# iris-ua/iris_lama

Measured on AMD Instinct MI355X. Metric: particle-scans/sec, higher is better.
Workload: dtype f64; 1 GPU; PFSlam2D 30 particles, 1080-beam synthetic corridor log (SURVEY.md 8(d)), res 0.05 m, patch 32, l2_max 0.5, GN+Cauchy(0.15), seed 42; particles=30, beams=1080, parallelism=particle-shard x1

## Files before the change

### include/lama_hip.h

```cpp
#ifndef LAMA_HIP_H
#define LAMA_HIP_H

#include <stdint.h>

#ifdef __cplusplus
extern "C" {
#endif

#define LAMA_HIP_OK 0
#define LAMA_HIP_E_INVALID (-1)
#define LAMA_HIP_E_HIP (-2)
#define LAMA_HIP_E_WINDOW (-3)
#define LAMA_HIP_E_CAPACITY (-4)
#define LAMA_HIP_E_STATE (-5)
#define LAMA_HIP_E_NUMERIC (-6)

typedef struct lama_hip_ctx lama_hip_ctx;

typedef struct lama_hip_cfg {
    uint32_t particles;
    double resolution;
    uint32_t patch_size;
    double l2_max;
    double meas_sigma;
// ... 21 lines not shown

int32_t lama_hip_ctx_create(const lama_hip_cfg* cfg, lama_hip_ctx** out);
void lama_hip_ctx_destroy(lama_hip_ctx* ctx);
const char* lama_hip_last_error(const lama_hip_ctx* ctx);

int32_t lama_hip_pf_init(lama_hip_ctx* ctx, const double* pts_xyz, uint32_t n,
                         const double* sensor_origin3, const double* sensor_quat_wxyz,
                         const double* pose0);

int32_t lama_hip_pf_set_poses(lama_hip_ctx* ctx, const double* poses);
int32_t lama_hip_pf_get_poses(lama_hip_ctx* ctx, double* poses);

int32_t lama_hip_pf_scan_match(lama_hip_ctx* ctx, const double* pts_xyz, uint32_t n,
                               const double* sensor_origin3, const double* sensor_quat_wxyz,
                               double* poses_out, double* loglik_out, int32_t* iters_out);

int32_t lama_hip_pf_resample(lama_hip_ctx* ctx, const int32_t* sample_idx);

int32_t lama_hip_pf_update_maps(lama_hip_ctx* ctx, const double* pts_xyz, uint32_t n,
                                const double* sensor_origin3, const double* sensor_quat_wxyz);

#define LAMA_HIP_MAP_DISTANCE 0
#define LAMA_HIP_MAP_OCCUPANCY 1
int32_t lama_hip_pf_map_patches(lama_hip_ctx* ctx, uint32_t particle, int32_t kind, uint32_t* num_patches);
int32_t lama_hip_pf_download_map(lama_hip_ctx* ctx, uint32_t particle, int32_t kind, uint32_t cap,
                                 uint64_t* patch_ids, uint8_t* cells, uint64_t* masks, uint32_t* num_patches);

int32_t lama_hip_pf_upload_map(lama_hip_ctx* ctx, uint32_t particle, int32_t kind, uint32_t num_patches,
                               const uint64_t* patch_ids, const uint8_t* cells, const uint64_t* masks);

int32_t lama_hip_pf_update_maps_begin(lama_hip_ctx* ctx, const double* pts_xyz, uint32_t n,
                                      const double* sensor_origin3, const double* sensor_quat_wxyz);
int32_t lama_hip_sync(lama_hip_ctx* ctx);
int32_t lama_hip_ctx_device(const lama_hip_ctx* ctx);

int32_t lama_hip_pf_patch_ids(lama_hip_ctx* ctx, uint32_t particle, int32_t kind, uint32_t cap, uint64_t* patch_ids, uint32_t* num_patches);
int32_t lama_hip_pf_map_checksums(lama_hip_ctx* ctx, int32_t kind, uint64_t* out);
int32_t lama_hip_pf_delete_patches(lama_hip_ctx* ctx, uint32_t particle, const uint64_t* patch_ids, uint32_t n, uint32_t* deleted);

int32_t lama_hip_match_batch(lama_hip_ctx* ctx, uint32_t particle, const double* pts_xyz, uint32_t n,
                             const double* sensor_origin3, const double* sensor_quat_wxyz,
                             const double* poses, uint32_t num_poses, double* loglik_out);

int32_t lama_hip_eval_batch(lama_hip_ctx* ctx, uint32_t particle, const double* pts_xyz, uint32_t n,
                            const double* sensor_origin3, const double* sensor_quat_wxyz,
                            const double* poses, uint32_t num_poses, double* sqnorm_out, double* loglik_out);

#define LAMA_HIP_SAMPLE_MAX_TERMS 256
int32_t lama_hip_map_sample_likelihood(lama_hip_ctx* ctx, uint32_t particle, const double* pts_xyz, uint32_t n,
                                       const double* sensor_origin3, const double* sensor_quat_wxyz, double yaw,
                                       const double* xy, uint32_t num_samples, uint32_t point_step, double* l_out);

int32_t lama_hip_map_add_obstacles(lama_hip_ctx* ctx, uint32_t particle, const uint32_t* cells_xy, uint32_t n);
int32_t lama_hip_match_solve(lama_hip_ctx* ctx, uint32_t particle, const double* pts_xyz, uint32_t n,
                             const double* sensor_origin3, const double* sensor_quat_wxyz, double* pose_inout,
                             double* out7, int32_t* iters_out, int32_t do_solve);
int32_t lama_hip_match_solve_with(lama_hip_ctx* ctx, uint32_t particle, const double* pts_xyz, uint32_t n,
                                  const double* sensor_origin3, const double* sensor_quat_wxyz, double* pose_inout,
                                  double* out7, int32_t* iters_out, int32_t strategy, uint32_t max_iterations );
int32_t lama_hip_match_eval(lama_hip_ctx* ctx, uint32_t particle, const double* pts_xyz, uint32_t n,
                            const double* sensor_origin3, const double* sensor_quat_wxyz, const double* pose,
                            double* residuals, double* jacobian);
int32_t lama_hip_match_cell_distances(lama_hip_ctx* ctx, uint32_t particle, const double* pts_xyz, uint32_t n,
                                      const double* sensor_origin3, const double* sensor_quat_wxyz, const double* pose,
                                      double* distances);

#define LAMA_HIP_ROBUST_UNIT 0
#define LAMA_HIP_ROBUST_TUKEY 1
#define LAMA_HIP_ROBUST_TDIST 2
#define LAMA_HIP_ROBUST_CAUCHY 3
#define LAMA_HIP_ROBUST_HUBER 4
#define LAMA_HIP_ROBUST_STORED 0x100
int32_t lama_hip_match_solve_batch(lama_hip_ctx* ctx, uint32_t num_problems, const uint32_t* particles, const double* pts_xyz,
                                   const uint32_t* scan_offsets, const double* sensor_origin3_per_problem,
                                   const double* sensor_quat_wxyz_per_problem, double* poses_inout, const uint32_t* max_iterations,
                                   int32_t strategy, int32_t robust_kind, double robust_param, double* out8, int32_t* iters_out,
                                   uint32_t* status_out);

#define LAMA_HIP_MAP_BUILD_FULL 1u
#define LAMA_HIP_MAP_BUILD_PRUNE 2u
int32_t lama_hip_map_integrate_scans(lama_hip_ctx* ctx, uint32_t particle, uint32_t num_scans, const double* poses4,
                                     const double* pts_xyz, const uint32_t* scan_offsets, const double* sensor_origin3_per_scan,
                                     const double* sensor_quat_wxyz_per_scan, uint32_t flags);
int32_t lama_hip_map_occupied_cells(lama_hip_ctx* ctx, uint32_t particle, uint32_t cap, uint32_t* cells_xy, uint32_t* n);

int32_t lama_hip_pf_export_particle(lama_hip_ctx* ctx, uint32_t particle, void* device_buf, uint64_t cap, uint64_t* bytes);
int32_t lama_hip_pf_import_particle(lama_hip_ctx* ctx, uint32_t particle, const void* device_buf, uint64_t bytes);
int32_t lama_hip_pf_export_particles(lama_hip_ctx* ctx, uint32_t n, const uint32_t* particles, void* const* device_bufs, const uint64_t* caps,
                                     uint64_t* bytes_out);
int32_t lama_hip_pf_import_particles(lama_hip_ctx* ctx, uint32_t n, const uint32_t* particles, const void* const* device_bufs, const uint64_t* bytes);

int32_t lama_hip_blob_alloc(lama_hip_ctx* ctx, uint64_t bytes, void** device_buf);
int32_t lama_hip_blob_free(lama_hip_ctx* ctx, void* device_buf);
int32_t lama_hip_blob_copy(lama_hip_ctx* dst_ctx, void* dst_device_buf, lama_hip_ctx* src_ctx, const void* src_device_buf, uint64_t bytes);

typedef struct lama_hip_pgo lama_hip_pgo;
int32_t lama_hip_pgo_create(int32_t device, uint32_t num_poses, const int32_t* fi, const int32_t* fj, const double* meas4,
                            const double* sqrt_info3, uint32_t num_factors, lama_hip_pgo** out);
void lama_hip_pgo_destroy(lama_hip_pgo* g);
const char* lama_hip_pgo_last_error(const lama_hip_pgo* g);
int32_t lama_hip_pgo_linearize(lama_hip_pgo* g, const double* poses4, double* err, double* Hdiag, double* Hoff, double* b,
                               double* chi2, double* kernel_ms);

int32_t lama_hip_pgo_pattern(const lama_hip_pgo* g, int32_t* row_ptr, int32_t* cols, uint32_t* nnzb);
int32_t lama_hip_pgo_set_poses(lama_hip_pgo* g, const double* poses4);
int32_t lama_hip_pgo_get_poses(lama_hip_pgo* g, double* poses4);
int32_t lama_hip_pgo_linearize_system(lama_hip_pgo* g, double* blocks, double* b, double* diag, double* half_chi2, double* kernel_ms);
int32_t lama_hip_pgo_try_step(lama_hip_pgo* g, const double* dx, double* half_chi2, double* kernel_ms);
int32_t lama_hip_pgo_accept(lama_hip_pgo* g);

typedef struct lama_hip_counters {
    double ms_scan_match;  uint64_t launches_scan_match;
    double ms_update_maps; uint64_t launches_update_maps;
    double ms_raycast;     uint64_t launches_raycast;
    double ms_brushfire;   uint64_t launches_brushfire;
    double ms_resample;    uint64_t launches_resample;
    uint64_t gn_iterations;
    uint64_t gn_evals;
    uint64_t ray_cells;
    uint64_t bf_cells;
    uint64_t dm_patches;
    uint64_t occ_patches;
    double ms_eval_batch;  uint64_t launches_eval_batch;
    uint64_t arena_growths;
    uint64_t window_shifts;
    uint64_t wrap_guard_scans;
    uint32_t brushfire_mode;
    uint32_t brushfire_waves;
    uint64_t sequential_raycast_scans;
    uint64_t parallel_raycast_scans;
    uint32_t brushfire_handovers;
    uint32_t replay_handovers;
    uint32_t window_patches;
    uint32_t window_growths;
    uint64_t bf_longest_chain_sum;
    uint64_t bf_longest_chain_last;
    uint64_t brushfire_early;
    uint64_t brushfire_routed;
    uint64_t pool_growths;
    uint64_t resample_clones;
    uint64_t resample_bytes;
    uint64_t hbm_bytes_allocated;
    uint64_t hbm_bytes_used;
    uint64_t hbm_bytes_total;
    uint32_t peer_access;
    uint32_t struct_bytes;
    double peer_copy_ms;
    uint64_t peer_copy_bytes;
} lama_hip_counters;
int32_t lama_hip_get_counters(lama_hip_ctx* ctx, lama_hip_counters* out);
int32_t lama_hip_get_counters_sized(lama_hip_ctx* ctx, void* out, uint32_t bytes);
uint32_t lama_hip_counters_bytes(void);
int32_t lama_hip_reset_counters(lama_hip_ctx* ctx);

#ifdef __cplusplus
}
#endif
#endif
```

### iris_lama_amd/csrc/lama_hip.hip

```cpp
#include "../../include/lama_hip.h"

#include <hip/hip_runtime.h>

#include <algorithm>
#include <cmath>
#include <cstdio>
#include <cstdlib>
#include <cstring>
#include <map>
#include <memory>
#include <mutex>
#include <string>
#include <vector>

#include "lama_kernels.h"
#include "lama_pgo.h"
#include "lama_map_build.h"
#include "lama_match_batch.h"
#include "../host/pgo_pattern.hpp"

using namespace lama_dev;

namespace {

// ... 19 lines not shown
    }
    size_t bytes() const { return n * sizeof(T); }
    void swap(DevBuf& o) { std::swap(p, o.p); std::swap(n, o.n); }
    operator T*() const { return p; }
};

template <class H, hipError_t (*Destroy)(H)>
struct HipHandle {
    H h = nullptr;
    HipHandle() {}
    HipHandle(HipHandle&& o) noexcept : h(o.h) { o.h = nullptr; }
    HipHandle& operator=(HipHandle&&) = delete;
    ~HipHandle() { if (h) (void)Destroy(h); }
    operator H() const { return h; }
};
using Stream = HipHandle<hipStream_t, hipStreamDestroy>;
using Event = HipHandle<hipEvent_t, hipEventDestroy>;
struct Delete { template <class T> void operator()(T* q) const { delete q; } };

struct RegionAlloc;
struct PoolChunk {
    DevBuf<uint8_t> plane[4];
    uint32_t patches = 0;
};
struct MapStore {
    DevBuf<int16_t> dm_dir, occ_dir;
    int32_t* counts = nullptr;
    std::vector<PoolChunk> dm_chunks, occ_chunks;
};
constexpr size_t DM_PLANE_B[3] = {SV_PATCH_BYTES, 4096, 128};
constexpr size_t OCC_PLANE_B[4] = {4096, 128, 128, 4};
struct HostPart { uint32_t home, dm_chunk, dm_off, dm_cap, occ_chunk, occ_off, occ_cap; };

struct RegionAlloc {
    std::map<uint32_t, uint32_t> free_;
    uint32_t cap = 0, used = 0;
    void reset(uint32_t c) { free_.clear(); cap = c; used = 0; if (c) free_[0] = c; }
    bool alloc(uint32_t n, uint32_t& off)
    {
        if (n == 0) { off = 0; return true; }
        for (auto it = free_.begin(); it != free_.end(); ++it) {
            if (it->second < n) continue;
            off = it->first;
            const uint32_t rest = it->second - n;
            free_.erase(it);
            if (rest) free_[off + n] = rest;
            used += n;
            return true;
        }
        return false;
    }
    void release(uint32_t off, uint32_t n)
    {
        if (n == 0) return;
        used -= n;
        auto nx = free_.lower_bound(off);
        if (nx != free_.begin()) {
            auto pv = std::prev(nx);
            if (pv->first + pv->second == off) { off = pv->first; n += pv->second; free_.erase(pv); }
        }
        if (nx != free_.end() && off + n == nx->first) { n += nx->second; free_.erase(nx); }
        free_[off] = n;
    }
    void extend(uint32_t newcap) { if (newcap > cap) { const uint32_t o = cap, n = newcap - cap; cap = newcap; used += n; release(o, n); } }
    uint32_t largest_free() const { uint32_t m = 0; for (auto& kv : free_) m = std::max(m, kv.second); return m; }
};

}

template <class T>
struct PinVec {
    T* p = nullptr; size_t n = 0, cap = 0; bool pinned = false;
    PinVec() {}
    PinVec(const PinVec&) = delete;
    PinVec& operator=(const PinVec&) = delete;
    ~PinVec() { release(); }
    void release() { if (p) { if (pinned) (void)hipHostFree(p); else std::free(p); } p = nullptr; }
    void reserve(size_t m)
    {
        if (m <= cap) return;
        m = std::max(m, 2 * cap);
        T* q = nullptr;
        bool pin = hipHostMalloc((void**)&q, m * sizeof(T), hipHostMallocDefault) == hipSuccess && q;
        if (!pin) { (void)hipGetLastError(); q = (T*)std::malloc(m * sizeof(T)); }
        if (!q) std::abort();
        if (p) std::memcpy(q, p, n * sizeof(T));
        release();
        p = q; cap = m; pinned = pin;
    }
    void resize(size_t m) { reserve(m); if (m > n) std::memset(p + n, 0, (m - n) * sizeof(T)); n = m; }
    void assign(size_t m, T v) { reserve(m); n = m; for (size_t i = 0; i < m; ++i) p[i] = v; }
    T* data() { return p; }
    const T* data() const { return p; }
    size_t size() const { return n; }
    T& operator[](size_t i) { return p[i]; }
    const T& operator[](size_t i) const { return p[i]; }
};

struct lama_hip_ctx {
    lama_hip_cfg cfg;
    std::string error;
    Stream stream;
    Event ev0, ev1;
    struct PendingTimer { hipEvent_t a, b; double* acc; uint64_t* launches; };
    std::vector<Event> ev_pool;
    std::vector<PendingTimer> pending;
    size_t ev_used = 0;
    bool initialised = false;
    bool poisoned = false;

    uint32_t P = 0, W = 0, WC = 0, wx0 = 0, wy0 = 0;
    uint32_t max_sqdist = 0;
    double scale = 0, off = 0;

    MapStore ms;
    std::vector<RegionAlloc> ra_dm, ra_occ;
    std::vector<HostPart> h_part;
    DevBuf<PartRec> d_part;
    PinVec<PartRec> h_part_stage;
    PinVec<CloneJob> h_jobs; DevBuf<CloneJob> d_jobs;
    PinVec<ZeroJob> h_zjobs; DevBuf<ZeroJob> d_zjobs;
    uint32_t floor_dm = 128, floor_occ = 128;
    PinVec<uint32_t> h_guard;
    uint64_t clone_bytes = 0;
    double* d_poses = nullptr;
    DevBuf<uint64_t> d_qlower, d_qraise;
    uint64_t* d_stats = nullptr;
    DevBuf<uint32_t> d_qsizes;
    DevBuf<uint64_t> d_dbg;
    DevBuf<uint32_t> d_slow;
    DevBuf<uint32_t> d_slow_list; uint32_t* d_slow_n = nullptr;
    DevBuf<uint8_t> d_heavy;
    DevBuf<uint8_t> d_early; DevBuf<uint32_t> d_elist;
    Stream stream3; Event ev_alloc, ev_go, ev_early;
    bool early_ok = false;
    uint32_t early_candidates = 0;
    std::vector<double> h_ll; bool ll_valid = false;
    PinVec<uint32_t> h_hlist; DevBuf<uint32_t> d_hlist;
    uint32_t early_on = 1;
    uint32_t early_min_count = 1024;
    Stream stream2; Event ev_route, ev_heavy;
    uint32_t route_min_count = 64, route_min_events = 48, route_percent = 150, route_cap = 64;
    bool route_forced = false; uint32_t num_cus = 256;
    bool debug_tail = false, debug_window = false;
    uint32_t big_stage_pad = 0;
    DevBuf<uint64_t> d_act; DevBuf<uint32_t> d_act_count;
    DevBuf<lama_dev::RayRec> d_rrec; DevBuf<uint64_t> d_rbbox; DevBuf<lama_dev::RayChunk> d_rchunk;
    int32_t* d_err = nullptr;
    DevBuf<double> d_pts; uint32_t last_n = 0;
    PinVec<uint64_t> h_stats;
    PinVec<double> h_tfs, h_pts;
    PinVec<int32_t> h_err;
    PinVec<uint32_t> h_slow_n;
    DevBuf<double> d_tfs;
    double* d_loglik = nullptr; int32_t* d_iters = nullptr;
    DevBuf<uint8_t> d_results;
    size_t results_bytes = 0, status_off = 0, status_bytes = 0;
    PinVec<uint8_t> h_status;
    PinVec<uint8_t> h_results;
    DevBuf<int32_t> d_oldcounts;
    DevBuf<double> d_mb_pts, d_mb_tfs; DevBuf<uint32_t> d_mb_offs; DevBuf<lama_dev::MbRay> d_mb_rays;
    DevBuf<uint32_t> d_mb_table, d_mb_off, d_mb_list, d_mb_bins; DevBuf<int32_t> d_mb_slot; DevBuf<uint64_t> d_mb_meta;
    PinVec<double> h_mb_tfs; PinVec<uint32_t> h_mb_offs; PinVec<uint64_t> h_mb_meta;
    DevBuf<double> d_bposes, d_bout;
    DevBuf<double> d_msb_f64; DevBuf<uint32_t> d_msb_u32;
    PinVec<double> h_msb_f64; PinVec<uint32_t> h_msb_u32;

    double scan_reach = 0.0;
    uint32_t visit_bound = 0;
    DevBuf<uint32_t> d_scalar;
    DevBuf<lama_dev::ShipDesc> d_ship_desc; DevBuf<uint8_t> d_ship_heads;
    PinVec<lama_dev::ShipDesc> h_ship_desc; PinVec<uint8_t> h_ship_heads;
    uint32_t* d_guard = nullptr;
    Affine last_mtf; uint32_t last_first = 0, last_count = 0;
    bool last_guarded = false;
    int recover_depth = 0;
    int64_t mbx0 = 0, mbx1 = 0, mby0 = 0, mby1 = 0; bool mb_valid = false;
    bool unguarded_retry = false;
    uint32_t saved_visit_bound = 0; lama_hip_counters saved_ctr;
    bool pending_maps = false;
    PinVec<double> h_poses;
    PinVec<int32_t> h_counts;
    lama_hip_counters ctr;

    ~lama_hip_ctx()
    {
        (void)hipSetDevice(cfg.device);
        if (stream) (void)hipStreamSynchronize(stream);
    }
};

namespace {

int32_t hip_fail(lama_hip_ctx* ctx, hipError_t e, const char* what)
{
    ctx->error = std::string(what) + ": " + hipGetErrorString(e);
    (void)hipStreamSynchronize(ctx->stream);
    return LAMA_HIP_E_HIP;
}
#define HIPCHK(ctx, call)                                                                              \
    do {                                                                                               \
        const hipError_t e_ = (call);                                                                  \
        if (e_ != hipSuccess) return hip_fail((ctx), e_, #call);                                       \
    } while (0)

int32_t fail(lama_hip_ctx* ctx, int32_t code, const std::string& msg)
{
    ctx->error = msg;
    return code;
}

Affine moving_tf(const double* origin3, const double* q)
{
    Affine a;
    const double w = q ? q[0] : 1.0, x = q ? q[1] : 0.0, y = q ? q[2] : 0.0, z = q ? q[3] : 0.0;
    const double tx = 2.0 * x, ty = 2.0 * y, tz = 2.0 * z;
    const double twx = tx * w, twy = ty * w, twz = tz * w;
    const double txx = tx * x, txy = ty * x, txz = tz * x;
    const double tyy = ty * y, tyz = tz * y, tzz = tz * z;
    a.R[0][0] = 1.0 - (tyy + tzz); a.R[0][1] = txy - twz;         a.R[0][2] = txz + twy;
    a.R[1][0] = txy + twz;         a.R[1][1] = 1.0 - (txx + tzz); a.R[1][2] = tyz - twx;
    a.R[2][0] = txz - twy;         a.R[2][1] = tyz + twx;         a.R[2][2] = 1.0 - (txx + tyy);
    for (int i = 0; i < 3; ++i) a.t[i] = origin3 ? origin3[i] : 0.0;
    return a;
}

void host_scan_tf(const double* pose4, const Affine& m, double* out12)
{
    const double theta = std::atan2(pose4[1], pose4[0]);
    const double sn = std::sin(theta), cs = std::cos(theta);
    const double F[3][3] = {{cs, 0.0 - sn, 0.0}, {sn, cs, 0.0}, {0.0, 0.0, (1.0 - cs) + cs}};
    const double ft[3] = {pose4[2], pose4[3], 0.0};
    for (int i = 0; i < 3; ++i) {
        for (int j = 0; j < 3; ++j) out12[3 * i + j] = (F[i][0] * m.R[0][j] + F[i][1] * m.R[1][j]) + F[i][2] * m.R[2][j];
        out12[9 + i] = ((F[i][0] * m.t[0] + F[i][1] * m.t[1]) + F[i][2] * m.t[2]) + ft[i];
    }
}

DevParams make_params(const lama_hip_ctx* c)
{
    DevParams p;
    p.P = c->P; p.W = c->W; p.WC = c->WC; p.wx0 = c->wx0; p.wy0 = c->wy0;
    p.qcap = c->cfg.queue_capacity; p.part = c->d_part;
    p.max_sqdist = c->max_sqdist; p.max_iter = c->cfg.max_iter;
    p.scale = c->scale; p.off = c->off; p.resolution = c->cfg.resolution;
    p.maxdist = std::sqrt((double)c->max_sqdist) * c->cfg.resolution;
    p.meas_sigma = c->cfg.meas_sigma;
    p.trunc_ray = c->cfg.truncated_ray; p.trunc_range = c->cfg.truncated_range;
    const MapStore& s = c->ms;
    p.dm_dir = s.dm_dir; p.occ_dir = s.occ_dir; p.counts = s.counts;
    p.guard = c->d_guard;
    p.guard_r = ((uint32_t)std::ceil(std::sqrt((double)c->max_sqdist)) + 1u + 31u) / 32u;
    p.poses = c->d_poses; p.q_lower = c->d_qlower; p.q_raise = c->d_qraise; p.stats = c->d_stats; p.qsizes = c->d_qsizes; p.err = c->d_err; p.dbg = c->d_dbg; p.slow = c->d_slow; p.slow_list = c->d_slow_list; p.slow_n = c->d_slow_n; p.heavy = nullptr; p.elist = nullptr; p.elist_n = nullptr; p.early = nullptr; p.lane = 0;
    p.act = c->d_act; p.act_count = c->d_act_count; p.act_cap = c->cfg.active_capacity;
    p.occ_policy = c->cfg.occupancy_policy; p.ray_rule = c->cfg.ray_rule; p.strategy = c->cfg.solver_strategy;
    auto logods = [](float prob) { return (double)(float)std::log(prob / (1.0 - prob)); };
    p.lo_miss = logods(0.4f); p.lo_hit = logods(0.7f); p.lo_min = logods(0.12f); p.lo_max = logods(0.97f);
    return p;
}

int32_t upload_scan(lama_hip_ctx* c, const double* pts, uint32_t n)
{
    if (!pts) {
        if (c->last_n == 0 || n != c->last_n) return fail(c, LAMA_HIP_E_INVALID, "pts == NULL but no matching scan is resident");
        return LAMA_HIP_OK;
    }
    c->last_n = n;
    HIPCHK(c, c->d_pts.grow((size_t)3 * n, (size_t)3 * 2048));
    c->h_pts.resize((size_t)3 * n);
    std::memcpy(c->h_pts.data(), pts, sizeof(double) * 3 * n);
    double r2 = 0.0;
    for (uint32_t i = 0; i < n; ++i) r2 = std::max(r2, pts[3 * i] * pts[3 * i] + pts[3 * i + 1] * pts[3 * i + 1] + pts[3 * i + 2] * pts[3 * i + 2]);
    if (!std::isfinite(r2)) { c->last_n = 0; return fail(c, LAMA_HIP_E_INVALID, "the scan holds a non-finite point (filter NaN / inf ranges before the update, as iris_lama_ros does)"); }
    c->scan_reach = std::sqrt(r2);
    HIPCHK(c, hipMemcpyAsync(c->d_pts, c->h_pts.data(), sizeof(double) * 3 * n, hipMemcpyHostToDevice, c->stream));
    return LAMA_HIP_OK;
}

int32_t ensure_batch(lama_hip_ctx* c, size_t entries, size_t floor = 0)
{
    if (entries <= c->d_bout.n) return LAMA_HIP_OK;
    c->d_bposes.reset(); c->d_bout.reset();
    const size_t cap = std::max(entries, floor);
    HIPCHK(c, c->d_bposes.alloc(4 * cap));
    HIPCHK(c, c->d_bout.alloc(cap));
    return LAMA_HIP_OK;
}

void resolve_timers(lama_hip_ctx* c);

int32_t grow_arenas(lama_hip_ctx* c, uint32_t need_dm, uint32_t need_occ);
int32_t recover_update(lama_hip_ctx* c, int32_t e);
int32_t run_update_maps(lama_hip_ctx* c, uint32_t n, const Affine& mtf, uint32_t first, uint32_t count);
int32_t permute_particles(lama_hip_ctx* c, const int32_t* idx);

int32_t check_device_errors(lama_hip_ctx* c, bool maps = false, bool match = false, bool err_in_results = false)
{
    c->h_err.resize(1);
    int32_t& e = c->h_err[0];
    e = 0;
    const bool stats = maps || match;
    const bool packed = maps && !err_in_results;
    if (stats) c->h_stats.resize((size_t)c->P * 4);
    if (packed) {
        c->h_status.resize(c->status_bytes); c->h_guard.resize(c->P); c->h_slow_n.resize(5);
        HIPCHK(c, hipMemcpyAsync(c->h_status.data(), c->d_results + c->status_off, c->status_bytes, hipMemcpyDeviceToHost, c->stream));
    } else {
        if (stats) {
            HIPCHK(c, hipMemcpyAsync(c->h_counts.data(), c->ms.counts, sizeof(int32_t) * 2 * c->P, hipMemcpyDeviceToHost, c->stream));
            if (maps) { c->h_guard.resize(c->P); HIPCHK(c, hipMemcpyAsync(c->h_guard.data(), c->d_guard, sizeof(uint32_t) * c->P, hipMemcpyDeviceToHost, c->stream)); }
            HIPCHK(c, hipMemcpyAsync(c->h_stats.data(), c->d_stats, sizeof(uint64_t) * c->h_stats.size(), hipMemcpyDeviceToHost, c->stream));
        }
        if (!err_in_results) HIPCHK(c, hipMemcpyAsync(&e, c->d_err, sizeof(e), hipMemcpyDeviceToHost, c->stream));
        if (maps) { c->h_slow_n.resize(5); HIPCHK(c, hipMemcpyAsync(c->h_slow_n.data(), c->d_slow_n, 5 * sizeof(uint32_t), hipMemcpyDeviceToHost, c->stream)); }
    }
    HIPCHK(c, hipStreamSynchronize(c->stream));
    if (packed) {
        const uint8_t* b = c->h_status.data();
        const size_t o_slow = (const uint8_t*)c->d_slow_n - (c->d_results + c->status_off);
        std::memcpy(&e, b, sizeof(e));
        std::memcpy(c->h_slow_n.data(), b + o_slow, 5 * sizeof(uint32_t));
        std::memcpy(c->h_stats.data(), b + o_slow + 32, sizeof(uint64_t) * 4 * c->P);
        std::memcpy(c->h_guard.data(), b + o_slow + 32 + sizeof(uint64_t) * 4 * c->P, sizeof(uint32_t) * c->P);
        std::memcpy(c->h_counts.data(), b + o_slow + 32 + sizeof(uint64_t) * 4 * c->P + sizeof(uint32_t) * 2 * c->P, sizeof(int32_t) * 2 * c->P);
    }
    if (maps) { c->ctr.brushfire_handovers += c->h_slow_n[0]; c->ctr.replay_handovers += c->h_slow_n[1] + c->h_slow_n[3]; c->ctr.brushfire_routed += c->h_slow_n[2] + c->h_slow_n[4]; c->ctr.brushfire_early += c->h_slow_n[4]; c->early_candidates = c->h_slow_n[2] + c->h_slow_n[4]; }
    if (err_in_results) std::memcpy(&e, c->h_results.data() + ((const uint8_t*)c->d_err - c->d_results), sizeof(e));
    resolve_timers(c);
    if (e != 0) {
        HIPCHK(c, hipMemsetAsync(c->d_err, 0, sizeof(int32_t), c->stream));
        if (maps && (e & ERR_CLEAN_ABORT) && (e & (ERR_DM_CAP | ERR_OCC_CAP)) && !(e & ERR_WINDOW) && c->last_guarded && c->recover_depth < 10) {
            const int32_t rr = recover_update(c, e);
            if (rr != LAMA_HIP_E_CAPACITY) return rr;
        }
        if (e & (ERR_DM_CAP | ERR_OCC_CAP)) {
            if (!stats) HIPCHK(c, hipMemcpyAsync(c->h_counts.data(), c->ms.counts, sizeof(int32_t) * 2 * c->P, hipMemcpyDeviceToHost, c->stream));
            HIPCHK(c, hipStreamSynchronize(c->stream));
            bool clamped = false;
            for (uint32_t p = 0; p < c->P; ++p) {
                const HostPart& hp = c->h_part[p];
                if ((uint32_t)c->h_counts[2 * p] > hp.dm_cap) { c->h_counts[2 * p] = (int32_t)hp.dm_cap; clamped = true; }
                if ((uint32_t)c->h_counts[2 * p + 1] > hp.occ_cap) { c->h_counts[2 * p + 1] = (int32_t)hp.occ_cap; clamped = true; }
            }
            if (clamped) {
                HIPCHK(c, hipMemcpyAsync(c->ms.counts, c->h_counts.data(), sizeof(int32_t) * 2 * c->P, hipMemcpyHostToDevice, c->stream));
                HIPCHK(c, hipStreamSynchronize(c->stream));
            }
        }
        if (e & ERR_WINDOW) return fail(c, LAMA_HIP_E_WINDOW, "a map cell fell outside the device window (the mapped area is wider than 1016 patches)");
        if (e & ERR_DM_CAP) return fail(c, LAMA_HIP_E_CAPACITY, "a particle's distance map exceeds 32767 patches (or the device is out of memory)");
        if (e & ERR_OCC_CAP) return fail(c, LAMA_HIP_E_CAPACITY, "a particle's occupancy map exceeds 32767 patches (or the device is out of memory)");
        if (e & ERR_QUEUE) return fail(c, LAMA_HIP_E_CAPACITY, "brushfire queue full (raise cfg.queue_capacity)");
        return fail(c, LAMA_HIP_E_NUMERIC, "unit complex number is (near) zero (SophusException in the reference)");
    }
    if (stats) {
        const PinVec<uint64_t>& st = c->h_stats;
        uint64_t dm = 0, oc = 0;
        for (uint32_t p = 0; p < c->P; ++p) {
            if (match) { c->ctr.gn_iterations += st[4 * p]; c->ctr.gn_evals += st[4 * p + 1]; }
            if (maps) { c->ctr.ray_cells += st[4 * p + 2]; c->ctr.bf_cells += st[4 * p + 3]; }
            dm += c->h_counts[2 * p]; oc += c->h_counts[2 * p + 1];
        }
        c->ctr.dm_patches = dm; c->ctr.occ_patches = oc;
        if (maps) {
            uint64_t mx = 0, sum = 0; uint32_t arg = 0;
            for (uint32_t p = 0; p < c->P; ++p) { sum += st[4 * p + 3]; if (st[4 * p + 3] > mx) { mx = st[4 * p + 3]; arg = p; } }
            c->ctr.bf_longest_chain_sum += mx; c->ctr.bf_longest_chain_last = mx;
            if (c->debug_tail) {
                uint32_t rank = 0; double ll = 0, mean_ll = 0;
                if (c->h_results.size() >= c->results_bytes && c->P > 1) {
                    const double* L = reinterpret_cast<const double*>(c->h_results.data() + sizeof(double) * 4 * c->P);
                    ll = L[arg];
                    for (uint32_t p = 0; p < c->P; ++p) { rank += L[p] < ll ? 1u : 0u; mean_ll += L[p]; }
                    mean_ll /= c->P;
                }
                std::fprintf(stderr, "brushfire pops: mean %.0f max %llu (particle %u) handovers %u brushfire %.3f ms; log-lik of that particle %.1f (pool mean %.1f), rank %u of %u\n", (double)sum / c->P, (unsigned long long)mx, arg, c->h_slow_n[0], c->ctr.ms_brushfire, ll, mean_ll, rank, c->P);
            }
        }
        if (maps) return grow_arenas(c, 0, 0);
    }
    return LAMA_HIP_OK;
}

constexpr uint32_t MAX_PATCHES = 32767u;

static uint32_t round_up32(uint32_t v) { return (v + 31u) / 32u * 32u; }

static uint32_t want_capacity(uint32_t floor_cap, uint32_t count, uint32_t extra)
{
    const uint32_t head = std::max<uint32_t>(std::max<uint32_t>(32u, count / 4u), extra);
    return std::min<uint32_t>(MAX_PATCHES, std::max<uint32_t>(floor_cap, round_up32(count + head)));
}

static PartRec dev_part(const lama_hip_ctx* c, const HostPart& h)
{
    PartRec r{};
    r.home = h.home; r.dm_cap = h.dm_cap; r.occ_cap = h.occ_cap;
    const PoolChunk& d = c->ms.dm_chunks[h.dm_chunk];
    const PoolChunk& o = c->ms.occ_chunks[h.occ_chunk];
    r.dm_sv = (sv_t*)(d.plane[0] + (size_t)h.dm_off * DM_PLANE_B[0]);
    r.dm_obs = (uint32_t*)(d.plane[1] + (size_t)h.dm_off * DM_PLANE_B[1]);
    r.dm_mask = (uint64_t*)(d.plane[2] + (size_t)h.dm_off * DM_PLANE_B[2]);
    r.occ = (uint32_t*)(o.plane[0] + (size_t)h.occ_off * OCC_PLANE_B[0]);
    r.occ_mask = (uint64_t*)(o.plane[1] + (size_t)h.occ_off * OCC_PLANE_B[1]);
    r.occ_hit = (uint64_t*)(o.plane[2] + (size_t)h.occ_off * OCC_PLANE_B[2]);
    r.rev = (int32_t*)(o.plane[3] + (size_t)h.occ_off * OCC_PLANE_B[3]);
    return r;
}

int32_t upload_part(lama_hip_ctx* c)
{
    c->h_part_stage.resize(c->P);
    for (uint32_t p = 0; p < c->P; ++p) c->h_part_stage[p] = dev_part(c, c->h_part[p]);
    HIPCHK(c, hipMemcpyAsync(c->d_part, c->h_part_stage.data(), sizeof(PartRec) * c->P, hipMemcpyHostToDevice, c->stream));
    return LAMA_HIP_OK;
}

int32_t add_chunk(lama_hip_ctx* c, bool dm, uint32_t min_patches)
{
    std::vector<PoolChunk>& chunks = dm ? c->ms.dm_chunks : c->ms.occ_chunks;
    uint64_t total = 0;
    for (const PoolChunk& k : chunks) total += k.patches;
    uint64_t want = std::max<uint64_t>(std::max<uint64_t>(min_patches, total / 4u), 1024u);
    want = (want + 1023u) / 1024u * 1024u;
    const uint64_t per_patch = dm ? (SV_PATCH_BYTES + 4096 + 128) : (4096 + 128 + 128 + 4);
    size_t free_b = 0, total_b = 0;
    if (hipMemGetInfo(&free_b, &total_b) == hipSuccess) {
        const uint64_t room = free_b > (1ull << 30) ? free_b - (1ull << 30) : 0;
        if (want * per_patch > room) want = room / per_patch / 32u * 32u;
        if (want < min_patches)
            return fail(c, LAMA_HIP_E_CAPACITY, std::string(dm ? "distance-map" : "occupancy") + " pool: the device has no room for " + std::to_string(min_patches) + " more patches");
    }
    if (want > 0xFFFFFFF0ull) want = 0xFFFFFFF0ull;
    PoolChunk k;
    k.patches = (uint32_t)want;
    const int nplanes = dm ? 3 : 4;
    for (int i = 0; i < nplanes; ++i) {
        const size_t bytes = (size_t)k.patches * (dm ? DM_PLANE_B[i] : OCC_PLANE_B[i]);
        hipError_t e = k.plane[i].alloc(bytes);
        if (e == hipSuccess && !(!dm && i == 3)) e = hipMemsetAsync(k.plane[i], 0, bytes, c->stream);
        if (e != hipSuccess) {
            (void)hipGetLastError();
            return fail(c, LAMA_HIP_E_CAPACITY, std::string(dm ? "distance-map" : "occupancy") + " pool: " + hipGetErrorString(e));
        }
    }
    chunks.push_back(std::move(k));
    (dm ? c->ra_dm : c->ra_occ).emplace_back();
    (dm ? c->ra_dm : c->ra_occ).back().reset(chunks.back().patches);
    c->ctr.pool_growths += 1;
    return LAMA_HIP_OK;
}

int32_t region_alloc(lama_hip_ctx* c, bool dm, uint32_t n, uint32_t& chunk, uint32_t& off)
{
    std::vector<RegionAlloc>& ras = dm ? c->ra_dm : c->ra_occ;
    for (uint32_t k = 0; k < ras.size(); ++k)
        if (ras[k].alloc(n, off)) { chunk = k; return LAMA_HIP_OK; }
    const int32_t rc = add_chunk(c, dm, n);
    if (rc) return rc;
    chunk = (uint32_t)ras.size() - 1;
    if (!ras[chunk].alloc(n, off)) return fail(c, LAMA_HIP_E_CAPACITY, "patch pool exhausted");
    return LAMA_HIP_OK;
}
static void region_release(lama_hip_ctx* c, bool dm, uint32_t chunk, uint32_t off, uint32_t n) { (dm ? c->ra_dm : c->ra_occ)[chunk].release(off, n); }

static void region_ptrs(const lama_hip_ctx* c, const HostPart& h, void* out[5])
{
    const PartRec r = dev_part(c, h);
    out[0] = r.dm_sv; out[1] = r.dm_obs; out[2] = r.dm_mask; out[3] = r.occ; out[4] = r.occ_mask;
}

static int32_t run_jobs(lama_hip_ctx* c, bool zero_first, size_t j0 = 0, size_t z0 = 0)
{
    const uint32_t nj = (uint32_t)(c->h_jobs.size() - j0), nz = (uint32_t)(c->h_zjobs.size() - z0);
    if (nj == 0 && nz == 0) return LAMA_HIP_OK;
    HIPCHK(c, c->d_jobs.grow(nj, 256));
    HIPCHK(c, c->d_zjobs.grow(nz, 256));
    const DevParams prm = make_params(c);
    if (nj) HIPCHK(c, hipMemcpyAsync(c->d_jobs, c->h_jobs.data() + j0, sizeof(CloneJob) * nj, hipMemcpyHostToDevice, c->stream));
    if (nz) HIPCHK(c, hipMemcpyAsync(c->d_zjobs, c->h_zjobs.data() + z0, sizeof(ZeroJob) * nz, hipMemcpyHostToDevice, c->stream));
    if (nz && zero_first) hipLaunchKernelGGL(k_zero_regions, dim3(nz, 5, CLONE_SPLIT), dim3(256), 0, c->stream, (const ZeroJob*)c->d_zjobs);
    if (nj) hipLaunchKernelGGL(k_clone_particles, dim3(nj, 7, CLONE_SPLIT), dim3(256), 0, c->stream, prm, (const CloneJob*)c->d_jobs);
    if (nz && !zero_first) hipLaunchKernelGGL(k_zero_regions, dim3(nz, 5, CLONE_SPLIT), dim3(256), 0, c->stream, (const ZeroJob*)c->d_zjobs);
    HIPCHK(c, hipGetLastError());
    return LAMA_HIP_OK;
}

struct CapRequest { uint32_t p, dm_cap, occ_cap; };
int32_t set_capacities(lama_hip_ctx* c, const std::vector<CapRequest>& reqs)
{
    constexpr size_t GROUP = 64;
    struct Old { bool dm; uint32_t chunk, off, cap; };
    bool any = false;
    int32_t err = LAMA_HIP_OK;
    c->h_jobs.resize(0); c->h_zjobs.resize(0);
    c->h_jobs.reserve(reqs.size()); c->h_zjobs.reserve(reqs.size());
    for (size_t g0 = 0; g0 < reqs.size() && err == LAMA_HIP_OK; g0 += GROUP) {
        std::vector<Old> released;
        const size_t j0 = c->h_jobs.size(), z0 = c->h_zjobs.size();
        for (size_t q = g0; q < std::min(reqs.size(), g0 + GROUP); ++q) {
            const CapRequest& r = reqs[q];
            HostPart& hp = c->h_part[r.p];
            const bool gd = r.dm_cap > hp.dm_cap, go = r.occ_cap > hp.occ_cap;
            if (!gd && !go) continue;
            if (r.dm_cap > MAX_PATCHES || r.occ_cap > MAX_PATCHES) { err = fail(c, LAMA_HIP_E_CAPACITY, "a particle's map exceeds 32767 patches"); break; }
            const HostPart before = hp;
            uint32_t dch = 0, doff = 0, och = 0, ooff = 0;
            if (gd) { err = region_alloc(c, true, r.dm_cap, dch, doff); if (err) break; }
            if (go) { err = region_alloc(c, false, r.occ_cap, och, ooff); if (err) { if (gd) region_release(c, true, dch, doff, r.dm_cap); break; } }
            if (gd) {
                released.push_back(Old{true, hp.dm_chunk, hp.dm_off, hp.dm_cap});
                hp.dm_chunk = dch; hp.dm_off = doff; hp.dm_cap = r.dm_cap;
            }
            if (go) {
                released.push_back(Old{false, hp.occ_chunk, hp.occ_off, hp.occ_cap});
                hp.occ_chunk = och; hp.occ_off = ooff; hp.occ_cap = r.occ_cap;
            }
            CloneJob j{};
            j.src_home = j.dst_home = hp.home;
            j.sdm = c->h_counts[2 * r.p]; j.socc = c->h_counts[2 * r.p + 1];
            void* sp[5]; void* dp[5];
            region_ptrs(c, before, sp); region_ptrs(c, hp, dp);
            ZeroJob z{};
            for (int k = 0; k < 5; ++k) { j.s[k] = sp[k]; j.d[k] = dp[k]; z.d[k] = (sp[k] != dp[k]) ? sp[k] : nullptr; }
            z.ndm = j.sdm; z.nocc = j.socc;
            c->h_jobs.resize(c->h_jobs.size() + 1); c->h_jobs[c->h_jobs.size() - 1] = j;
            c->h_zjobs.resize(c->h_zjobs.size() + 1); c->h_zjobs[c->h_zjobs.size() - 1] = z;
        }
        if (released.empty()) continue;
        any = true;
        const int32_t rc = run_jobs(c, false, j0, z0);
        if (rc) return rc;
        for (const Old& o : released) region_release(c, o.dm, o.chunk, o.off, o.cap);
    }
    if (!any) return err;
    const std::string msg = c->error;
    const int32_t rc = upload_part(c);
    if (rc) return rc;
    HIPCHK(c, hipStreamSynchronize(c->stream));
    c->ctr.arena_growths += 1;
    if (err) c->error = msg;
    return err;
}

int32_t grow_arenas(lama_hip_ctx* c, uint32_t , uint32_t )
{
    std::vector<CapRequest> reqs;
    for (uint32_t p = 0; p < c->P; ++p) {
        const HostPart& pr = c->h_part[p];
        const uint32_t dmc = (uint32_t)c->h_counts[2 * p], occ = (uint32_t)c->h_counts[2 * p + 1];
        const uint32_t gh = p < c->h_guard.size() ? c->h_guard[p] : 0u;
        uint32_t nd = pr.dm_cap, no = pr.occ_cap;
        if (dmc + std::max<uint32_t>(std::max<uint32_t>(16u, dmc / 16u), gh) > pr.dm_cap) nd = want_capacity(c->floor_dm, dmc, gh + gh / 4u);
        if (occ + std::max<uint32_t>(16u, occ / 16u) > pr.occ_cap) no = want_capacity(c->floor_occ, occ, 0u);
        if (nd > pr.dm_cap || no > pr.occ_cap) reqs.push_back(CapRequest{p, std::max(nd, pr.dm_cap), std::max(no, pr.occ_cap)});
    }
    if (reqs.empty()) return LAMA_HIP_OK;
    return set_capacities(c, reqs);
}

int32_t recover_update(lama_hip_ctx* c, int32_t e)
{
    ++c->recover_depth;
    c->visit_bound = c->saved_visit_bound;
    {
        const lama_hip_counters now = c->ctr;
        c->ctr = c->saved_ctr;
        c->ctr.arena_growths = now.arena_growths; c->ctr.pool_growths = now.pool_growths; c->ctr.dm_patches = now.dm_patches; c->ctr.occ_patches = now.occ_patches;
    }
    DevParams prm = make_params(c);
    const size_t WW = (size_t)c->W * c->W;
    hipLaunchKernelGGL(k_update_cleanup, dim3(c->P, (unsigned)((WW + 255) / 256)), dim3(256), 0, c->stream, prm);
    for (const PoolChunk& k : c->ms.occ_chunks) HIPCHK(c, hipMemsetAsync(k.plane[2], 0, (size_t)k.patches * 128, c->stream));
    HIPCHK(c, hipMemsetAsync(c->d_act_count, 0, (size_t)c->P * 4, c->stream));
    HIPCHK(c, hipMemsetAsync(c->d_err, 0, sizeof(int32_t), c->stream));
    c->h_guard.resize(c->P);
    HIPCHK(c, hipMemcpyAsync(c->h_counts.data(), c->ms.counts, sizeof(int32_t) * 2 * c->P, hipMemcpyDeviceToHost, c->stream));
    HIPCHK(c, hipMemcpyAsync(c->h_guard.data(), c->d_guard, sizeof(uint32_t) * c->P, hipMemcpyDeviceToHost, c->stream));
    HIPCHK(c, hipStreamSynchronize(c->stream));
    std::vector<CapRequest> reqs;
    bool at_limit = false, fixed_counts = false;
    for (uint32_t p = 0; p < c->P; ++p) {
        HostPart& pr = c->h_part[p];
        uint32_t wdm = (uint32_t)c->h_counts[2 * p], wocc = (uint32_t)c->h_counts[2 * p + 1];
        uint32_t nd = pr.dm_cap, no = pr.occ_cap;
        if (wocc > pr.occ_cap) { no = want_capacity(c->floor_occ, wocc, 0u); c->h_counts[2 * p + 1] = (int32_t)pr.occ_cap; fixed_counts = true; }
        if (wdm > pr.dm_cap) { c->h_counts[2 * p] = (int32_t)pr.dm_cap; wdm = pr.dm_cap; fixed_counts = true; nd = want_capacity(c->floor_dm, wdm, 64u); }
        const uint32_t gh = c->h_guard[p];
        if ((e & ERR_DM_CAP) && !c->unguarded_retry && (uint64_t)wdm + gh > pr.dm_cap) {
            if ((uint64_t)wdm + gh > MAX_PATCHES) at_limit = true;
            nd = std::max(nd, std::min<uint32_t>(MAX_PATCHES, round_up32(wdm + gh + gh / 8u + 16u)));
        }
        if (nd > pr.dm_cap || no > pr.occ_cap) {
            if (no > MAX_PATCHES || (wocc > MAX_PATCHES)) { --c->recover_depth; return LAMA_HIP_E_CAPACITY; }
            reqs.push_back(CapRequest{p, std::max(nd, pr.dm_cap), std::max(no, pr.occ_cap)});
        }
    }
    if (fixed_counts) HIPCHK(c, hipMemcpyAsync(c->ms.counts, c->h_counts.data(), sizeof(int32_t) * 2 * c->P, hipMemcpyHostToDevice, c->stream));
    if (reqs.empty() && !at_limit) { --c->recover_depth; return LAMA_HIP_E_CAPACITY; }
    if (at_limit && c->unguarded_retry) { --c->recover_depth; return LAMA_HIP_E_CAPACITY; }
    int32_t rc = set_capacities(c, reqs);
    const bool saved_unguarded = c->unguarded_retry;
    c->unguarded_retry = at_limit;
    if (rc == LAMA_HIP_OK) rc = run_update_maps(c, c->last_n, c->last_mtf, c->last_first, c->last_count);
    if (rc == LAMA_HIP_OK) rc = check_device_errors(c, true, false);
    --c->recover_depth;
    c->unguarded_retry = saved_unguarded;
    return rc;
}

int32_t finish_pending(lama_hip_ctx* c)
{
    if (!c->pending_maps) return LAMA_HIP_OK;
    c->pending_maps = false;
    (void)hipSetDevice(c->cfg.device);
    const int32_t rc = check_device_errors(c, true, false);
    if (rc) c->error = "deferred from lama_hip_pf_update_maps_begin: " + c->error;
    return rc;
}
#define ENTER(c) do { if ((c)->poisoned) return fail((c), LAMA_HIP_E_STATE, "the context ran out of device memory in the middle of a resample and cannot continue"); const int32_t rc_enter_ = finish_pending(c); if (rc_enter_) return rc_enter_; } while (0)

struct Timer {
    lama_hip_ctx* c; double* acc; uint64_t* launches; hipEvent_t a = nullptr, b = nullptr;
    Timer(lama_hip_ctx* c_, double* acc_, uint64_t* l_) : c(c_), acc(acc_), launches(l_)
    {
        if (!c->cfg.profile) return;
        if (c->ev_used + 2 > c->ev_pool.size())
            for (int i = 0; i < 2; ++i) { c->ev_pool.emplace_back(); (void)hipEventCreate(&c->ev_pool.back().h); }
        a = c->ev_pool[c->ev_used++]; b = c->ev_pool[c->ev_used++];
        (void)hipEventRecord(a, c->stream);
    }
    void stop()
    {
        if (!c->cfg.profile) return;
        (void)hipEventRecord(b, c->stream);
        c->pending.push_back({a, b, acc, launches});
    }
};

void resolve_timers(lama_hip_ctx* c)
{
    for (auto& t : c->pending) {
        float ms = 0;
        if (hipEventElapsedTime(&ms, t.a, t.b) == hipSuccess) { *t.acc += ms; *t.launches += 1; }
    }
    c->pending.clear();
    c->ev_used = 0;
    c->ctr.ms_update_maps = c->ctr.ms_raycast + c->ctr.ms_brushfire;
    c->ctr.launches_update_maps = c->ctr.launches_raycast;
}

constexpr int64_t LAMA_HIP_MAX_WINDOW = 1016;

int32_t regrid_window(lama_hip_ctx* c, uint32_t newW, int64_t nox, int64_t noy)
{
    const int64_t ox = c->wx0 >> 5, oy = c->wy0 >> 5;
    const int dx = (int)(nox - ox), dy = (int)(noy - oy);
    const size_t WW = (size_t)c->W * c->W, nWW = (size_t)newW * newW, P = c->P;
    if (!c->initialised && newW == c->W) { c->wx0 = (uint32_t)(nox * 32); c->wy0 = (uint32_t)(noy * 32); return LAMA_HIP_OK; }
    {
        size_t free_b = 0, total_b = 0;
        if (hipMemGetInfo(&free_b, &total_b) == hipSuccess && 2 * P * nWW * 2 + (1ull << 28) > free_b)
            return fail(c, LAMA_HIP_E_WINDOW, "not enough device memory to re-tile the window directories (" + std::to_string(2 * P * nWW * 2 >> 20) + " MB for a " + std::to_string(newW) + "-patch window)");
    }
    DevBuf<int16_t> nd[2];
    for (int k = 0; k < 2; ++k) {
        hipError_t e = nd[k].alloc(P * nWW);
        if (e == hipSuccess && newW != c->W) e = hipMemsetAsync(nd[k], 0xFF, P * nWW * 2, c->stream);
        if (e != hipSuccess) return hip_fail(c, e, "window directories");
    }
    const dim3 grid((unsigned)P, (unsigned)((std::max(WW, nWW) + 255) / 256));
    int16_t* const to_dm = nd[0]; int16_t* const to_occ = nd[1];
    hipLaunchKernelGGL(k_shift_window, grid, dim3(256), 0, c->stream, c->ms.dm_dir, to_dm, c->W, newW, dx, dy, WW, nWW, c->d_err);
    hipLaunchKernelGGL(k_shift_window, grid, dim3(256), 0, c->stream, c->ms.occ_dir, to_occ, c->W, newW, dx, dy, WW, nWW, c->d_err);
    {
        hipError_t e = hipGetLastError();
        if (e == hipSuccess) e = hipStreamSynchronize(c->stream);
        if (e != hipSuccess) return hip_fail(c, e, "k_shift_window");
    }
    c->ms.dm_dir.swap(nd[0]); c->ms.occ_dir.swap(nd[1]);
    if (newW != c->W) {
        c->W = newW; c->WC = newW * 32; c->cfg.window_patches = newW;
        c->ctr.window_growths += 1;
    }
    c->wx0 = (uint32_t)(nox * 32); c->wy0 = (uint32_t)(noy * 32);
    c->ctr.window_shifts += 1;
    c->ctr.window_patches = c->W;
    return LAMA_HIP_OK;
}

int32_t ensure_window(lama_hip_ctx* c, int64_t x0, int64_t x1, int64_t y0, int64_t y1)
{
    if (!c->mb_valid) { c->mbx0 = x0; c->mbx1 = x1; c->mby0 = y0; c->mby1 = y1; c->mb_valid = true; }
    else { c->mbx0 = std::min(c->mbx0, x0); c->mbx1 = std::max(c->mbx1, x1); c->mby0 = std::min(c->mby0, y0); c->mby1 = std::max(c->mby1, y1); }
    const int64_t ox = c->wx0 >> 5, oy = c->wy0 >> 5, W = c->W;
    if (c->debug_window) std::fprintf(stderr, "ensure_window: box x [%ld, %ld] y [%ld, %ld] mapped x [%ld, %ld] y [%ld, %ld] window x [%ld, %ld) y [%ld, %ld)\n", (long)x0, (long)x1, (long)y0, (long)y1, (long)c->mbx0, (long)c->mbx1, (long)c->mby0, (long)c->mby1, (long)ox, (long)(ox + W), (long)oy, (long)(oy + W));
    if (c->mbx0 >= ox && c->mbx1 < ox + W && c->mby0 >= oy && c->mby1 < oy + W) return LAMA_HIP_OK;
    const int64_t span = std::max(c->mbx1 - c->mbx0 + 1, c->mby1 - c->mby0 + 1);
    int64_t newW = W;
    if (span > W) newW = std::min<int64_t>(LAMA_HIP_MAX_WINDOW, std::max<int64_t>((span + 8 + 7) / 8 * 8, (W + W / 2 + 7) / 8 * 8));
    int64_t hx0 = c->mbx0, hx1 = c->mbx1, hy0 = c->mby0, hy1 = c->mby1;
    if (span > newW) { hx0 = x0; hx1 = x1; hy0 = y0; hy1 = y1; if (x1 - x0 + 1 > newW || y1 - y0 + 1 > newW) return LAMA_HIP_OK; }
    auto place = [&](int64_t o, int64_t lo, int64_t hi) {
        const int64_t a = hi - newW + 1, b = lo;
        int64_t no = std::min(std::max(o, a), b);
        if (no > o) no = std::min(no + 4, b); else if (no < o) no = std::max(no - 4, a);
        return no;
    };
    const int64_t nox = c->initialised ? place(ox, hx0, hx1) : (hx0 + hx1 + 1) / 2 - newW / 2;
    const int64_t noy = c->initialised ? place(oy, hy0, hy1) : (hy0 + hy1 + 1) / 2 - newW / 2;
    return regrid_window(c, (uint32_t)newW, nox, noy);
}

int32_t start_without_first_scan(lama_hip_ctx* c)
{
    if (c->initialised) return LAMA_HIP_OK;
    for (uint32_t p = 0; p < c->P; ++p) { c->h_poses[4 * p] = 1.0; c->h_poses[4 * p + 1] = 0.0; c->h_poses[4 * p + 2] = 0.0; c->h_poses[4 * p + 3] = 0.0; }
    HIPCHK(c, hipMemcpyAsync(c->d_poses, c->h_poses.data(), sizeof(double) * 4 * c->P, hipMemcpyHostToDevice, c->stream));
    c->initialised = true;
    return LAMA_HIP_OK;
}

int32_t fit_window(lama_hip_ctx* c, const Affine& mtf, uint32_t first, uint32_t count)
{
    double far = c->scan_reach;
    if (c->cfg.ray_rule == 0 && c->cfg.truncated_range > 0.0) far = std::min(far, c->cfg.truncated_range);
    const uint32_t guard_r = ((uint32_t)std::ceil(std::sqrt((double)c->max_sqdist)) + 1u + 31u) / 32u;
    const double reach = far + std::sqrt(mtf.t[0] * mtf.t[0] + mtf.t[1] * mtf.t[1]) + (double)(guard_r + 1u) * 32.0 * c->cfg.resolution;
    double xlo = 1e300, xhi = -1e300, ylo = 1e300, yhi = -1e300;
    for (uint32_t p = first; p < first + count; ++p) {
        const double x = c->h_poses[4 * p + 2], y = c->h_poses[4 * p + 3];
        xlo = std::min(xlo, x - reach); xhi = std::max(xhi, x + reach);
        ylo = std::min(ylo, y - reach); yhi = std::max(yhi, y + reach);
    }
    auto patch = [&](double w) { return (int64_t)std::floor((c->scale * w + c->off) / 32.0); };
    return ensure_window(c, patch(xlo), patch(xhi), patch(ylo), patch(yhi));
}

static unsigned xcd_grid(const lama_hip_ctx* c, uint32_t first, uint32_t count)
{
    return (first == 0 && count == c->P) ? (count + 7u) / 8u * 8u : count;
}

int32_t launch_allocation_phase(lama_hip_ctx* c, const DevParams& prm, uint32_t n, uint32_t first, uint32_t count, int alloc_only)
{
    const size_t need = (size_t)c->P * n;
    if (need > c->d_rrec.n) {
        c->d_rrec.reset(); c->d_rbbox.reset(); c->d_rchunk.reset();
        hipError_t e = c->d_rrec.alloc(need);
        if (e == hipSuccess) e = c->d_rbbox.alloc(need);
        if (e == hipSuccess) e = c->d_rchunk.alloc((size_t)c->P * ((n + 63) / 64));
        if (e != hipSuccess) { c->d_rrec.reset(); return hip_fail(c, e, "ray buffers"); }
    }
    hipLaunchKernelGGL(k_ray_hits, dim3(xcd_grid(c, first, count), (n + 255) / 256), dim3(256), 0, c->stream, prm, c->d_pts, (int)n, c->d_tfs, (int)first,
                       c->d_rrec, c->d_rbbox, alloc_only, c->d_rchunk);
    const int rw_seg = count <= 64 ? 4 : 1;
    hipLaunchKernelGGL(k_ray_alloc_walk, dim3(xcd_grid(c, first, count), (n * rw_seg + 255) / 256), dim3(256), 0, c->stream, prm, (const lama_dev::RayRec*)c->d_rrec, (int)n, (int)first, rw_seg);
    double far = c->scan_reach;
    if (c->cfg.truncated_range > 0.0) far = std::min(far, c->cfg.truncated_range);
    const int reach_cells = (int)std::ceil(far * c->scale) + 2;
    hipLaunchKernelGGL(k_occ_reverse_dir, dim3(count), dim3(256), 0, c->stream, prm, (int)first, (const double*)c->d_tfs, reach_cells,
                       c->unguarded_retry ? 1 : 0);
    return LAMA_HIP_OK;
}

static uint32_t route_places(const lama_hip_ctx* c, uint32_t count)
{
    const uint32_t slots = c->num_cus * 12u;
    if (c->route_forced || count >= slots) return c->route_cap;
    return std::min<uint32_t>(c->route_cap, std::max<uint32_t>(8u, (slots - count) / 7u));
}

int32_t run_update_maps(lama_hip_ctx* c, uint32_t n, const Affine& mtf, uint32_t first, uint32_t count)
{
    {
        const int32_t rcw = fit_window(c, mtf, first, count);
        if (rcw) return rcw;
    }
    c->last_mtf = mtf; c->last_first = first; c->last_count = count;
    if (c->recover_depth == 0) { c->saved_visit_bound = c->visit_bound; c->saved_ctr = c->ctr; }
    PinVec<double>& tfs = c->h_tfs;
    tfs.resize((size_t)c->P * 12);
    for (uint32_t p = 0; p < c->P; ++p) host_scan_tf(&c->h_poses[4 * p], mtf, &tfs[12 * (size_t)p]);
    HIPCHK(c, hipMemcpyAsync(c->d_tfs, tfs.data(), sizeof(double) * tfs.size(), hipMemcpyHostToDevice, c->stream));
    DevParams prm = make_params(c);
    bool early_lane = false;
    {
        Timer t(c, &c->ctr.ms_raycast, &c->ctr.launches_raycast);
        (void)hipMemsetAsync(c->d_slow_n, 0, 32 + sizeof(uint64_t) * 4 * c->P, c->stream);
        bool sequential = c->cfg.sequential_raycast == 1 || c->cfg.occupancy_policy == 1 ||
                          c->cfg.ray_rule == 1;
        if (!sequential && (n > 4096u || (uint64_t)n + 4096u > c->cfg.active_capacity)) sequential = true;
        if (!sequential && (uint64_t)c->visit_bound + n >= 65536u) {
            uint32_t m = 0;
            if (c->initialised) {
                (void)hipMemsetAsync(c->d_scalar, 0, sizeof(uint32_t), c->stream);
                hipLaunchKernelGGL(k_occ_max_visited, dim3(c->P), dim3(256), 0, c->stream, prm, c->d_scalar);
                HIPCHK(c, hipMemcpyAsync(&m, c->d_scalar, sizeof(uint32_t), hipMemcpyDeviceToHost, c->stream));
                HIPCHK(c, hipStreamSynchronize(c->stream));
            }
            c->visit_bound = m;
            if ((uint64_t)m + n >= 65536u) { sequential = true; c->ctr.wrap_guard_scans += 1; }
        }
        c->visit_bound = (uint32_t)std::min<uint64_t>((uint64_t)c->visit_bound + n, 65535u);
        if (sequential) c->ctr.sequential_raycast_scans += 1; else c->ctr.parallel_raycast_scans += 1;
        c->last_guarded = c->cfg.ray_rule == 0;
        if (!c->last_guarded) {
            const double side = 32.0 * c->cfg.resolution;
            const double rp = c->scan_reach / side + 2.5;
            const uint32_t bound = (uint32_t)std::min(32767.0, std::ceil(3.1416 * rp * rp));
            std::vector<CapRequest> reqs;
            for (uint32_t p = first; p < first + count; ++p) {
                const HostPart& pr = c->h_part[p];
                const uint32_t nd = std::min<uint32_t>(MAX_PATCHES, round_up32((uint32_t)c->h_counts[2 * p] + bound)), no = std::min<uint32_t>(MAX_PATCHES, round_up32((uint32_t)c->h_counts[2 * p + 1] + bound));
                if (nd > pr.dm_cap || no > pr.occ_cap) reqs.push_back(CapRequest{p, std::max(nd, pr.dm_cap), std::max(no, pr.occ_cap)});
            }
            if (!reqs.empty()) {
                const int32_t rg = set_capacities(c, reqs);
                if (rg) return rg;
                prm = make_params(c);
            }
        }
        if (sequential) {
            if (c->last_guarded) { const int32_t ra = launch_allocation_phase(c, prm, n, first, count, 1); if (ra) return ra; }
            hipLaunchKernelGGL(k_raycast, dim3(count), dim3(UM_BLOCK), 0, c->stream, prm, c->d_pts, (int)n, c->d_tfs, (int)first);
        } else {
            const bool two_waves_e = c->cfg.brushfire_waves == 2 || (c->cfg.brushfire_waves == 0 && count <= BF_TW_MAX_PARTICLES);
            early_lane = c->early_on && two_waves_e && c->cfg.brushfire_mode == 0 && first == 0 && count == c->P &&
                         count >= std::max<uint32_t>(c->route_min_count, c->early_min_count) && c->route_cap > 0;
            uint32_t host_n = 0;
            if (early_lane && c->ll_valid) {
                const uint32_t places = route_places(c, count);
                double mean = 0; for (uint32_t p = 0; p < c->P; ++p) mean += c->h_ll[p]; mean /= c->P;
                const double lim = 2.5 * std::min(mean, 0.0) - 5.0;
                std::vector<std::pair<double, uint32_t>> cand;
                for (uint32_t p = 0; p < c->P; ++p) if (c->h_ll[p] < lim) cand.emplace_back(c->h_ll[p], p);
                if (cand.size() > places) { std::partial_sort(cand.begin(), cand.begin() + places, cand.end()); cand.resize(places); }
                c->h_hlist.resize(256);
                for (auto& e : cand) c->h_hlist[host_n++] = e.second;
                if (host_n) HIPCHK(c, hipMemcpyAsync(c->d_hlist, c->h_hlist.data(), sizeof(uint32_t) * host_n, hipMemcpyHostToDevice, c->stream));
            }
            const bool prev_ok = c->early_ok && c->early_candidates > 0;
            early_lane = early_lane && (host_n > 0 || prev_ok);
            if (early_lane)
                hipLaunchKernelGGL(k_early_list, dim3(1), dim3(256), 0, c->stream, prev_ok ? (const uint8_t*)c->d_heavy : (const uint8_t*)nullptr,
                                   (const uint32_t*)c->d_hlist, host_n, c->d_early, c->d_elist, c->d_slow_n + 4, (int)c->P, route_places(c, count));
            { const int32_t ra = launch_allocation_phase(c, prm, n, first, count, 0); if (ra) return ra; }
#ifdef LAMA_WAVE_SIM
            const unsigned gy = 4u;
#else
            const unsigned gy = count <= 64 ? 128u : (count >= 1024 ? 8u : 32u);
#endif
            if (early_lane) {
                DevParams pe = prm;
                pe.elist = c->d_elist; pe.elist_n = c->d_slow_n + 4; pe.lane = 1;
                const unsigned eg = route_places(c, count);
                hipLaunchKernelGGL(k_ray_patches, dim3(eg, 128u), dim3(256), 0, c->stream, pe, (const lama_dev::RayRec*)c->d_rrec,
                                   (const uint64_t*)c->d_rbbox, (const lama_dev::RayChunk*)c->d_rchunk, (int)n, 0);
                hipLaunchKernelGGL((k_ray_replay<RP_SORT_SMALL, RP_SORT_SMALL, false, RP_BLOCK_LARGE>), dim3(eg), dim3(RP_BLOCK_LARGE), 0, c->stream, pe, 0);
                hipLaunchKernelGGL((k_ray_replay<8192, 8192, true, RP_BLOCK_LARGE>), dim3(eg), dim3(RP_BLOCK_LARGE), 0, c->stream, pe, 0);
                HIPCHK(c, hipEventRecord(c->ev_alloc, c->stream));
                HIPCHK(c, hipStreamWaitEvent(c->stream3, c->ev_alloc, 0));
                hipLaunchKernelGGL(k_mark_early, dim3(1), dim3(64), 0, c->stream3, pe);
                HIPCHK(c, hipEventRecord(c->ev_go, c->stream3));
                hipLaunchKernelGGL((k_brushfire<LQ_BIG, RQ_BIG, true, true>), dim3(eg), dim3(2 * UM_BLOCK), c->big_stage_pad, c->stream3, pe, 0, 2);
                HIPCHK(c, hipEventRecord(c->ev_early, c->stream3));
                HIPCHK(c, hipStreamWaitEvent(c->stream, c->ev_go, 0));
                prm.early = c->d_early;
            }
            hipLaunchKernelGGL(k_ray_patches, dim3(xcd_grid(c, first, count), gy), dim3(256), 0, c->stream, prm, (const lama_dev::RayRec*)c->d_rrec,
                               (const uint64_t*)c->d_rbbox, (const lama_dev::RayChunk*)c->d_rchunk, (int)n, (int)first);
            const unsigned resume_grid = std::min<unsigned>(count, 256u);
            if (count <= 512) {
                hipLaunchKernelGGL((k_ray_replay<RP_SORT_SMALL, RP_SORT_SMALL, false, RP_BLOCK_LARGE>), dim3(count), dim3(RP_BLOCK_LARGE), 0, c->stream, prm, (int)first);
                hipLaunchKernelGGL((k_ray_replay<8192, 8192, true, RP_BLOCK_LARGE>), dim3(resume_grid), dim3(RP_BLOCK_LARGE), 0, c->stream, prm, (int)first);
            } else {
                hipLaunchKernelGGL((k_ray_replay<RP_SORT_SMALL, RP_SORT_SMALL, false, RP_BLOCK_SMALL>), dim3(count), dim3(RP_BLOCK_SMALL), 0, c->stream, prm, (int)first);
                hipLaunchKernelGGL((k_ray_replay<8192, 8192, true, RP_BLOCK_SMALL>), dim3(resume_grid), dim3(RP_BLOCK_SMALL), 0, c->stream, prm, (int)first);
            }
        }
        t.stop();
    }
    HIPCHK(c, hipGetLastError());
    {
        Timer t(c, &c->ctr.ms_brushfire, &c->ctr.launches_brushfire);
        if (c->cfg.brushfire_mode == 1)
            hipLaunchKernelGGL(k_brushfire_canon, dim3(count), dim3(CN_BLOCK), 0, c->stream, prm, (int)first);
        const bool two_waves = c->cfg.brushfire_waves == 2 || (c->cfg.brushfire_waves == 0 && count <= BF_TW_MAX_PARTICLES);
        c->ctr.brushfire_mode = c->cfg.brushfire_mode;
        c->ctr.brushfire_waves = two_waves ? 2u : 1u;
        const unsigned resume_grid = std::min<unsigned>(count, 256u);
        const bool route = two_waves && count >= c->route_min_count && c->route_cap > 0;
        if (two_waves) {
            if (route) {
                prm.heavy = c->d_heavy;
                hipLaunchKernelGGL(k_bf_route, dim3(1), dim3(256), 0, c->stream, prm, (int)first, (int)count, c->route_min_events, c->route_percent, route_places(c, count));
                HIPCHK(c, hipEventRecord(c->ev_route, c->stream));
                hipLaunchKernelGGL((k_brushfire<LQ_BIG, RQ_BIG, true, true>), dim3(route_places(c, count)), dim3(2 * UM_BLOCK), 0, c->stream, prm, (int)first, 1);
                HIPCHK(c, hipStreamWaitEvent(c->stream2, c->ev_route, 0));
                hipLaunchKernelGGL((k_brushfire<LQ_SMALL, RQ_SMALL, false, true>), dim3(count), dim3(2 * UM_BLOCK), 0, c->stream2, prm, (int)first, 0);
                HIPCHK(c, hipEventRecord(c->ev_heavy, c->stream2));
                HIPCHK(c, hipStreamWaitEvent(c->stream, c->ev_heavy, 0));
            } else {
                hipLaunchKernelGGL((k_brushfire<LQ_SMALL, RQ_SMALL, false, true>), dim3(count), dim3(2 * UM_BLOCK), 0, c->stream, prm, (int)first, 0);
            }
            hipLaunchKernelGGL((k_brushfire<LQ_BIG, RQ_BIG, true, true>), dim3(resume_grid), dim3(2 * UM_BLOCK), 0, c->stream, prm, (int)first, 0);
        } else {
            hipLaunchKernelGGL((k_brushfire<LQ_SMALL, RQ_SMALL, false, false>), dim3(count), dim3(UM_BLOCK), 0, c->stream, prm, (int)first, 0);
            hipLaunchKernelGGL((k_brushfire<LQ_BIG, RQ_BIG, true, false>), dim3(resume_grid), dim3(UM_BLOCK), 0, c->stream, prm, (int)first, 0);
        }
        if (early_lane) HIPCHK(c, hipStreamWaitEvent(c->stream, c->ev_early, 0));
        hipLaunchKernelGGL(k_brushfire_slow, dim3(count), dim3(UM_BLOCK), 0, c->stream, prm, (int)first);
        c->early_ok = route && first == 0 && count == c->P;
        t.stop();
    }
    HIPCHK(c, hipGetLastError());
    return LAMA_HIP_OK;
}


int32_t permute_particles(lama_hip_ctx* c, const int32_t* idx)
{
    const uint32_t P = c->P;
    std::vector<uint8_t> taken(P, 0);
    std::vector<HostPart> np(P);
    std::vector<int32_t> nc(2 * (size_t)P);
    std::vector<double> npose(4 * (size_t)P);
    std::vector<uint32_t> clones;
    for (uint32_t i = 0; i < P; ++i) {
        const uint32_t j = (uint32_t)idx[i];
        std::memcpy(&npose[4 * i], &c->h_poses[4 * j], sizeof(double) * 4);
        nc[2 * i] = c->h_counts[2 * j]; nc[2 * i + 1] = c->h_counts[2 * j + 1];
        if (!taken[j]) { taken[j] = 1; np[i] = c->h_part[j]; } else clones.push_back(i);
    }
    std::vector<uint32_t> dead;
    for (uint32_t j = 0; j < P; ++j) if (!taken[j]) dead.push_back(j);
    c->h_jobs.resize(0); c->h_zjobs.resize(0);
    c->clone_bytes = 0;
    const size_t WW = (size_t)c->W * c->W;
    uint32_t dir_off16 = 0, dir_n16 = (uint32_t)(WW * 2 / 16);
    {
        const int64_t oy = c->wy0 >> 5, W = c->W;
// ... 4 lines not shown
    }
    struct Slot { bool keep_dm, keep_occ; HostPart rec; int32_t odm, oocc; };
    std::vector<Slot> slots(dead.size());
    for (size_t k = 0; k < dead.size(); ++k) {
        const uint32_t d = dead[k], i = clones[k], j = (uint32_t)idx[i];
        const HostPart& dr = c->h_part[d];
        const HostPart& sr = c->h_part[j];
        Slot sl{dr.dm_cap == sr.dm_cap, dr.occ_cap == sr.occ_cap, dr, c->h_counts[2 * d], c->h_counts[2 * d + 1]};
        void* dp[5];
        region_ptrs(c, dr, dp);
        ZeroJob z{};
        if (!sl.keep_dm) { z.ndm = sl.odm; z.d[0] = dp[0]; z.d[1] = dp[1]; z.d[2] = dp[2]; region_release(c, true, dr.dm_chunk, dr.dm_off, dr.dm_cap); }
        if (!sl.keep_occ) { z.nocc = sl.oocc; z.d[3] = dp[3]; z.d[4] = dp[4]; region_release(c, false, dr.occ_chunk, dr.occ_off, dr.occ_cap); }
        if (z.ndm || z.nocc) { c->h_zjobs.resize(c->h_zjobs.size() + 1); c->h_zjobs[c->h_zjobs.size() - 1] = z; }
        slots[k] = sl;
    }
    for (size_t k = 0; k < dead.size(); ++k) {
        const uint32_t i = clones[k], j = (uint32_t)idx[i];
        const HostPart sr = c->h_part[j];
        Slot& sl = slots[k];
        HostPart r = sl.rec;
        r.dm_cap = sr.dm_cap; r.occ_cap = sr.occ_cap;
        CloneJob job{};
        job.src_home = sr.home; job.dst_home = r.home;
        job.sdm = c->h_counts[2 * j]; job.socc = c->h_counts[2 * j + 1];
        if (sl.keep_dm) job.odm = sl.odm;
        else { const int32_t rc = region_alloc(c, true, sr.dm_cap, r.dm_chunk, r.dm_off); if (rc) { c->poisoned = true; return rc; } job.odm = 0; }
        if (sl.keep_occ) job.oocc = sl.oocc;
        else { const int32_t rc = region_alloc(c, false, sr.occ_cap, r.occ_chunk, r.occ_off); if (rc) { c->poisoned = true; return rc; } job.oocc = 0; }
        void* sp[5]; void* dp[5];
        region_ptrs(c, sr, sp); region_ptrs(c, r, dp);
        for (int q = 0; q < 5; ++q) { job.s[q] = sp[q]; job.d[q] = dp[q]; }
        job.dir_off16 = dir_off16; job.dir_n16 = dir_n16;
        np[i] = r;
        c->h_jobs.resize(c->h_jobs.size() + 1); c->h_jobs[c->h_jobs.size() - 1] = job;
        c->clone_bytes += 2 * (uint64_t)dir_n16 * 16 + (uint64_t)job.sdm * (SV_PATCH_BYTES + 4096 + 128) + (uint64_t)job.socc * (4096 + 128);
    }
    c->h_part = np;
    std::memcpy(c->h_poses.data(), npose.data(), npose.size() * sizeof(double));
    std::memcpy(c->h_counts.data(), nc.data(), nc.size() * sizeof(int32_t));
    int32_t rc = upload_part(c);
    if (rc) return rc;
    {
        Timer t(c, &c->ctr.ms_resample, &c->ctr.launches_resample);
        rc = run_jobs(c, true);
        t.stop();
    }
    if (rc) return rc;
    HIPCHK(c, hipMemcpyAsync(c->ms.counts, c->h_counts.data(), sizeof(int32_t) * 2 * P, hipMemcpyHostToDevice, c->stream));
    HIPCHK(c, hipMemcpyAsync(c->d_poses, c->h_poses.data(), sizeof(double) * 4 * P, hipMemcpyHostToDevice, c->stream));
    HIPCHK(c, hipStreamSynchronize(c->stream));
    resolve_timers(c);
    c->ctr.resample_clones += clones.size();
    c->ctr.resample_bytes += c->clone_bytes;
    return LAMA_HIP_OK;
}

}

extern "C" {

void lama_hip_default_cfg(lama_hip_cfg* cfg)
{
    std::memset(cfg, 0, sizeof(*cfg));
    cfg->particles = 30;
    cfg->resolution = 0.05;
    cfg->patch_size = 32;
    cfg->l2_max = 0.5;
    cfg->meas_sigma = 0.05;
    cfg->max_iter = 100;
    cfg->device = 0;
    cfg->window_patches = 128;
    cfg->dm_patch_capacity = 128;
    cfg->occ_patch_capacity = 128;
    cfg->queue_capacity = 32768;
    cfg->active_capacity = 8192;
}

int32_t lama_hip_device_count(int32_t* count)
{
    int n = 0;
    hipError_t e = hipGetDeviceCount(&n);
    if (count) *count = (e == hipSuccess) ? n : 0;
    return e == hipSuccess ? LAMA_HIP_OK : LAMA_HIP_E_HIP;
}

const char* lama_hip_last_error(const lama_hip_ctx* ctx) { return ctx ? ctx->error.c_str() : "null context"; }

int32_t lama_hip_ctx_create(const lama_hip_cfg* cfg_in, lama_hip_ctx** out)
{
    if (!cfg_in || !out) return LAMA_HIP_E_INVALID;
    *out = nullptr;
    lama_hip_cfg cfg = *cfg_in;
    if (cfg.window_patches == 0) cfg.window_patches = 128;
    if (cfg.dm_patch_capacity == 0) cfg.dm_patch_capacity = 128;
    if (cfg.occ_patch_capacity == 0) cfg.occ_patch_capacity = 128;
    if (cfg.queue_capacity == 0) cfg.queue_capacity = 32768;
    if (cfg.active_capacity == 0) cfg.active_capacity = 8192;
    if (cfg.active_capacity > 8192) cfg.active_capacity = 8192;
    if (cfg.brushfire_mode > 1 || cfg.brushfire_waves > 2) return LAMA_HIP_E_INVALID;
    if (cfg.particles == 0 || cfg.patch_size != 32 || !(cfg.resolution > 0) || cfg.window_patches > (uint32_t)LAMA_HIP_MAX_WINDOW ||
        (cfg.window_patches & 7) || cfg.dm_patch_capacity > 32767 || cfg.occ_patch_capacity > 32767 ||
        cfg.queue_capacity < (uint32_t)LQ_BIG)
        return LAMA_HIP_E_INVALID;
    int ndev = 0;
    if (hipGetDeviceCount(&ndev) != hipSuccess || ndev <= 0 || cfg.device < 0 || cfg.device >= ndev) return LAMA_HIP_E_HIP;

    std::unique_ptr<lama_hip_ctx, Delete> owner(new lama_hip_ctx());
    lama_hip_ctx* c = owner.get();
    c->cfg = cfg;
    std::memset(&c->ctr, 0, sizeof(c->ctr));
    c->P = cfg.particles; c->W = cfg.window_patches; c->WC = c->W * 32;
    c->ctr.window_patches = c->W;
    c->debug_tail = std::getenv("LAMA_HIP_DEBUG_TAIL") != nullptr;
    c->debug_window = std::getenv("LAMA_HIP_DEBUG_WINDOW") != nullptr;
    {
        constexpr uint32_t CU_LDS = 160u * 1024u, GRAN = 1280u;
        const uint32_t used = (uint32_t)((sizeof(lama_dev::BfLds<LQ_BIG, RQ_BIG>) + GRAN - 1) / GRAN * GRAN);
        c->big_stage_pad = CU_LDS > used + 2u * GRAN ? CU_LDS - used - 2u * GRAN : 0u;
    }
    if (const char* rr = std::getenv("LAMA_HIP_BF_ROUTE")) {
        unsigned a = 0, b = 0, pc = 0, d = 0, e = 1;
        if (std::sscanf(rr, "%u,%u,%u,%u,%u", &a, &b, &pc, &d, &e) >= 4) { c->route_min_count = a; c->route_min_events = b; c->route_percent = pc; c->route_cap = std::min(d, 256u); c->early_on = e; c->early_min_count = 0; c->route_forced = true; }
    }
    c->scale = 1.0 / cfg.resolution;
    c->off = double(2642244ull >> 1) * 32.0;
    uint32_t md = (uint32_t)std::ceil(cfg.l2_max * c->scale);
    c->max_sqdist = md * md;
    if (c->max_sqdist == 0 || md > MAX_OFFSET_CELLS) return LAMA_HIP_E_INVALID;

    if (hipSetDevice(cfg.device)) return LAMA_HIP_E_HIP;
    { hipDeviceProp_t prop; if (hipGetDeviceProperties(&prop, cfg.device) == hipSuccess && prop.multiProcessorCount > 0) c->num_cus = (uint32_t)prop.multiProcessorCount; }
    if (hipStreamCreate(&c->stream.h) || hipEventCreate(&c->ev0.h) || hipEventCreate(&c->ev1.h)) return LAMA_HIP_E_HIP;
    const size_t P = c->P, WW = (size_t)c->W * c->W, dc = cfg.dm_patch_capacity, oc = cfg.occ_patch_capacity;
    {
        MapStore& m = c->ms;
        c->floor_dm = (uint32_t)dc; c->floor_occ = (uint32_t)oc;
        if (P * dc > 0xFFFFFFF0ull || P * oc > 0xFFFFFFF0ull) return LAMA_HIP_E_INVALID;
        if (m.dm_dir.alloc(P * WW) || hipMemset(m.dm_dir, 0xFF, P * WW * 2)) return LAMA_HIP_E_HIP;
        if (m.occ_dir.alloc(P * WW) || hipMemset(m.occ_dir, 0xFF, P * WW * 2)) return LAMA_HIP_E_HIP;
        if (add_chunk(c, true, (uint32_t)(P * dc)) != LAMA_HIP_OK || add_chunk(c, false, (uint32_t)(P * oc)) != LAMA_HIP_OK) return LAMA_HIP_E_HIP;
        c->ctr.pool_growths = 0;
        c->h_part.resize(P);
        for (size_t p = 0; p < P; ++p) {
            HostPart r{};
            r.home = (uint32_t)p; r.dm_cap = (uint32_t)dc; r.occ_cap = (uint32_t)oc;
            if (region_alloc(c, true, (uint32_t)dc, r.dm_chunk, r.dm_off) != LAMA_HIP_OK || region_alloc(c, false, (uint32_t)oc, r.occ_chunk, r.occ_off) != LAMA_HIP_OK) return LAMA_HIP_E_HIP;
            c->h_part[p] = r;
        }
        if (c->d_part.alloc(P)) return LAMA_HIP_E_HIP;
        if (upload_part(c) != LAMA_HIP_OK) return LAMA_HIP_E_HIP;
        if (hipStreamSynchronize(c->stream)) return LAMA_HIP_E_HIP;
    }
    c->results_bytes = P * 4 * 8 + P * 8 + P * 4 + 8;
    c->status_off = P * 4 * 8 + P * 8 + P * 4;
    const size_t slow_off = (c->results_bytes + 7) / 8 * 8;
    c->status_bytes = (slow_off - c->status_off) + 32 + P * 4 * 8 + P * 2 * 4 + P * 2 * 4;
    if (c->d_results.alloc(c->status_off + c->status_bytes) || hipMemset(c->d_results, 0, c->status_off + c->status_bytes)) return LAMA_HIP_E_HIP;
    c->d_poses = reinterpret_cast<double*>(c->d_results.p);
    c->d_loglik = c->d_poses + P * 4;
    c->d_iters = reinterpret_cast<int32_t*>(c->d_loglik + P);
    c->d_err = c->d_iters + P;
    c->d_slow_n = reinterpret_cast<uint32_t*>(c->d_results + slow_off);
    c->d_stats = reinterpret_cast<uint64_t*>(c->d_results + slow_off + 32);
    c->d_guard = reinterpret_cast<uint32_t*>(c->d_stats + P * 4);
    c->ms.counts = reinterpret_cast<int32_t*>(c->d_guard + P * 2);
    if (c->d_qlower.alloc(P * (size_t)cfg.queue_capacity) || c->d_qraise.alloc(P * (size_t)cfg.queue_capacity)) return LAMA_HIP_E_HIP;
    if (c->d_qsizes.alloc(P * 2) || hipMemset(c->d_qsizes, 0, P * 2 * 4)) return LAMA_HIP_E_HIP;
    if (c->d_dbg.alloc(P * 16 + (1u << 20) / 8) || hipMemset(c->d_dbg, 0, P * 16 * 8 + (1u << 20))) return LAMA_HIP_E_HIP;
    if (c->d_slow.alloc(P) || hipMemset(c->d_slow, 0, P * 4)) return LAMA_HIP_E_HIP;
    if (c->d_slow_list.alloc(4 * P) || hipMemset(c->d_slow_list, 0, 4 * P * 4)) return LAMA_HIP_E_HIP;
    if (c->d_heavy.alloc(P) || hipMemset(c->d_heavy, 0, P)) return LAMA_HIP_E_HIP;
    if (c->d_early.alloc(P) || hipMemset(c->d_early, 0, P)) return LAMA_HIP_E_HIP;
    if (c->d_elist.alloc(256) || hipMemset(c->d_elist, 0, 256 * 4)) return LAMA_HIP_E_HIP;
    if (c->d_hlist.alloc(256) || hipMemset(c->d_hlist, 0, 256 * 4)) return LAMA_HIP_E_HIP;
    if (hipStreamCreate(&c->stream2.h) || hipStreamCreate(&c->stream3.h)) return LAMA_HIP_E_HIP;
    if (hipEventCreateWithFlags(&c->ev_alloc.h, hipEventDisableTiming) || hipEventCreateWithFlags(&c->ev_early.h, hipEventDisableTiming) ||
        hipEventCreateWithFlags(&c->ev_go.h, hipEventDisableTiming) ||
        hipEventCreateWithFlags(&c->ev_route.h, hipEventDisableTiming) || hipEventCreateWithFlags(&c->ev_heavy.h, hipEventDisableTiming))
        return LAMA_HIP_E_HIP;
    if (c->d_scalar.alloc(4) || hipMemset(c->d_scalar, 0, 16)) return LAMA_HIP_E_HIP;
    if (c->d_act.alloc(P * (size_t)cfg.active_capacity)) return LAMA_HIP_E_HIP;
    if (c->d_act_count.alloc(P) || hipMemset(c->d_act_count, 0, P * 4)) return LAMA_HIP_E_HIP;
    if (c->d_tfs.alloc(P * 12) || c->d_oldcounts.alloc(P * 2)) return LAMA_HIP_E_HIP;
    if (hipDeviceSynchronize()) return LAMA_HIP_E_HIP;
    c->h_poses.assign(P * 4, 0.0);
    c->h_counts.assign(P * 2, 0);
    *out = owner.release();
    return LAMA_HIP_OK;
}

void lama_hip_ctx_destroy(lama_hip_ctx* c) { delete c; }

int32_t lama_hip_pf_set_poses(lama_hip_ctx* c, const double* poses)
{
    if (!c || !poses) return LAMA_HIP_E_INVALID;
    ENTER(c);
    HIPCHK(c, hipSetDevice(c->cfg.device));
    std::memcpy(c->h_poses.data(), poses, sizeof(double) * 4 * c->P);
    HIPCHK(c, hipMemcpyAsync(c->d_poses, c->h_poses.data(), sizeof(double) * 4 * c->P, hipMemcpyHostToDevice, c->stream));
    return LAMA_HIP_OK;
}

int32_t lama_hip_pf_get_poses(lama_hip_ctx* c, double* poses)
{
    if (!c || !poses) return LAMA_HIP_E_INVALID;
    ENTER(c);
    std::memcpy(poses, c->h_poses.data(), sizeof(double) * 4 * c->P);
    return LAMA_HIP_OK;
}

int32_t lama_hip_pf_init(lama_hip_ctx* c, const double* pts, uint32_t n, const double* origin3, const double* quat,
                         const double* pose0)
{
    if (!c || !pts || !pose0 || n == 0) return LAMA_HIP_E_INVALID;
    ENTER(c);
    if (c->initialised) return fail(c, LAMA_HIP_E_STATE, "lama_hip_pf_init called twice");
    HIPCHK(c, hipSetDevice(c->cfg.device));
    const double mx = c->scale * pose0[2] + c->off, my = c->scale * pose0[3] + c->off;
    const uint32_t px = ((uint32_t)mx) >> 5, py = ((uint32_t)my) >> 5;
    c->wx0 = (px - c->W / 2) * 32;
    c->wy0 = (py - c->W / 2) * 32;
    for (uint32_t p = 0; p < c->P; ++p) std::memcpy(&c->h_poses[4 * p], pose0, sizeof(double) * 4);
    HIPCHK(c, hipMemcpyAsync(c->d_poses, c->h_poses.data(), sizeof(double) * 4 * c->P, hipMemcpyHostToDevice, c->stream));
    int32_t rc = upload_scan(c, pts, n);
    if (rc) return rc;
    const Affine mtf = moving_tf(origin3, quat);
    rc = run_update_maps(c, n, mtf, 0, 1);
    if (rc) return rc;
    rc = check_device_errors(c, true, false);
    if (rc) return rc;
    if (c->P > 1) {
        std::vector<int32_t> idx(c->P, 0);
        rc = permute_particles(c, idx.data());
        if (rc) return rc;
    }
    rc = check_device_errors(c, true, false);
    if (rc) return rc;
    c->initialised = true;
    return LAMA_HIP_OK;
}

int32_t lama_hip_pf_scan_match(lama_hip_ctx* c, const double* pts, uint32_t n, const double* origin3, const double* quat,
                               double* poses_out, double* loglik_out, int32_t* iters_out)
{
    if (!c || !pts || n == 0) return LAMA_HIP_E_INVALID;
    ENTER(c);
    if (!c->initialised) return fail(c, LAMA_HIP_E_STATE, "lama_hip_pf_scan_match before lama_hip_pf_init");
    HIPCHK(c, hipSetDevice(c->cfg.device));
    int32_t rc = upload_scan(c, pts, n);
    if (rc) return rc;
    const Affine mtf = moving_tf(origin3, quat);
    DevParams prm = make_params(c);
    {
        Timer t(c, &c->ctr.ms_scan_match, &c->ctr.launches_scan_match);
        if (c->max_sqdist > (uint32_t)SM_LUT) hipLaunchKernelGGL(k_scan_match<true>, dim3(c->P), dim3(SM_BLOCK), 0, c->stream, prm, c->d_pts, (int)n, mtf, c->d_loglik, c->d_iters);
        else hipLaunchKernelGGL(k_scan_match<false>, dim3(c->P), dim3(SM_BLOCK), 0, c->stream, prm, c->d_pts, (int)n, mtf, c->d_loglik, c->d_iters);
        t.stop();
    }
    HIPCHK(c, hipGetLastError());
    c->h_results.resize(c->results_bytes);
    HIPCHK(c, hipMemcpyAsync(c->h_results.data(), c->d_results, c->results_bytes, hipMemcpyDeviceToHost, c->stream));
    rc = check_device_errors(c, false, c->cfg.profile != 0, true);
    if (rc) return rc;
    const uint8_t* r = c->h_results.data();
    std::memcpy(c->h_poses.data(), r, sizeof(double) * 4 * c->P);
    if (poses_out) std::memcpy(poses_out, r, sizeof(double) * 4 * c->P);
    if (loglik_out) std::memcpy(loglik_out, r + sizeof(double) * 4 * c->P, sizeof(double) * c->P);
    if (iters_out) std::memcpy(iters_out, r + sizeof(double) * 5 * c->P, sizeof(int32_t) * c->P);
    c->h_ll.resize(c->P); std::memcpy(c->h_ll.data(), r + sizeof(double) * 4 * c->P, sizeof(double) * c->P); c->ll_valid = true;
    return LAMA_HIP_OK;
}

int32_t lama_hip_pf_resample(lama_hip_ctx* c, const int32_t* sample_idx)
{
    if (!c || !sample_idx) return LAMA_HIP_E_INVALID;
    ENTER(c);
    if (!c->initialised) return fail(c, LAMA_HIP_E_STATE, "lama_hip_pf_resample before lama_hip_pf_init");
    for (uint32_t i = 0; i < c->P; ++i)
        if (sample_idx[i] < 0 || (uint32_t)sample_idx[i] >= c->P) return fail(c, LAMA_HIP_E_INVALID, "sample_idx out of range");
    HIPCHK(c, hipSetDevice(c->cfg.device));
    c->early_ok = false;
    if (c->ll_valid) { std::vector<double> nl(c->P); for (uint32_t i = 0; i < c->P; ++i) nl[i] = c->h_ll[sample_idx[i]]; c->h_ll.swap(nl); }
    return permute_particles(c, sample_idx);
}

int32_t lama_hip_pf_update_maps_begin(lama_hip_ctx* c, const double* pts, uint32_t n, const double* origin3, const double* quat)
{
    if (!c || n == 0) return LAMA_HIP_E_INVALID;
    ENTER(c);
    if (!c->initialised) return fail(c, LAMA_HIP_E_STATE, "lama_hip_pf_update_maps before lama_hip_pf_init");
    HIPCHK(c, hipSetDevice(c->cfg.device));
    int32_t rc = upload_scan(c, pts, n);
    if (rc) return rc;
    const Affine mtf = moving_tf(origin3, quat);
    rc = run_update_maps(c, n, mtf, 0, c->P);
    if (rc) return rc;
    c->pending_maps = true;
    return LAMA_HIP_OK;
}

int32_t lama_hip_ctx_device(const lama_hip_ctx* c) { return c ? c->cfg.device : -1; }

int32_t lama_hip_sync(lama_hip_ctx* c)
{
    if (!c) return LAMA_HIP_E_INVALID;
    HIPCHK(c, hipSetDevice(c->cfg.device));
    return finish_pending(c);
}

int32_t lama_hip_pf_update_maps(lama_hip_ctx* c, const double* pts, uint32_t n, const double* origin3, const double* quat)
{
    const int32_t rc = lama_hip_pf_update_maps_begin(c, pts, n, origin3, quat);
    if (rc) return rc;
    return lama_hip_sync(c);
}

int32_t lama_hip_pf_map_patches(lama_hip_ctx* c, uint32_t particle, int32_t kind, uint32_t* num)
{
    if (!c || !num || particle >= c->P || (kind != LAMA_HIP_MAP_DISTANCE && kind != LAMA_HIP_MAP_OCCUPANCY)) return LAMA_HIP_E_INVALID;
    ENTER(c);
    *num = (uint32_t)c->h_counts[2 * particle + (kind == LAMA_HIP_MAP_OCCUPANCY ? 1 : 0)];
    return LAMA_HIP_OK;
}

int32_t lama_hip_pf_patch_ids(lama_hip_ctx* c, uint32_t particle, int32_t kind, uint32_t cap, uint64_t* patch_ids, uint32_t* num_patches)
{
    if (!c || particle >= c->P || (kind != LAMA_HIP_MAP_DISTANCE && kind != LAMA_HIP_MAP_OCCUPANCY)) return LAMA_HIP_E_INVALID;
    ENTER(c);
    HIPCHK(c, hipSetDevice(c->cfg.device));
    const MapStore& s = c->ms;
    const size_t WW = (size_t)c->W * c->W;
    const bool dm = kind == LAMA_HIP_MAP_DISTANCE;
    std::vector<int16_t> dir(WW);
    HIPCHK(c, hipMemcpy(dir.data(), (dm ? s.dm_dir : s.occ_dir) + c->h_part[particle].home * WW, WW * 2, hipMemcpyDeviceToHost));
    std::vector<uint64_t> ids;
    for (uint32_t wy = 0; wy < c->W; ++wy)
        for (uint32_t wx = 0; wx < c->W; ++wx)
            if (dir[wy * c->W + wx] >= 0) ids.push_back(((uint64_t)(c->wx0 >> 5) + wx) * 2642244ull + ((uint64_t)(c->wy0 >> 5) + wy));
    std::sort(ids.begin(), ids.end());
    if (num_patches) *num_patches = (uint32_t)ids.size();
    if (patch_ids) for (size_t k = 0; k < ids.size() && k < cap; ++k) patch_ids[k] = ids[k];
    return LAMA_HIP_OK;
}

int32_t lama_hip_pf_map_checksums(lama_hip_ctx* c, int32_t kind, uint64_t* out)
{
    if (!c || !out || (kind != LAMA_HIP_MAP_DISTANCE && kind != LAMA_HIP_MAP_OCCUPANCY)) return LAMA_HIP_E_INVALID;
    ENTER(c);
    if (c->cfg.occupancy_policy != 0 && kind == LAMA_HIP_MAP_OCCUPANCY) return fail(c, LAMA_HIP_E_INVALID, "map checksums cover the frequency occupancy policy");
    HIPCHK(c, hipSetDevice(c->cfg.device));
    DevBuf<uint64_t> sums;
    HIPCHK(c, sums.alloc(c->P));
    uint64_t* const d_out = sums;
    DevParams prm = make_params(c);
    hipLaunchKernelGGL(k_map_checksum, dim3(c->P), dim3(256), 0, c->stream, prm, kind == LAMA_HIP_MAP_DISTANCE ? 0 : 1, d_out);
    HIPCHK(c, hipGetLastError());
    HIPCHK(c, hipMemcpyAsync(out, d_out, sizeof(uint64_t) * c->P, hipMemcpyDeviceToHost, c->stream));
    HIPCHK(c, hipStreamSynchronize(c->stream));
    return LAMA_HIP_OK;
}

int32_t lama_hip_pf_delete_patches(lama_hip_ctx* c, uint32_t particle, const uint64_t* patch_ids, uint32_t n, uint32_t* deleted)
{
    if (!c || particle >= c->P || (!patch_ids && n)) return LAMA_HIP_E_INVALID;
    ENTER(c);
    if (deleted) *deleted = 0;
    if (n == 0) return LAMA_HIP_OK;
    HIPCHK(c, hipSetDevice(c->cfg.device));
    HIPCHK(c, hipStreamSynchronize(c->stream));
    MapStore& s = c->ms;
    const size_t WW = (size_t)c->W * c->W;
    const HostPart hp = c->h_part[particle];
    const PartRec pr = dev_part(c, hp);
    for (int kind = 0; kind < 2; ++kind) {
        const bool dm = kind == 0;
        int16_t* d_dir = (dm ? s.dm_dir : s.occ_dir) + hp.home * WW;
        std::vector<int16_t> dir(WW);
        HIPCHK(c, hipMemcpy(dir.data(), d_dir, WW * 2, hipMemcpyDeviceToHost));
        int count = c->h_counts[2 * particle + (dm ? 0 : 1)];
        bool touched = false;
        for (uint32_t k = 0; k < n; ++k) {
            const uint64_t px = patch_ids[k] / 2642244ull, py = patch_ids[k] % 2642244ull;
            const int64_t wx = (int64_t)px - (int64_t)(c->wx0 >> 5), wy = (int64_t)py - (int64_t)(c->wy0 >> 5);
            if (wx < 0 || wy < 0 || wx >= (int64_t)c->W || wy >= (int64_t)c->W) continue;
            const size_t pidx = (size_t)wy * c->W + (size_t)wx;
            const int slot = dir[pidx];
            if (slot < 0) continue;
            const int last = count - 1;
            auto plane_move = [&](void* plane, size_t bytes_per_slot) -> hipError_t {
                char* b = (char*)plane;
                if (slot != last) {
                    hipError_t e = hipMemcpyAsync(b + (size_t)slot * bytes_per_slot, b + (size_t)last * bytes_per_slot, bytes_per_slot, hipMemcpyDeviceToDevice, c->stream);
                    if (e != hipSuccess) return e;
                }
                return hipMemsetAsync(b + (size_t)last * bytes_per_slot, 0, bytes_per_slot, c->stream);
            };
            if (dm) {
                HIPCHK(c, plane_move(pr.dm_sv, SV_PATCH_BYTES)); HIPCHK(c, plane_move(pr.dm_obs, 4096)); HIPCHK(c, plane_move(pr.dm_mask, 128));
            } else {
                HIPCHK(c, plane_move(pr.occ, 4096)); HIPCHK(c, plane_move(pr.occ_mask, 128));
                HIPCHK(c, plane_move(pr.occ_hit, 128));
            }
            if (slot != last)
                for (size_t q = 0; q < WW; ++q) if (dir[q] == last) { dir[q] = (int16_t)slot; break; }
            dir[pidx] = -1;
            --count;
            touched = true;
            if (dm && deleted) ++*deleted;
        }
        if (touched) {
            HIPCHK(c, hipMemcpyAsync(d_dir, dir.data(), WW * 2, hipMemcpyHostToDevice, c->stream));
            c->h_counts[2 * particle + (dm ? 0 : 1)] = count;
            HIPCHK(c, hipMemcpyAsync(s.counts + 2 * particle + (dm ? 0 : 1), &c->h_counts[2 * particle + (dm ? 0 : 1)], sizeof(int32_t), hipMemcpyHostToDevice, c->stream));
            HIPCHK(c, hipStreamSynchronize(c->stream));
        }
    }
    return LAMA_HIP_OK;
}

int32_t lama_hip_pf_download_map(lama_hip_ctx* c, uint32_t particle, int32_t kind, uint32_t cap,
                                 uint64_t* patch_ids, uint8_t* cells, uint64_t* masks, uint32_t* num_patches)
{
    if (!c || particle >= c->P || (kind != LAMA_HIP_MAP_DISTANCE && kind != LAMA_HIP_MAP_OCCUPANCY)) return LAMA_HIP_E_INVALID;
    ENTER(c);
    HIPCHK(c, hipSetDevice(c->cfg.device));
    const MapStore& s = c->ms;
    const size_t WW = (size_t)c->W * c->W;
    const bool dm = kind == LAMA_HIP_MAP_DISTANCE;
    const HostPart hp = c->h_part[particle];
    const PartRec pr = dev_part(c, hp);
    const uint32_t count = (uint32_t)c->h_counts[2 * particle + (dm ? 0 : 1)];
    if (num_patches) *num_patches = count;
    if (count == 0 || cap == 0) return LAMA_HIP_OK;
    std::vector<int16_t> dir(WW);
    HIPCHK(c, hipMemcpy(dir.data(), (dm ? s.dm_dir : s.occ_dir) + hp.home * WW, WW * 2, hipMemcpyDeviceToHost));
    std::vector<std::pair<uint64_t, int>> order;
    for (uint32_t wy = 0; wy < c->W; ++wy)
        for (uint32_t wx = 0; wx < c->W; ++wx) {
            int slot = dir[wy * c->W + wx];
            if (slot < 0) continue;
            const uint64_t px = (c->wx0 >> 5) + wx, py = (c->wy0 >> 5) + wy;
            order.emplace_back(px * 2642244ull + py, slot);
        }
    std::sort(order.begin(), order.end());
    if (order.size() != count) return fail(c, LAMA_HIP_E_STATE, "directory / count mismatch");
    std::vector<uint64_t> hmask((size_t)count * 16);
    HIPCHK(c, hipMemcpy(hmask.data(), dm ? pr.dm_mask : pr.occ_mask,
                        hmask.size() * 8, hipMemcpyDeviceToHost));
    std::vector<sv_t> hsv; std::vector<uint32_t> hobs, hocc;
    if (dm) {
// ... 281 lines not shown
    PGOCHK(g, hipMemcpyAsync(g->d_poses, poses4, sizeof(double) * 4 * g->N, hipMemcpyHostToDevice, g->stream));
    PgoPtrs p{g->d_poses, g->d_fi, g->d_fj, g->d_meas, g->d_sqrt, g->d_err, g->d_hoff, g->d_fdi, g->d_fdj, g->d_fg, g->d_incptr, g->d_inc,
              g->d_hdiag, g->d_b, g->d_chi};
    PGOCHK(g, hipEventRecord(g->ev0, g->stream));
    hipLaunchKernelGGL(k_pgo_factors, dim3(g->blocksF), dim3(PGO_BLOCK), 0, g->stream, p, g->F);
    hipLaunchKernelGGL(k_pgo_reduce, dim3((g->N + PGO_BLOCK - 1) / PGO_BLOCK), dim3(PGO_BLOCK), 0, g->stream, p, g->N);
    PGOCHK(g, hipEventRecord(g->ev1, g->stream));
    PGOCHK(g, hipGetLastError());
    if (err) PGOCHK(g, hipMemcpyAsync(err, g->d_err, sizeof(double) * 3 * g->F, hipMemcpyDeviceToHost, g->stream));
    if (Hoff) PGOCHK(g, hipMemcpyAsync(Hoff, g->d_hoff, sizeof(double) * 9 * g->F, hipMemcpyDeviceToHost, g->stream));
    if (Hdiag) PGOCHK(g, hipMemcpyAsync(Hdiag, g->d_hdiag, sizeof(double) * 9 * g->N, hipMemcpyDeviceToHost, g->stream));
    if (b) PGOCHK(g, hipMemcpyAsync(b, g->d_b, sizeof(double) * 3 * g->N, hipMemcpyDeviceToHost, g->stream));
    PGOCHK(g, hipMemcpyAsync(g->h_chi.data(), g->d_chi, sizeof(double) * g->blocksF, hipMemcpyDeviceToHost, g->stream));
    PGOCHK(g, hipStreamSynchronize(g->stream));
    if (chi2) { double t = 0; for (double x : g->h_chi) t += x; *chi2 = t; }
    if (kernel_ms) { float ms = 0; PGOCHK(g, hipEventElapsedTime(&ms, g->ev0, g->ev1)); *kernel_ms = ms; }
    return LAMA_HIP_OK;
}

int32_t lama_hip_pgo_pattern(const lama_hip_pgo* g, int32_t* row_ptr, int32_t* cols, uint32_t* nnzb)
{
    if (!g || !nnzb) return LAMA_HIP_E_INVALID;
    *nnzb = g->nnzb;
    if (row_ptr) std::copy(g->h_rowptr.begin(), g->h_rowptr.end(), row_ptr);
    if (cols) std::copy(g->h_cols.begin(), g->h_cols.end(), cols);
    return LAMA_HIP_OK;
}

int32_t lama_hip_pgo_set_poses(lama_hip_pgo* g, const double* poses4)
{
    if (!g || !poses4) return LAMA_HIP_E_INVALID;
    PGOCHK(g, hipSetDevice(g->device));
    PGOCHK(g, hipMemcpyAsync(g->d_poses, poses4, sizeof(double) * 4 * g->N, hipMemcpyHostToDevice, g->stream));
    PGOCHK(g, hipStreamSynchronize(g->stream));
    return LAMA_HIP_OK;
}

int32_t lama_hip_pgo_get_poses(lama_hip_pgo* g, double* poses4)
{
    if (!g || !poses4) return LAMA_HIP_E_INVALID;
    PGOCHK(g, hipSetDevice(g->device));
    PGOCHK(g, hipMemcpyAsync(poses4, g->d_poses, sizeof(double) * 4 * g->N, hipMemcpyDeviceToHost, g->stream));
    PGOCHK(g, hipStreamSynchronize(g->stream));
    return LAMA_HIP_OK;
}

int32_t lama_hip_pgo_linearize_system(lama_hip_pgo* g, double* blocks, double* b, double* diag, double* half_chi2, double* kernel_ms)
{
    if (!g) return LAMA_HIP_E_INVALID;
    PGOCHK(g, hipSetDevice(g->device));
    PgoPtrs p{g->d_poses, g->d_fi, g->d_fj, g->d_meas, g->d_sqrt, g->d_err, g->d_hoff, g->d_fdi, g->d_fdj, g->d_fg, g->d_incptr, g->d_inc,
              g->d_hdiag, g->d_b, g->d_chi};
    PgoSysPtrs s{g->d_hdiag, g->d_hoff, g->d_brow, g->d_bcol, g->d_cptr, g->d_contrib, g->d_blocks, g->d_diag};
    PGOCHK(g, hipEventRecord(g->ev0, g->stream));
    hipLaunchKernelGGL(k_pgo_factors, dim3(g->blocksF), dim3(PGO_BLOCK), 0, g->stream, p, g->F);
    hipLaunchKernelGGL(k_pgo_reduce, dim3((g->N + PGO_BLOCK - 1) / PGO_BLOCK), dim3(PGO_BLOCK), 0, g->stream, p, g->N);
    hipLaunchKernelGGL(k_pgo_assemble, dim3((g->nnzb + PGO_BLOCK - 1) / PGO_BLOCK), dim3(PGO_BLOCK), 0, g->stream, s, g->nnzb);
    hipLaunchKernelGGL(k_pgo_sum, dim3(1), dim3(64), 0, g->stream, (const double*)g->d_chi, g->blocksF, (double*)g->d_half);
    PGOCHK(g, hipEventRecord(g->ev1, g->stream));
    PGOCHK(g, hipGetLastError());
    if (blocks) PGOCHK(g, hipMemcpyAsync(blocks, g->d_blocks, sizeof(double) * 9 * g->nnzb, hipMemcpyDeviceToHost, g->stream));
    if (b) PGOCHK(g, hipMemcpyAsync(b, g->d_b, sizeof(double) * 3 * g->N, hipMemcpyDeviceToHost, g->stream));
    if (diag) PGOCHK(g, hipMemcpyAsync(diag, g->d_diag, sizeof(double) * 3 * g->N, hipMemcpyDeviceToHost, g->stream));
    double h = 0.0;
    PGOCHK(g, hipMemcpyAsync(&h, g->d_half, sizeof(double), hipMemcpyDeviceToHost, g->stream));
    PGOCHK(g, hipStreamSynchronize(g->stream));
    if (half_chi2) *half_chi2 = h;
    if (kernel_ms) { float ms = 0; PGOCHK(g, hipEventElapsedTime(&ms, g->ev0, g->ev1)); *kernel_ms = ms; }
    return LAMA_HIP_OK;
}

int32_t lama_hip_pgo_try_step(lama_hip_pgo* g, const double* dx, double* half_chi2, double* kernel_ms)
{
    if (!g || !dx || !half_chi2) return LAMA_HIP_E_INVALID;
    PGOCHK(g, hipSetDevice(g->device));
    PgoPtrs p{g->d_cand, g->d_fi, g->d_fj, g->d_meas, g->d_sqrt, g->d_err, g->d_hoff, g->d_fdi, g->d_fdj, g->d_fg, g->d_incptr, g->d_inc,
              g->d_hdiag, g->d_b, g->d_chi};
    PGOCHK(g, hipMemcpyAsync(g->d_dx, dx, sizeof(double) * 3 * g->N, hipMemcpyHostToDevice, g->stream));
    PGOCHK(g, hipEventRecord(g->ev0, g->stream));
    hipLaunchKernelGGL(k_pgo_retract, dim3((g->N + PGO_BLOCK - 1) / PGO_BLOCK), dim3(PGO_BLOCK), 0, g->stream, (const double*)g->d_poses,
                       (const double*)g->d_dx, (double*)g->d_cand, g->N);
    hipLaunchKernelGGL(k_pgo_error, dim3(g->blocksF), dim3(PGO_BLOCK), 0, g->stream, p, (const double*)g->d_cand, g->F);
    hipLaunchKernelGGL(k_pgo_sum, dim3(1), dim3(64), 0, g->stream, (const double*)g->d_chi, g->blocksF, (double*)g->d_half);
    PGOCHK(g, hipEventRecord(g->ev1, g->stream));
    PGOCHK(g, hipGetLastError());
    double h = 0.0;
    PGOCHK(g, hipMemcpyAsync(&h, g->d_half, sizeof(double), hipMemcpyDeviceToHost, g->stream));
    PGOCHK(g, hipStreamSynchronize(g->stream));
    *half_chi2 = h;
    if (kernel_ms) { float ms = 0; PGOCHK(g, hipEventElapsedTime(&ms, g->ev0, g->ev1)); *kernel_ms = ms; }
    return LAMA_HIP_OK;
}

int32_t lama_hip_pgo_accept(lama_hip_pgo* g)
{
    if (!g) return LAMA_HIP_E_INVALID;
    g->d_poses.swap(g->d_cand);
    return LAMA_HIP_OK;
}

int32_t lama_hip_map_add_obstacles(lama_hip_ctx* c, uint32_t particle, const uint32_t* cells_xy, uint32_t n)
{
    if (!c || !cells_xy || n == 0 || particle >= c->P) return LAMA_HIP_E_INVALID;
    ENTER(c);
    HIPCHK(c, hipSetDevice(c->cfg.device));
    {
        const int64_t r = (int64_t)(((uint32_t)std::ceil(std::sqrt((double)c->max_sqdist)) + 1u + 31u) / 32u);
        int64_t x0 = INT64_MAX, x1 = INT64_MIN, y0 = INT64_MAX, y1 = INT64_MIN;
        for (uint32_t i = 0; i < n; ++i) {
            const int64_t px = cells_xy[2 * i] >> 5, py = cells_xy[2 * i + 1] >> 5;
            x0 = std::min(x0, px); x1 = std::max(x1, px); y0 = std::min(y0, py); y1 = std::max(y1, py);
        }
        const int32_t rw = ensure_window(c, x0 - r, x1 + r, y0 - r, y1 + r);
        if (rw) return rw;
    }
    { const int32_t rf = start_without_first_scan(c); if (rf) return rf; }
    {
        const int r = (int)(((uint32_t)std::ceil(std::sqrt((double)c->max_sqdist)) + 1u + 31u) / 32u);
        std::vector<uint64_t> keys;
        keys.reserve((size_t)n);
        uint64_t last = ~0ull;
        for (uint32_t i = 0; i < n; ++i) {
            const uint64_t k = ((uint64_t)(cells_xy[2 * i + 1] >> 5) << 32) | (uint64_t)(cells_xy[2 * i] >> 5);
            if (k != last) { keys.push_back(k); last = k; }
        }
        std::sort(keys.begin(), keys.end());
        keys.erase(std::unique(keys.begin(), keys.end()), keys.end());
        std::vector<uint64_t> dil;
        dil.reserve(keys.size() * (size_t)((2 * r + 1) * (2 * r + 1)));
        for (uint64_t k : keys)
            for (int dy = -r; dy <= r; ++dy)
                for (int dx = -r; dx <= r; ++dx) dil.push_back((((k >> 32) + (uint64_t)(int64_t)dy) << 32) | (uint32_t)((uint32_t)k + (uint32_t)dx));
        std::sort(dil.begin(), dil.end());
        dil.erase(std::unique(dil.begin(), dil.end()), dil.end());
        const uint64_t want = (uint64_t)c->h_counts[2 * particle] + dil.size();
        if (want > c->h_part[particle].dm_cap) {
            const int32_t rg = set_capacities(c, {CapRequest{particle, (uint32_t)std::min<uint64_t>(MAX_PATCHES, (want + 31u) / 32u * 32u), c->h_part[particle].occ_cap}});
            if (rg) return rg;
        }
        c->last_guarded = false;
    }
    DevBuf<uint32_t> cells;
    HIPCHK(c, cells.alloc(2 * (size_t)n));
    uint32_t* const d_cells = cells;
    HIPCHK(c, hipMemcpyAsync(d_cells, cells_xy, sizeof(uint32_t) * 2 * (size_t)n, hipMemcpyHostToDevice, c->stream));
    DevParams prm = make_params(c);
    if (n > c->cfg.queue_capacity) return fail(c, LAMA_HIP_E_CAPACITY, "more obstacle cells than cfg.queue_capacity");
    HIPCHK(c, hipMemsetAsync(c->d_slow_n, 0, 5 * sizeof(uint32_t), c->stream));
    hipLaunchKernelGGL(k_dm_add_obstacles, dim3(1), dim3(UM_BLOCK), 0, c->stream, prm, (int)particle, d_cells, n);
    hipLaunchKernelGGL((k_brushfire<LQ_SMALL, RQ_SMALL, false, true>), dim3(1), dim3(2 * UM_BLOCK), 0, c->stream, prm, (int)particle, 0);
    hipLaunchKernelGGL((k_brushfire<LQ_BIG, RQ_BIG, true, true>), dim3(1), dim3(2 * UM_BLOCK), 0, c->stream, prm, (int)particle, 0);
    hipLaunchKernelGGL(k_brushfire_slow, dim3(1), dim3(UM_BLOCK), 0, c->stream, prm, (int)particle);
    HIPCHK(c, hipGetLastError());
    return check_device_errors(c, true, false);
}

int32_t lama_hip_map_integrate_scans(lama_hip_ctx* c, uint32_t particle, uint32_t K, const double* poses4, const double* pts, const uint32_t* offs,
                                     const double* origins, const double* quats, uint32_t flags)
{
    if (!c || particle >= c->P || (flags & ~3u)) return LAMA_HIP_E_INVALID;
    ENTER(c);
    if (c->cfg.occupancy_policy != 0) return fail(c, LAMA_HIP_E_INVALID, "key scans are integrated into a frequency occupancy map (cfg.occupancy_policy 0)");
    if (K == 0) return LAMA_HIP_OK;
    if (!poses4 || !offs) return fail(c, LAMA_HIP_E_INVALID, "poses4 / scan_offsets missing");
    for (uint32_t k = 0; k < K; ++k)
        if (offs[k + 1] < offs[k]) return fail(c, LAMA_HIP_E_INVALID, "scan_offsets must not decrease");
    const uint64_t total64 = (uint64_t)offs[K] - offs[0];
    if (total64 == 0) return LAMA_HIP_OK;
    if (!pts || total64 >= (uint64_t)MB_HIT) return fail(c, LAMA_HIP_E_INVALID, "pts_xyz missing, or more than 2^31 - 1 points");
    const uint32_t total = (uint32_t)total64;
    const bool full = flags & 1u, prune = flags & 2u;
    c->h_mb_tfs.resize((size_t)12 * K); c->h_mb_offs.resize((size_t)K + 1);
    for (uint32_t k = 0; k < K; ++k) {
        host_scan_tf(poses4 + 4 * (size_t)k, moving_tf(origins ? origins + 3 * (size_t)k : nullptr, quats ? quats + 4 * (size_t)k : nullptr), &c->h_mb_tfs[12 * (size_t)k]);
        for (int j = 0; j < 12; ++j)
            if (!std::isfinite(c->h_mb_tfs[12 * (size_t)k + j])) return fail(c, LAMA_HIP_E_INVALID, "a key pose or sensor transform is not finite");
    }
    for (uint32_t k = 0; k <= K; ++k) c->h_mb_offs[k] = offs[k] - offs[0];
    HIPCHK(c, hipSetDevice(c->cfg.device));
    HIPCHK(c, c->d_mb_pts.grow((size_t)3 * total)); HIPCHK(c, c->d_mb_tfs.grow((size_t)12 * K)); HIPCHK(c, c->d_mb_offs.grow((size_t)K + 1));
    HIPCHK(c, c->d_mb_rays.grow(total)); HIPCHK(c, c->d_mb_meta.grow(8));
    c->h_mb_meta.resize(8);
    MbBounds* const d_bounds = reinterpret_cast<MbBounds*>(c->d_mb_meta.p);
    MbMeta* const d_meta = reinterpret_cast<MbMeta*>(c->d_mb_meta.p + 4);
    {
        MbBounds b0{0xFFFFFFFFu, 0u, 0xFFFFFFFFu, 0u, 0u, 0u, 0ull};
        std::memcpy(c->h_mb_meta.data(), &b0, sizeof(b0));
    }
    HIPCHK(c, hipMemcpyAsync(c->d_mb_meta, c->h_mb_meta.data(), sizeof(MbBounds), hipMemcpyHostToDevice, c->stream));
    HIPCHK(c, hipMemcpyAsync(c->d_mb_pts, pts + 3 * (size_t)offs[0], sizeof(double) * 3 * total, hipMemcpyHostToDevice, c->stream));
    HIPCHK(c, hipMemcpyAsync(c->d_mb_tfs, c->h_mb_tfs.data(), sizeof(double) * 12 * K, hipMemcpyHostToDevice, c->stream));
    HIPCHK(c, hipMemcpyAsync(c->d_mb_offs, c->h_mb_offs.data(), sizeof(uint32_t) * ((size_t)K + 1), hipMemcpyHostToDevice, c->stream));
    DevParams prm = make_params(c);
    prm.trunc_ray = 0.0; prm.trunc_range = 0.0;
    const unsigned ray_blocks = (total + 255u) / 256u;
    MbRay* const d_rays = c->d_mb_rays;
    {
        Timer t(c, &c->ctr.ms_raycast, &c->ctr.launches_raycast);
        hipLaunchKernelGGL(k_mb_geom, dim3(ray_blocks), dim3(256), 0, c->stream, prm, (const double*)c->d_mb_pts, (const uint32_t*)c->d_mb_offs,
                           (const double*)c->d_mb_tfs, K, total, full ? 1 : 0, d_rays, d_bounds);
        t.stop();
    }
    HIPCHK(c, hipGetLastError());
    HIPCHK(c, hipMemcpyAsync(c->h_mb_meta.data(), c->d_mb_meta, sizeof(MbBounds), hipMemcpyDeviceToHost, c->stream));
    HIPCHK(c, hipStreamSynchronize(c->stream));
    MbBounds bnd;
    std::memcpy(&bnd, c->h_mb_meta.data(), sizeof(bnd));
    if (bnd.flags & MB_NONFINITE) { resolve_timers(c); return fail(c, LAMA_HIP_E_INVALID, "a key scan holds a non-finite point (filter NaN / inf ranges first, as iris_lama_ros does)"); }
    if (bnd.flags & MB_TOO_LONG) { resolve_timers(c); return fail(c, LAMA_HIP_E_WINDOW, "a ray is longer than 8191 cells"); }
    {
        const int64_t x0 = bnd.x0, x1 = bnd.x1, y0 = bnd.y0, y1 = bnd.y1;
        const int64_t ux0 = c->mb_valid ? std::min(c->mbx0, x0) : x0, ux1 = c->mb_valid ? std::max(c->mbx1, x1) : x1;
        const int64_t uy0 = c->mb_valid ? std::min(c->mby0, y0) : y0, uy1 = c->mb_valid ? std::max(c->mby1, y1) : y1;
        if (ux1 - ux0 + 1 > LAMA_HIP_MAX_WINDOW || uy1 - uy0 + 1 > LAMA_HIP_MAX_WINDOW) {
            resolve_timers(c);
            return fail(c, LAMA_HIP_E_WINDOW, "the key scans and the map so far are wider than the largest device window (1016 patches)");
        }
        const int32_t rw = ensure_window(c, x0, x1, y0, y1);
        if (rw) { resolve_timers(c); return rw; }
    }
    { const int32_t rf = start_without_first_scan(c); if (rf) return rf; }
    const uint32_t bx0 = bnd.x0 - (c->wx0 >> 5), by0 = bnd.y0 - (c->wy0 >> 5), bw = bnd.x1 - bnd.x0 + 1u, bh = bnd.y1 - bnd.y0 + 1u, nb = bw * bh;
    if (bx0 + bw > c->W || by0 + bh > c->W) { resolve_timers(c); return fail(c, LAMA_HIP_E_WINDOW, "the key scans fell outside the device window"); }
    HIPCHK(c, c->d_mb_table.grow(nb)); HIPCHK(c, c->d_mb_off.grow((size_t)nb + 1)); HIPCHK(c, c->d_mb_list.grow(nb)); HIPCHK(c, c->d_mb_slot.grow(nb));
    prm = make_params(c);
    prm.trunc_ray = 0.0; prm.trunc_range = 0.0;
    uint32_t* const d_table = c->d_mb_table; uint32_t* const d_off = c->d_mb_off; uint32_t* const d_list = c->d_mb_list; int32_t* const d_slot = c->d_mb_slot;
    HIPCHK(c, hipMemsetAsync(d_table, 0, sizeof(uint32_t) * nb, c->stream));
    {
        Timer t(c, &c->ctr.ms_raycast, &c->ctr.launches_raycast);
        hipLaunchKernelGGL(k_mb_bin, dim3(ray_blocks), dim3(256), 0, c->stream, prm, (const MbRay*)d_rays, total, bx0, by0, bw, bh, d_table, (const uint32_t*)nullptr, (uint32_t*)nullptr);
        hipLaunchKernelGGL(k_mb_scan, dim3(1), dim3(MB_SCAN_BLOCK), 0, c->stream, prm, (int)particle, bx0, by0, bw, nb, d_table, d_off, d_list, d_meta);
        t.stop();
    }
    HIPCHK(c, hipGetLastError());
    HIPCHK(c, hipMemcpyAsync(c->h_mb_meta.data() + 4, d_meta, sizeof(MbMeta), hipMemcpyDeviceToHost, c->stream));
    HIPCHK(c, hipStreamSynchronize(c->stream));
    MbMeta meta;
    std::memcpy(&meta, c->h_mb_meta.data() + 4, sizeof(meta));
    const uint64_t want = (uint64_t)c->h_counts[2 * particle + 1] + meta.need;
    if (want > MAX_PATCHES) { resolve_timers(c); return fail(c, LAMA_HIP_E_CAPACITY, "the particle's occupancy map would exceed 32767 patches"); }
    if (want > c->h_part[particle].occ_cap) {
        const int32_t rg = set_capacities(c, {CapRequest{particle, c->h_part[particle].dm_cap, want_capacity(c->floor_occ, (uint32_t)want, 0u)}});
        if (rg) { resolve_timers(c); return rg; }
        prm = make_params(c);
        prm.trunc_ray = 0.0; prm.trunc_range = 0.0;
    }
    HIPCHK(c, c->d_mb_bins.grow(meta.items, (size_t)1 << 16));
    uint32_t* const d_bins = c->d_mb_bins;
    {
        Timer t(c, &c->ctr.ms_raycast, &c->ctr.launches_raycast);
        hipLaunchKernelGGL(k_mb_alloc, dim3((meta.touched + 255u) / 256u), dim3(256), 0, c->stream, prm, (int)particle, bx0, by0, bw, (const uint32_t*)d_list, meta.touched, d_slot);
        hipLaunchKernelGGL(k_mb_bin, dim3(ray_blocks), dim3(256), 0, c->stream, prm, (const MbRay*)d_rays, total, bx0, by0, bw, bh, d_table, (const uint32_t*)d_off, d_bins);
        hipLaunchKernelGGL(k_mb_patches, dim3(meta.touched), dim3(256), 0, c->stream, prm, (int)particle, bx0, by0, bw, (const uint32_t*)d_list, (const int32_t*)d_slot,
                           (const uint32_t*)d_off, (const uint32_t*)d_bins, (const MbRay*)d_rays);
        if (prune) hipLaunchKernelGGL(k_mb_prune, dim3((unsigned)std::min<uint64_t>(std::max<uint64_t>(want, 1), 4096)), dim3(256), 0, c->stream, prm, (int)particle);
        t.stop();
    }
    HIPCHK(c, hipGetLastError());
    c->h_err.resize(1);
    HIPCHK(c, hipMemcpyAsync(&c->h_counts[2 * particle], c->ms.counts + 2 * particle, sizeof(int32_t) * 2, hipMemcpyDeviceToHost, c->stream));
    HIPCHK(c, hipMemcpyAsync(&c->h_err[0], c->d_err, sizeof(int32_t), hipMemcpyDeviceToHost, c->stream));
    HIPCHK(c, hipStreamSynchronize(c->stream));
    resolve_timers(c);
    c->ctr.ray_cells += bnd.visits;
    { uint64_t oc = 0; for (uint32_t p = 0; p < c->P; ++p) oc += (uint64_t)c->h_counts[2 * p + 1]; c->ctr.occ_patches = oc; }
    c->visit_bound = 65535u;
    if (c->h_err[0] != 0) {
        HIPCHK(c, hipMemsetAsync(c->d_err, 0, sizeof(int32_t), c->stream));
        HIPCHK(c, hipStreamSynchronize(c->stream));
        return fail(c, LAMA_HIP_E_CAPACITY, "an occupancy patch could not be allocated while integrating key scans");
    }
    return LAMA_HIP_OK;
}

int32_t lama_hip_map_occupied_cells(lama_hip_ctx* c, uint32_t particle, uint32_t cap, uint32_t* cells_xy, uint32_t* n_out)
{
    if (!c || !n_out || particle >= c->P) return LAMA_HIP_E_INVALID;
    ENTER(c);
    if (c->cfg.occupancy_policy != 0) return fail(c, LAMA_HIP_E_INVALID, "occupied cells are listed for a frequency occupancy map (cfg.occupancy_policy 0)");
    *n_out = 0;
    const uint32_t count = (uint32_t)c->h_counts[2 * particle + 1];
    if (count == 0) return LAMA_HIP_OK;
    HIPCHK(c, hipSetDevice(c->cfg.device));
    HIPCHK(c, c->d_mb_table.grow(count)); HIPCHK(c, c->d_mb_off.grow((size_t)count + 1)); HIPCHK(c, c->d_mb_list.grow(count)); HIPCHK(c, c->d_mb_slot.grow(count));
    uint32_t* const d_cnt = c->d_mb_table; uint32_t* const d_off = c->d_mb_off; uint32_t* const d_pos = c->d_mb_list; int32_t* const d_slot = c->d_mb_slot;
    const DevParams prm = make_params(c);
    hipLaunchKernelGGL(k_mb_order, dim3(1), dim3(MB_SCAN_BLOCK), 0, c->stream, prm, (int)particle, d_slot, d_pos);
    hipLaunchKernelGGL(k_mb_occupied, dim3(count), dim3(256), 0, c->stream, prm, (int)particle, (const int32_t*)d_slot, (const uint32_t*)d_pos, d_cnt, (const uint32_t*)nullptr, 0u, (uint32_t*)nullptr);
    hipLaunchKernelGGL(k_mb_exscan, dim3(1), dim3(MB_SCAN_BLOCK), 0, c->stream, (const uint32_t*)d_cnt, count, d_off);
    HIPCHK(c, hipGetLastError());
    uint32_t total = 0;
    HIPCHK(c, hipMemcpyAsync(&total, d_off + count, sizeof(uint32_t), hipMemcpyDeviceToHost, c->stream));
    HIPCHK(c, hipStreamSynchronize(c->stream));
    *n_out = total;
    const uint32_t m = std::min(cap, total);
    if (!cells_xy || m == 0) return LAMA_HIP_OK;
    HIPCHK(c, c->d_mb_bins.grow(2 * (size_t)m, (size_t)1 << 16));
    uint32_t* const d_out = c->d_mb_bins;
    hipLaunchKernelGGL(k_mb_occupied, dim3(count), dim3(256), 0, c->stream, prm, (int)particle, (const int32_t*)d_slot, (const uint32_t*)d_pos, d_cnt, (const uint32_t*)d_off, m, d_out);
    HIPCHK(c, hipGetLastError());
    HIPCHK(c, hipMemcpyAsync(cells_xy, d_out, sizeof(uint32_t) * 2 * (size_t)m, hipMemcpyDeviceToHost, c->stream));
    HIPCHK(c, hipStreamSynchronize(c->stream));
    return LAMA_HIP_OK;
}

static int32_t match_eval_impl(lama_hip_ctx* c, uint32_t particle, const double* pts, uint32_t n, const double* origin3, const double* quat,
// ... 299 lines not shown
        for (uint32_t k = 0; k < n; ++k) {
            int32_t hdr[8];
            std::memcpy(hdr, c->h_ship_heads.data() + (size_t)BLOB_HEAD * k + 32, 32);
            const HostPart& pr = c->h_part[particles[k]];
            const uint32_t nd = want_capacity(c->floor_dm, (uint32_t)hdr[0], 0u), no = want_capacity(c->floor_occ, (uint32_t)hdr[1], 0u);
            if ((uint32_t)hdr[0] > pr.dm_cap || (uint32_t)hdr[1] > pr.occ_cap) reqs.push_back(CapRequest{particles[k], std::max(nd, pr.dm_cap), std::max(no, pr.occ_cap)});
        }
        (void)max_dm; (void)max_occ;
        if (!reqs.empty()) { rc = set_capacities(c, reqs); if (rc) return rc; }
    }
    rc = upload_ship_desc(c, n);
    if (rc) return rc;
    HIPCHK(c, hipMemcpyAsync(c->d_oldcounts, c->ms.counts, sizeof(int32_t) * 2 * c->P, hipMemcpyDeviceToDevice, c->stream));
    hipLaunchKernelGGL(k_import_particles, dim3(n, 7, SHIP_SPLIT), dim3(256), 0, c->stream, make_params(c), (const ShipDesc*)c->d_ship_desc, (const int32_t*)c->d_oldcounts,
                       c->d_poses, c->d_err);
    HIPCHK(c, hipGetLastError());
    { const int32_t ri = check_device_errors(c); if (ri) return ri; }
    for (uint32_t k = 0; k < n; ++k) {
        const uint8_t* head = c->h_ship_heads.data() + (size_t)BLOB_HEAD * k;
        int32_t hdr[8];
        std::memcpy(hdr, head + 32, 32);
        const uint32_t i = particles[k];
        std::memcpy(&c->h_poses[4 * i], head, 32);
        c->h_counts[2 * i] = hdr[0]; c->h_counts[2 * i + 1] = hdr[1];
        c->visit_bound = std::max<uint32_t>(c->visit_bound, (uint32_t)std::min<int32_t>(std::max<int32_t>(hdr[4], 0), 65535));
    }
    return LAMA_HIP_OK;
}

int32_t lama_hip_pf_import_particle(lama_hip_ctx* c, uint32_t particle, const void* buf, uint64_t bytes)
{
    const void* b1 = buf;
    return lama_hip_pf_import_particles(c, 1, &particle, &b1, &bytes);
}

int32_t lama_hip_blob_alloc(lama_hip_ctx* c, uint64_t bytes, void** buf)
{
    if (!c || !buf || bytes == 0) return LAMA_HIP_E_INVALID;
    *buf = nullptr;
    HIPCHK(c, hipSetDevice(c->cfg.device));
    HIPCHK(c, hipMalloc(buf, bytes));
    return LAMA_HIP_OK;
}

int32_t lama_hip_blob_free(lama_hip_ctx* c, void* buf)
{
    if (!c) return LAMA_HIP_E_INVALID;
    if (!buf) return LAMA_HIP_OK;
    HIPCHK(c, hipSetDevice(c->cfg.device));
    HIPCHK(c, hipFree(buf));
    return LAMA_HIP_OK;
}

static int peer_access_between(int a, int b)
{
    static std::mutex mu;
    static std::map<std::pair<int, int>, int> state;
    std::lock_guard<std::mutex> lock(mu);
    int prev_dev = -1;
    (void)hipGetDevice(&prev_dev);
    auto one_way = [&](int from, int to) -> int {
        const auto key = std::make_pair(from, to);
        auto it = state.find(key);
        if (it != state.end()) return it->second;
        int can = 0, ok = 0;
        if (hipDeviceCanAccessPeer(&can, from, to) == hipSuccess && can) {
            if (hipSetDevice(from) == hipSuccess) {
                const hipError_t e = hipDeviceEnablePeerAccess(to, 0);
                ok = (e == hipSuccess || e == hipErrorPeerAccessAlreadyEnabled) ? 1 : 0;
                if (!ok) (void)hipGetLastError();
            }
        } else (void)hipGetLastError();
        state[key] = ok;
        return ok;
    };
    const int ab = one_way(a, b), ba = one_way(b, a);
    if (prev_dev >= 0) (void)hipSetDevice(prev_dev);
    return ab && ba;
}

int32_t lama_hip_blob_copy(lama_hip_ctx* dc, void* dst, lama_hip_ctx* sc, const void* src, uint64_t bytes)
{
    if (!dc || !sc || !dst || !src) return LAMA_HIP_E_INVALID;
    if (bytes == 0) return LAMA_HIP_OK;
    if (dc->cfg.device == sc->cfg.device) {
        HIPCHK(dc, hipSetDevice(dc->cfg.device));
        HIPCHK(dc, hipMemcpyAsync(dst, src, bytes, hipMemcpyDeviceToDevice, dc->stream));
        HIPCHK(dc, hipStreamSynchronize(dc->stream));
        return LAMA_HIP_OK;
    }
    const int peer = peer_access_between(dc->cfg.device, sc->cfg.device);
    dc->ctr.peer_access = (uint32_t)peer;
    HIPCHK(dc, hipSetDevice(dc->cfg.device));
    hipEvent_t e0 = dc->ev0, e1 = dc->ev1;
    HIPCHK(dc, hipEventRecord(e0, dc->stream));
    HIPCHK(dc, hipMemcpyPeerAsync(dst, dc->cfg.device, src, sc->cfg.device, bytes, dc->stream));
    HIPCHK(dc, hipEventRecord(e1, dc->stream));
    HIPCHK(dc, hipStreamSynchronize(dc->stream));
    float ms = 0;
    if (hipEventElapsedTime(&ms, e0, e1) == hipSuccess) { dc->ctr.peer_copy_ms += ms; dc->ctr.peer_copy_bytes += bytes; }
    return LAMA_HIP_OK;
}

int32_t lama_hip_debug_cycles(lama_hip_ctx* c, uint64_t* out )
{
    if (!c || !out) return LAMA_HIP_E_INVALID;
    ENTER(c);
    HIPCHK(c, hipMemcpy(out, c->d_dbg, sizeof(uint64_t) * 8 * c->P, hipMemcpyDeviceToHost));
    return LAMA_HIP_OK;
}

int32_t lama_hip_debug_cycles2(lama_hip_ctx* c, uint64_t* out )
{
    if (!c || !out) return LAMA_HIP_E_INVALID;
    ENTER(c);
    HIPCHK(c, hipMemcpy(out, c->d_dbg + 8 * (size_t)c->P, sizeof(uint64_t) * 8 * c->P, hipMemcpyDeviceToHost));
    return LAMA_HIP_OK;
}

int32_t lama_hip_debug_log(lama_hip_ctx* c, uint64_t* out )
{
    if (!c || !out) return LAMA_HIP_E_INVALID;
    ENTER(c);
    HIPCHK(c, hipMemcpy(out, c->d_dbg + 16 * (size_t)c->P, 1u << 20, hipMemcpyDeviceToHost));
    return LAMA_HIP_OK;
}

#if defined(LAMA_KC_PROBE) || (defined(LAMA_KC_OLD) && LAMA_KC_OLD == 4)
int32_t lama_hip_debug_kc_probe(uint64_t* out )
{
    uint32_t n = 0;
    if (hipMemcpyFromSymbol(&n, HIP_SYMBOL(lama_dev::g_kc_n), sizeof(n)) != hipSuccess) return LAMA_HIP_E_HIP;
    out[0] = n;
    if (hipMemcpyFromSymbol(out + 1, HIP_SYMBOL(lama_dev::g_kc_ev), sizeof(uint64_t) * 512) != hipSuccess) return LAMA_HIP_E_HIP;
    n = 0;
    if (hipMemcpyToSymbol(HIP_SYMBOL(lama_dev::g_kc_n), &n, sizeof(n)) != hipSuccess) return LAMA_HIP_E_HIP;
    return LAMA_HIP_OK;
}
#endif

static void memory_figures(const lama_hip_ctx* c, lama_hip_counters* o)
{
    const MapStore& m = c->ms;
    const uint64_t P = c->P, WW = (uint64_t)c->W * c->W;
    const uint64_t dirs = 2 * P * WW * 2;
    uint64_t dm_used = 0, occ_used = 0;
    for (uint32_t p = 0; p < c->P; ++p) { dm_used += (uint64_t)c->h_counts[2 * p]; occ_used += (uint64_t)c->h_counts[2 * p + 1]; }
    uint64_t dm_pool = 0, occ_pool = 0;
    for (const PoolChunk& k : m.dm_chunks) dm_pool += k.patches;
    for (const PoolChunk& k : m.occ_chunks) occ_pool += k.patches;
    o->hbm_bytes_allocated = dirs + dm_pool * (SV_PATCH_BYTES + 4096 + 128) + occ_pool * (4096 + 128 + 128 + 4);
    o->hbm_bytes_used = dirs + dm_used * (SV_PATCH_BYTES + 4096 + 128) + occ_used * (4096 + 128 + 128 + 4);
    const uint64_t other = 2 * P * (uint64_t)c->cfg.queue_capacity * 8 + P * (uint64_t)c->cfg.active_capacity * 8 + (uint64_t)c->d_rrec.n * (sizeof(lama_dev::RayRec) + 8) +
                           P * (16 * 8 + 12 * 8 + 4 * 8 + 64) + (1u << 20) + (uint64_t)c->d_pts.bytes();
    o->hbm_bytes_total = o->hbm_bytes_allocated + other;
}

int32_t lama_hip_get_counters(lama_hip_ctx* c, lama_hip_counters* out)
{
    if (!c || !out) return LAMA_HIP_E_INVALID;
    ENTER(c);
    *out = c->ctr;
    memory_figures(c, out);
    out->struct_bytes = (uint32_t)sizeof(lama_hip_counters);
    return LAMA_HIP_OK;
}

uint32_t lama_hip_counters_bytes(void) { return (uint32_t)sizeof(lama_hip_counters); }

int32_t lama_hip_get_counters_sized(lama_hip_ctx* c, void* out, uint32_t bytes)
{
    if (!c || !out) return LAMA_HIP_E_INVALID;
    lama_hip_counters full;
    const int32_t rc = lama_hip_get_counters(c, &full);
    if (rc) return rc;
    std::memcpy(out, &full, std::min<size_t>(bytes, sizeof(full)));
    return LAMA_HIP_OK;
}

int32_t lama_hip_reset_counters(lama_hip_ctx* c)
{
    if (!c) return LAMA_HIP_E_INVALID;
    ENTER(c);
    const lama_hip_counters old = c->ctr;
    std::memset(&c->ctr, 0, sizeof(c->ctr));
    c->ctr.dm_patches = old.dm_patches; c->ctr.occ_patches = old.occ_patches;
    c->ctr.brushfire_mode = old.brushfire_mode; c->ctr.brushfire_waves = old.brushfire_waves;
    c->ctr.window_patches = c->W; c->ctr.peer_access = old.peer_access;
    return LAMA_HIP_OK;
}

}
```

### iris_lama_amd/ffi.py

```python
import ctypes as C
import math
import os
import sys

import numpy as np

_HERE = os.path.dirname(os.path.abspath(__file__))
HIP_LIB = os.path.join(_HERE, "lib", "liblama_hip.so")
HIP_LIB_WIDE = os.path.join(_HERE, "lib", "liblama_hip_wide.so")
HOST_LIB = os.path.join(_HERE, "lib", "liblama_host.so")
_PRODUCT_HOST_LIB = HOST_LIB

MAP_DISTANCE, MAP_OCCUPANCY = 0, 1

DIST_T = np.dtype([("obstacle", "<i2", (3,)), ("sqdist", "<u2"), ("valid", "u1"), ("queued", "u1")])
FREQ_T = np.dtype([("occupied", "<u2"), ("visited", "<u2")])


class LamaError(RuntimeError):
    pass


class HipCfg(C.Structure):
    _fields_ = [("particles", C.c_uint32), ("resolution", C.c_double), ("patch_size", C.c_uint32),
                ("l2_max", C.c_double), ("meas_sigma", C.c_double), ("max_iter", C.c_uint32),
                ("truncated_ray", C.c_double), ("truncated_range", C.c_double), ("device", C.c_int32),
                ("window_patches", C.c_uint32), ("dm_patch_capacity", C.c_uint32),
                ("occ_patch_capacity", C.c_uint32), ("queue_capacity", C.c_uint32), ("profile", C.c_uint32),
                ("active_capacity", C.c_uint32), ("sequential_raycast", C.c_uint32), ("brushfire_mode", C.c_uint32),
                ("brushfire_waves", C.c_uint32), ("occupancy_policy", C.c_uint32), ("ray_rule", C.c_uint32),
                ("solver_strategy", C.c_uint32)]


class HipCounters(C.Structure):
    _fields_ = [("ms_scan_match", C.c_double), ("launches_scan_match", C.c_uint64),
                ("ms_update_maps", C.c_double), ("launches_update_maps", C.c_uint64),
                ("ms_raycast", C.c_double), ("launches_raycast", C.c_uint64),
                ("ms_brushfire", C.c_double), ("launches_brushfire", C.c_uint64),
                ("ms_resample", C.c_double), ("launches_resample", C.c_uint64),
                ("gn_iterations", C.c_uint64), ("gn_evals", C.c_uint64), ("ray_cells", C.c_uint64),
                ("bf_cells", C.c_uint64), ("dm_patches", C.c_uint64), ("occ_patches", C.c_uint64),
                ("ms_eval_batch", C.c_double), ("launches_eval_batch", C.c_uint64), ("arena_growths", C.c_uint64), ("window_shifts", C.c_uint64), ("wrap_guard_scans", C.c_uint64),
                ("brushfire_mode", C.c_uint32), ("brushfire_waves", C.c_uint32),
                ("sequential_raycast_scans", C.c_uint64), ("parallel_raycast_scans", C.c_uint64),
                ("brushfire_handovers", C.c_uint32), ("replay_handovers", C.c_uint32),
                ("window_patches", C.c_uint32), ("window_growths", C.c_uint32),
                ("bf_longest_chain_sum", C.c_uint64), ("bf_longest_chain_last", C.c_uint64), ("brushfire_early", C.c_uint64), ("brushfire_routed", C.c_uint64),
                ("pool_growths", C.c_uint64), ("resample_clones", C.c_uint64), ("resample_bytes", C.c_uint64),
                ("hbm_bytes_allocated", C.c_uint64), ("hbm_bytes_used", C.c_uint64), ("hbm_bytes_total", C.c_uint64),
                ("peer_access", C.c_uint32), ("struct_bytes", C.c_uint32), ("peer_copy_ms", C.c_double), ("peer_copy_bytes", C.c_uint64)]

    def as_dict(self):
        return {n: getattr(self, n) for n, _ in self._fields_}


HIP_SYMBOLS = [
    "lama_hip_default_cfg", "lama_hip_device_count", "lama_hip_ctx_create", "lama_hip_ctx_destroy",
    "lama_hip_last_error", "lama_hip_pf_init", "lama_hip_pf_set_poses", "lama_hip_pf_get_poses",
    "lama_hip_pf_scan_match", "lama_hip_pf_resample", "lama_hip_pf_update_maps", "lama_hip_pf_map_patches",
    "lama_hip_pf_download_map", "lama_hip_pf_upload_map", "lama_hip_match_batch", "lama_hip_pf_export_particle",
    "lama_hip_pf_import_particle", "lama_hip_get_counters", "lama_hip_get_counters_sized", "lama_hip_counters_bytes", "lama_hip_reset_counters",
    "lama_hip_map_add_obstacles", "lama_hip_match_solve", "lama_hip_eval_batch", "lama_hip_map_sample_likelihood",
    "lama_hip_pgo_create", "lama_hip_pgo_destroy", "lama_hip_pgo_last_error", "lama_hip_pgo_linearize",
    "lama_hip_pf_patch_ids", "lama_hip_pf_delete_patches", "lama_hip_pf_update_maps_begin", "lama_hip_sync", "lama_hip_ctx_device",
    "lama_hip_pf_map_checksums", "lama_hip_match_eval", "lama_hip_match_cell_distances", "lama_hip_match_solve_with",
    "lama_hip_blob_alloc", "lama_hip_blob_free", "lama_hip_blob_copy", "lama_hip_pf_export_particles", "lama_hip_pf_import_particles",
    "lama_hip_pgo_pattern", "lama_hip_pgo_set_poses", "lama_hip_pgo_get_poses", "lama_hip_pgo_linearize_system",
    "lama_hip_pgo_try_step", "lama_hip_pgo_accept",
    "lama_hip_map_integrate_scans", "lama_hip_map_occupied_cells",
    "lama_hip_match_solve_batch",
]

_hip = None
_hip_wide = None


def _torch_runtime_first():
    if "torch" not in sys.modules and not os.environ.get("LAMA_NO_TORCH_PRELOAD"):
        try:
            import importlib.util
            if importlib.util.find_spec("torch") is not None:
                import torch
        except Exception:
            pass


def hip_lib(wide=False):
    global _hip, _hip_wide
    if wide:
        if _hip_wide is None:
            if not os.path.exists(HIP_LIB_WIDE):
                raise LamaError(f"{HIP_LIB_WIDE} is missing: run `python -c 'import __graft_entry__ as g; g.build()'`. There is no CPU fallback.")
            _torch_runtime_first()
            L = C.CDLL(HIP_LIB_WIDE)
            _bind_hip(L)
            _hip_wide = L
        return _hip_wide
    if _hip is None:
        if not os.path.exists(HIP_LIB):
            raise LamaError(f"{HIP_LIB} is missing: run `python -c 'import __graft_entry__ as g; g.build()'` "
                            "(hipcc --offload-arch=gfx950). There is no CPU fallback.")
        _torch_runtime_first()
        L = C.CDLL(HIP_LIB)
        _bind_hip(L)
        _hip = L
    return _hip


def needs_wide(l2_max, resolution):
    return resolution > 0.0 and math.ceil(l2_max * (1.0 / resolution)) > 127


def is_device_library(path):
    return path.endswith("liblama_hip.so") or path.endswith("liblama_hip_wide.so")


def _lib_of_origin(path):
    if path.endswith("liblama_hip.so"):
        return hip_lib()
    if path.endswith("liblama_hip_wide.so"):
        return hip_lib(wide=True)
    L = C.CDLL(path)
    _bind_hip(L)
    return L


def hip_lib_or_none():
    return _hip


def _bind_hip(L):
    if True:
        vp, i32, u32, u64 = C.c_void_p, C.c_int32, C.c_uint32, C.c_uint64
        L.lama_hip_default_cfg.argtypes = [vp]
        L.lama_hip_default_cfg.restype = None
        L.lama_hip_device_count.argtypes = [vp]
        L.lama_hip_ctx_create.argtypes = [vp, vp]
        L.lama_hip_ctx_destroy.argtypes = [vp]
        L.lama_hip_ctx_destroy.restype = None
        L.lama_hip_last_error.argtypes = [vp]
        L.lama_hip_last_error.restype = C.c_char_p
        L.lama_hip_pf_init.argtypes = [vp, vp, u32, vp, vp, vp]
        L.lama_hip_pf_set_poses.argtypes = [vp, vp]
        L.lama_hip_pf_get_poses.argtypes = [vp, vp]
        L.lama_hip_pf_scan_match.argtypes = [vp, vp, u32, vp, vp, vp, vp, vp]
        L.lama_hip_pf_resample.argtypes = [vp, vp]
        L.lama_hip_pf_update_maps.argtypes = [vp, vp, u32, vp, vp]
        L.lama_hip_pf_update_maps_begin.argtypes = [vp, vp, u32, vp, vp]
        L.lama_hip_sync.argtypes = [vp]
        L.lama_hip_ctx_device.argtypes = [vp]
        L.lama_hip_ctx_device.restype = C.c_int32
        L.lama_hip_pf_map_patches.argtypes = [vp, u32, i32, vp]
        L.lama_hip_pf_download_map.argtypes = [vp, u32, i32, u32, vp, vp, vp, vp]
        L.lama_hip_pf_upload_map.argtypes = [vp, u32, i32, u32, vp, vp, vp]
        L.lama_hip_match_batch.argtypes = [vp, u32, vp, u32, vp, vp, vp, u32, vp]
        L.lama_hip_pf_export_particle.argtypes = [vp, u32, vp, u64, vp]
        L.lama_hip_pf_import_particle.argtypes = [vp, u32, vp, u64]
        L.lama_hip_pf_export_particles.argtypes = [vp, u32, vp, vp, vp, vp]
        L.lama_hip_pf_import_particles.argtypes = [vp, u32, vp, vp, vp]
        L.lama_hip_get_counters.argtypes = [vp, vp]
        L.lama_hip_get_counters_sized.argtypes = [vp, vp, u32]
        L.lama_hip_counters_bytes.argtypes = []
        L.lama_hip_counters_bytes.restype = C.c_uint32
        L.lama_hip_reset_counters.argtypes = [vp]
        L.lama_hip_map_add_obstacles.argtypes = [vp, u32, vp, u32]
        L.lama_hip_match_solve.argtypes = [vp, u32, vp, u32, vp, vp, vp, vp, vp, i32]
        L.lama_hip_eval_batch.argtypes = [vp, u32, vp, u32, vp, vp, vp, u32, vp, vp]
        L.lama_hip_pf_patch_ids.argtypes = [vp, u32, i32, u32, vp, vp]
        L.lama_hip_pf_delete_patches.argtypes = [vp, u32, vp, u32, vp]
        L.lama_hip_map_sample_likelihood.argtypes = [vp, u32, vp, u32, vp, vp, C.c_double, vp, u32, u32, vp]
        L.lama_hip_match_eval.argtypes = [vp, u32, vp, u32, vp, vp, vp, vp, vp]
        L.lama_hip_match_cell_distances.argtypes = [vp, u32, vp, u32, vp, vp, vp, vp]
        L.lama_hip_match_solve_with.argtypes = [vp, u32, vp, u32, vp, vp, vp, vp, vp, i32, u32]
        has_mb = hasattr(L, "lama_hip_map_integrate_scans")
        if has_mb:
            L.lama_hip_map_integrate_scans.argtypes = [vp, u32, u32, vp, vp, vp, vp, vp, u32]
            L.lama_hip_map_occupied_cells.argtypes = [vp, u32, u32, vp, vp]
        has_msb = hasattr(L, "lama_hip_match_solve_batch")
        if has_msb:
            L.lama_hip_match_solve_batch.argtypes = [vp, u32, vp, vp, vp, vp, vp, vp, vp, i32, i32, C.c_double, vp, vp, vp]
        has_cks = hasattr(L, "lama_hip_pf_map_checksums")
        if has_cks:
            L.lama_hip_pf_map_checksums.argtypes = [vp, i32, vp]
        has_pgo = hasattr(L, "lama_hip_pgo_create")
        if has_pgo:
            L.lama_hip_pgo_create.argtypes = [i32, u32, vp, vp, vp, vp, u32, vp]
            L.lama_hip_pgo_destroy.argtypes = [vp]
            L.lama_hip_pgo_destroy.restype = None
            L.lama_hip_pgo_last_error.argtypes = [vp]
            L.lama_hip_pgo_last_error.restype = C.c_char_p
            L.lama_hip_pgo_linearize.argtypes = [vp, vp, vp, vp, vp, vp, vp, vp]
            L.lama_hip_pgo_pattern.argtypes = [vp, vp, vp, vp]
            L.lama_hip_pgo_set_poses.argtypes = [vp, vp]
            L.lama_hip_pgo_get_poses.argtypes = [vp, vp]
            L.lama_hip_pgo_linearize_system.argtypes = [vp, vp, vp, vp, vp, vp]
            L.lama_hip_pgo_try_step.argtypes = [vp, vp, vp, vp]
            L.lama_hip_pgo_accept.argtypes = [vp]
        for s in HIP_SYMBOLS:
            if s.startswith("lama_hip_pgo_") and not has_pgo:
                continue
            if s == "lama_hip_pf_map_checksums" and not has_cks:
                continue
            if s in ("lama_hip_map_integrate_scans", "lama_hip_map_occupied_cells") and not has_mb:
                continue
            if s == "lama_hip_match_solve_batch" and not has_msb:
                continue
            if s not in ("lama_hip_default_cfg", "lama_hip_ctx_destroy", "lama_hip_last_error", "lama_hip_pgo_destroy",
                         "lama_hip_pgo_last_error"):
                getattr(L, s).restype = i32


def _p(a):
    return a.ctypes.data_as(C.c_void_p) if a is not None else None


_IDQ = np.array([1.0, 0.0, 0.0, 0.0])
_Z3 = np.zeros(3)


MAP_BUILD_FULL, MAP_BUILD_PRUNE = 1, 2
ROBUST_KINDS = {"unit": 0, "tukey": 1, "tdist": 2, "cauchy": 3, "huber": 4}
ROBUST_STORED = 0x100
E_NUMERIC = -6


def pack_scans(scans):
    if isinstance(scans, tuple) and len(scans) == 2 and not (hasattr(scans[1], "ndim") and np.ndim(scans[1]) == 2):
        pts = np.ascontiguousarray(scans[0], dtype=np.float64)
        offs = np.asarray(scans[1])
        if pts.ndim != 2 or pts.shape[1] != 3:
            raise ValueError("points must be (N, 3)")
        if offs.ndim != 1 or len(offs) < 1 or np.any(offs < 0) or np.any(offs > 0xFFFFFFFF):
            raise ValueError("offsets must be K + 1 non-negative 32-bit numbers")
        offs = np.ascontiguousarray(offs, dtype=np.uint32)
        if np.any(np.diff(offs.astype(np.int64)) < 0):
            raise ValueError("scan offsets must not decrease")
        if offs[0] != 0 or offs[-1] != len(pts):
            raise ValueError(f"scan offsets must run from 0 to the number of points ({len(pts)}), got {offs[0]} .. {offs[-1]}")
        return pts, offs
    arrs = []
    for a in scans:
        a = np.asarray(a, dtype=np.float64)
        if a.size == 0:
            a = a.reshape(0, 3)
        if a.ndim != 2 or a.shape[1] != 3:
            raise ValueError("every scan must be (n, 3)")
        arrs.append(a)
    offs = np.zeros(len(arrs) + 1, dtype=np.uint32)
    if arrs:
        offs[1:] = np.cumsum([len(a) for a in arrs])
    pts = np.ascontiguousarray(np.concatenate(arrs) if arrs else np.zeros((0, 3)), dtype=np.float64)
    return pts, offs


def default_cfg(**kw):
    cfg = HipCfg()
    hip_lib().lama_hip_default_cfg(C.byref(cfg))
    for k, v in kw.items():
        setattr(cfg, k, v)
    return cfg


def device_count():
    n = C.c_int32(0)
    hip_lib().lama_hip_device_count(C.byref(n))
    return n.value


class HipContext:

    def __init__(self, cfg):
        self.L = hip_lib(wide=needs_wide(cfg.l2_max, cfg.resolution))
        self.cfg = cfg
        self.P = cfg.particles
        h = C.c_void_p()
        rc = self.L.lama_hip_ctx_create(C.byref(cfg), C.byref(h))
        if rc != 0:
            raise LamaError(f"lama_hip_ctx_create failed with status {rc} (no usable HIP device or invalid cfg)")
        self.h = h

    def close(self):
        if getattr(self, "h", None) and not getattr(self, "_is_borrowed", False):
            self.L.lama_hip_ctx_destroy(self.h)
        self.h = None

    def __del__(self):
        self.close()

    def _chk(self, rc):
        if rc != 0:
            raise LamaError(f"status {rc}: {self.L.lama_hip_last_error(self.h).decode()}")

    @staticmethod
    def _scan(pts, origin, quat):
        pts = np.ascontiguousarray(pts, dtype=np.float64)
        origin = np.ascontiguousarray(_Z3 if origin is None else origin, dtype=np.float64)
        quat = np.ascontiguousarray(_IDQ if quat is None else quat, dtype=np.float64)
        return pts, origin, quat

    def init(self, pts, pose0, origin=None, quat=None):
        pts, origin, quat = self._scan(pts, origin, quat)
        pose0 = np.ascontiguousarray(pose0, dtype=np.float64)
        self._chk(self.L.lama_hip_pf_init(self.h, _p(pts), len(pts), _p(origin), _p(quat), _p(pose0)))

    def set_poses(self, poses):
        poses = np.ascontiguousarray(poses, dtype=np.float64)
        assert poses.shape == (self.P, 4)
        self._chk(self.L.lama_hip_pf_set_poses(self.h, _p(poses)))

    def get_poses(self):
        out = np.zeros((self.P, 4))
        self._chk(self.L.lama_hip_pf_get_poses(self.h, _p(out)))
        return out

    def scan_match(self, pts, origin=None, quat=None):
        pts, origin, quat = self._scan(pts, origin, quat)
        poses = np.zeros((self.P, 4))
        ll = np.zeros(self.P)
        it = np.zeros(self.P, dtype=np.int32)
        self._chk(self.L.lama_hip_pf_scan_match(self.h, _p(pts), len(pts), _p(origin), _p(quat), _p(poses), _p(ll), _p(it)))
        return poses, ll, it

    def resample(self, idx):
        idx = np.ascontiguousarray(idx, dtype=np.int32)
        assert idx.shape == (self.P,)
        self._chk(self.L.lama_hip_pf_resample(self.h, _p(idx)))

    def update_maps(self, pts, origin=None, quat=None):
        pts, origin, quat = self._scan(pts, origin, quat)
        self._chk(self.L.lama_hip_pf_update_maps(self.h, _p(pts), len(pts), _p(origin), _p(quat)))

    def download_map(self, particle, kind):
        n = C.c_uint32(0)
        self._chk(self.L.lama_hip_pf_map_patches(self.h, particle, kind, C.byref(n)))
        n = n.value
        ids = np.zeros(n, dtype=np.uint64)
        dt = DIST_T if kind == MAP_DISTANCE else FREQ_T
        cells = np.zeros((n, 1024), dtype=dt)
        masks = np.zeros((n, 16), dtype=np.uint64)
        got = C.c_uint32(0)
        self._chk(self.L.lama_hip_pf_download_map(self.h, particle, kind, n, _p(ids), _p(cells), _p(masks), C.byref(got)))
        assert got.value == n
        return {int(ids[k]): (cells[k], masks[k]) for k in range(n)}

    def upload_map(self, particle, kind, patches):
        ids = np.array(sorted(patches), dtype=np.uint64)
        dt = DIST_T if kind == MAP_DISTANCE else FREQ_T
        cells = np.zeros((len(ids), 1024), dtype=dt)
        masks = np.zeros((len(ids), 16), dtype=np.uint64)
        for k, i in enumerate(ids):
            cells[k], masks[k] = patches[int(i)]
        self._chk(self.L.lama_hip_pf_upload_map(self.h, particle, kind, len(ids), _p(ids), _p(cells), _p(masks)))

    def match_batch(self, particle, pts, poses, origin=None, quat=None):
        pts, origin, quat = self._scan(pts, origin, quat)
        poses = np.ascontiguousarray(poses, dtype=np.float64)
        out = np.zeros(len(poses))
        self._chk(self.L.lama_hip_match_batch(self.h, particle, _p(pts), len(pts), _p(origin), _p(quat), _p(poses), len(poses), _p(out)))
        return out
# ... 20 lines not shown
        self._chk(self.L.lama_hip_pf_patch_ids(self.h, particle, kind, n.value, _p(ids), C.byref(n)))
        return ids

    def delete_patches(self, particle, ids):
        ids = np.ascontiguousarray(ids, dtype=np.uint64)
        d = C.c_uint32(0)
        self._chk(self.L.lama_hip_pf_delete_patches(self.h, particle, _p(ids), len(ids), C.byref(d)))
        return d.value

    def eval_batch(self, particle, pts, poses, origin=None, quat=None):
        pts, origin, quat = self._scan(pts, origin, quat)
        poses = np.ascontiguousarray(poses, dtype=np.float64)
        sq, ll = np.zeros(len(poses)), np.zeros(len(poses))
        self._chk(self.L.lama_hip_eval_batch(self.h, particle, _p(pts), len(pts), _p(origin), _p(quat), _p(poses), len(poses), _p(sq), _p(ll)))
        return sq, ll

    def sample_likelihood(self, particle, pts, yaw, xy, point_step, origin=None, quat=None):
        pts, origin, quat = self._scan(pts, origin, quat)
        xy = np.ascontiguousarray(xy, dtype=np.float64).reshape(-1, 2)
        out = np.zeros(len(xy))
        self._chk(self.L.lama_hip_map_sample_likelihood(self.h, particle, _p(pts), len(pts), _p(origin), _p(quat), float(yaw), _p(xy),
                                                        len(xy), int(point_step), _p(out)))
        return out

    def add_obstacles(self, particle, cells_xy):
        cells = np.ascontiguousarray(cells_xy, dtype=np.uint32).reshape(-1, 2)
        self._chk(self.L.lama_hip_map_add_obstacles(self.h, particle, _p(cells), len(cells)))

    def integrate_scans(self, particle, poses4, scans, origins=None, quats=None, full=True, prune=True):
        pts, offs = pack_scans(scans)
        K = len(offs) - 1
        poses4 = np.ascontiguousarray(poses4, dtype=np.float64).reshape(-1, 4)
        if len(poses4) != K:
            raise ValueError(f"{len(poses4)} poses for {K} scans")
        if origins is not None:
            origins = np.ascontiguousarray(origins, dtype=np.float64).reshape(-1, 3)
            if len(origins) != K:
                raise ValueError(f"{len(origins)} sensor origins for {K} scans")
        if quats is not None:
            quats = np.ascontiguousarray(quats, dtype=np.float64).reshape(-1, 4)
            if len(quats) != K:
                raise ValueError(f"{len(quats)} sensor orientations for {K} scans")
        flags = (MAP_BUILD_FULL if full else 0) | (MAP_BUILD_PRUNE if prune else 0)
        self._chk(self.L.lama_hip_map_integrate_scans(self.h, particle, K, _p(poses4), _p(pts), _p(offs), _p(origins), _p(quats), flags))

    def occupied_cells(self, particle):
        n = C.c_uint32(0)
        self._chk(self.L.lama_hip_map_occupied_cells(self.h, particle, 0, None, C.byref(n)))
        out = np.zeros((n.value, 2), dtype=np.uint32)
        if n.value:
            self._chk(self.L.lama_hip_map_occupied_cells(self.h, particle, n.value, _p(out), C.byref(n)))
        return out

    def match_solve(self, particle, pts, pose4, origin=None, quat=None, solve=True):
        pts, origin, quat = self._scan(pts, origin, quat)
        pose = np.array(pose4, dtype=np.float64)
        out = np.zeros(7)
        it = C.c_int32(0)
        self._chk(self.L.lama_hip_match_solve(self.h, particle, _p(pts), len(pts), _p(origin), _p(quat), _p(pose), _p(out),
                                              C.byref(it), 1 if solve else 0))
        return pose, out[:6].copy(), float(out[6]), it.value

    def match_solve_with(self, particle, pts, pose4, strategy=0, max_iterations=0, origin=None, quat=None):
        pts, origin, quat = self._scan(pts, origin, quat)
        pose = np.array(pose4, dtype=np.float64)
        out = np.zeros(7)
        it = C.c_int32(0)
        self._chk(self.L.lama_hip_match_solve_with(self.h, particle, _p(pts), len(pts), _p(origin), _p(quat), _p(pose), _p(out),
                                                   C.byref(it), int(strategy), int(max_iterations)))
        return pose, out, it.value

    def match_solve_batch(self, particles, scans, poses4, max_iterations=100, strategy=0, robust="cauchy", robust_param=0.15,
                          origins=None, quats=None, check=True):
        pts, offs = pack_scans(scans)
        B = len(offs) - 1
        poses = np.array(poses4, dtype=np.float64).reshape(-1, 4)
        if len(poses) != B:
            raise ValueError(f"{len(poses)} poses for {B} problems")
        pa = np.ascontiguousarray(np.broadcast_to(np.asarray(particles, dtype=np.uint32), (B,)))
        mi = np.ascontiguousarray(np.broadcast_to(np.asarray(max_iterations, dtype=np.uint32), (B,)))
        if origins is not None:
            origins = np.ascontiguousarray(origins, dtype=np.float64).reshape(-1, 3)
            if len(origins) != B:
                raise ValueError(f"{len(origins)} sensor origins for {B} problems")
        if quats is not None:
            quats = np.ascontiguousarray(quats, dtype=np.float64).reshape(-1, 4)
            if len(quats) != B:
                raise ValueError(f"{len(quats)} sensor orientations for {B} problems")
        kind = ROBUST_KINDS[robust] if isinstance(robust, str) else int(robust)
        out8, it, st = np.zeros((B, 8)), np.zeros(B, dtype=np.int32), np.zeros(B, dtype=np.uint32)
        args = (self.h, B, _p(pa), _p(pts), _p(offs), _p(origins), _p(quats), _p(poses), _p(mi), int(strategy), kind, float(robust_param),
                _p(out8), _p(it), _p(st))
        rc = self.L.lama_hip_match_solve_batch(*args)
        if rc != 0 and (check or rc != E_NUMERIC):
            self._chk(rc)
        return poses, out8, it, st

    def match_eval(self, particle, pts, pose4, origin=None, quat=None, jac=True):
        pts, origin, quat = self._scan(pts, origin, quat)
        n = len(pts)
        pose = np.ascontiguousarray(pose4, dtype=np.float64)
        r, J = np.zeros(n), (np.zeros((3, n)) if jac else None)
        self._chk(self.L.lama_hip_match_eval(self.h, particle, _p(pts), n, _p(origin), _p(quat), _p(pose), _p(r), _p(J)))
        return r, (J.T.copy() if jac else None)

    def cell_distances(self, particle, pts, pose4, origin=None, quat=None):
        pts, origin, quat = self._scan(pts, origin, quat)
        n = len(pts)
        pose = np.ascontiguousarray(pose4, dtype=np.float64)
        d = np.zeros(n)
        self._chk(self.L.lama_hip_match_cell_distances(self.h, particle, _p(pts), n, _p(origin), _p(quat), _p(pose), _p(d)))
        return d

    def export_bytes(self, particle):
        n = C.c_uint64(0)
        self._chk(self.L.lama_hip_pf_export_particle(self.h, particle, None, 0, C.byref(n)))
        return n.value

    def export_particle(self, particle, device_ptr, cap):
        n = C.c_uint64(0)
        self._chk(self.L.lama_hip_pf_export_particle(self.h, particle, C.c_void_p(device_ptr), cap, C.byref(n)))
        return n.value

    def import_particle(self, particle, device_ptr, nbytes):
        self._chk(self.L.lama_hip_pf_import_particle(self.h, particle, C.c_void_p(device_ptr), nbytes))

    def export_sizes(self, particles):
        pa = np.ascontiguousarray(particles, dtype=np.uint32)
        out = np.zeros(len(pa), dtype=np.uint64)
        self._chk(self.L.lama_hip_pf_export_particles(self.h, len(pa), _p(pa), None, None, _p(out)))
        return out

    def export_particles(self, particles, device_ptrs, caps):
        pa = np.ascontiguousarray(particles, dtype=np.uint32)
        ptrs = np.ascontiguousarray(device_ptrs, dtype=np.uint64)
        cp = np.ascontiguousarray(caps, dtype=np.uint64)
        out = np.zeros(len(pa), dtype=np.uint64)
        self._chk(self.L.lama_hip_pf_export_particles(self.h, len(pa), _p(pa), _p(ptrs), _p(cp), _p(out)))
        return out

    def import_particles(self, particles, device_ptrs, nbytes):
        pa = np.ascontiguousarray(particles, dtype=np.uint32)
        ptrs = np.ascontiguousarray(device_ptrs, dtype=np.uint64)
        nb = np.ascontiguousarray(nbytes, dtype=np.uint64)
        self._chk(self.L.lama_hip_pf_import_particles(self.h, len(pa), _p(pa), _p(ptrs), _p(nb)))

    def counters(self):
        c = HipCounters()
        self._chk(self.L.lama_hip_get_counters(self.h, C.byref(c)))
        return c.as_dict()

    def reset_counters(self):
        self._chk(self.L.lama_hip_reset_counters(self.h))


_host = None


def host_lib():
    global _host
    if _host is None:
        if not os.path.exists(HOST_LIB):
            raise LamaError(f"{HOST_LIB} is missing: run `make -C iris_lama_amd host`")
        _torch_runtime_first()
        L = C.CDLL(HOST_LIB)
        L.lama_corridor_generate.argtypes = [C.c_int, C.c_int, C.c_void_p, C.c_void_p, C.c_void_p]
        L.lama_corridor_generate.restype = C.c_int
        _host = L
    return _host


def corridor_log(steps=40, beams=1080):
    pts = np.zeros((steps + 1, beams, 3))
    odom = np.zeros((steps + 1, 3))
    truth = np.zeros((steps + 1, 3))
    rc = host_lib().lama_corridor_generate(steps, beams, _p(pts), _p(odom), _p(truth))
    if rc != 0:
        raise LamaError("lama_corridor_generate failed")
    return pts, odom, truth


class PFOptions(C.Structure):
    _fields_ = [("particles", C.c_uint32), ("srr", C.c_double), ("str", C.c_double), ("stt", C.c_double),
                ("srt", C.c_double), ("meas_sigma", C.c_double), ("meas_sigma_gain", C.c_double),
                ("trans_thresh", C.c_double), ("rot_thresh", C.c_double), ("l2_max", C.c_double),
                ("truncated_ray", C.c_double), ("truncated_range", C.c_double), ("resolution", C.c_double),
                ("patch_size", C.c_uint32), ("max_iter", C.c_uint32), ("seed", C.c_uint32),
                ("create_summary", C.c_int32), ("gpu_device", C.c_int32), ("shard_rank", C.c_uint32),
                ("shard_world", C.c_uint32), ("profile", C.c_int32), ("brushfire_mode", C.c_uint32),
                ("window_patches", C.c_uint32), ("dm_patch_capacity", C.c_uint32), ("occ_patch_capacity", C.c_uint32),
                ("queue_capacity", C.c_uint32), ("gpus", C.c_int32)]


HOST_SYMBOLS = [
    "lama_corridor_generate", "lama_pf_default_options", "lama_pf_engine_origin",
    "lama_pf_create", "lama_pf_destroy", "lama_pf_last_error", "lama_pf_set_prior", "lama_pf_update",
    "lama_pf_update_begin", "lama_pf_local_range", "lama_pf_local_loglik", "lama_pf_plan_resample",
    "lama_pf_apply_resample", "lama_pf_update_maps", "lama_pf_device_context", "lama_pf_get_poses",
    "lama_pf_set_pose", "lama_pf_get_weights", "lama_pf_set_weights", "lama_pf_neff", "lama_pf_best",
    "lama_pf_best_pose_xyr", "lama_pf_num_resamples", "lama_pf_exchange_times", "lama_pf_shard_context", "lama_pf_memory_usage", "lama_pf_summary",
    "lama_pf_last_times", "lama_pf_draw_from_motion", "lama_pf_normalize", "lama_pf_resample_indices",
    "lama_pose_minus", "lama_pose_from_xyr",
    "lama_slam_default_options", "lama_slam_create", "lama_slam_destroy", "lama_slam_last_error", "lama_slam_set_pose",
    "lama_slam_get_pose", "lama_slam_update", "lama_slam_enough_motion", "lama_slam_processed_cells",
    "lama_slam_iterations", "lama_slam_device_context", "lama_slam_engine_origin", "lama_slam_deleted_patches", "lama_loc_create3",
    "lama_slam_view_bounds", "lama_slam_view_cells", "lama_slam_view_occupancy", "lama_slam_view_distance_cells", "lama_slam_view_distance_points",
    "lama_slam_match_eval", "lama_slam_match_solve", "lama_slam_match_solve_generic", "lama_slam_solve_batch",
    "lama_loc_create", "lama_loc_destroy", "lama_loc_last_error", "lama_loc_engine_origin", "lama_loc_set_obstacles_world",
    "lama_loc_write_distance_map", "lama_loc_read_distance_map", "lama_loc_device_context",
    "lama_loc_set_pose", "lama_loc_get_pose", "lama_loc_update", "lama_loc_covar", "lama_loc_rmse", "lama_loc_iterations",
    "lama_loc_create2", "lama_loc_occ_set_cells", "lama_loc_occ_bounds", "lama_loc_trigger_global_localization",
    "lama_loc_global_localization_active", "lama_loc_gloc_candidates", "lama_loc_sampling_likelihoods",
    "lama_random_set_seed", "lama_random_uniform",
    "lama_sdm_write", "lama_sdm_read", "lama_sdm_image", "lama_sdm_export_png", "lama_dm_build", "lama_dm_build_fetch",
    "lama_lo_create", "lama_lo_destroy", "lama_lo_last_error", "lama_lo_engine_origin", "lama_lo_update", "lama_lo_get_odom",
    "lama_lo_iterations", "lama_lo_deleted_patches", "lama_lo_device_context",
    "lama_pgo_optimize",
    "lama_mapbuilder_default_options", "lama_mapbuilder_create", "lama_mapbuilder_destroy", "lama_mapbuilder_last_error",
    "lama_mapbuilder_engine_origin", "lama_mapbuilder_device_context", "lama_mapbuilder_add", "lama_mapbuilder_set_pose",
    "lama_mapbuilder_set_poses", "lama_mapbuilder_build", "lama_mapbuilder_reset", "lama_mapbuilder_occupied_cells",
    "lama_mapbuilder_timing", "lama_mapbuilder_view_cells", "lama_mapbuilder_match_solve",
]


def _bind_host(L):
    vp, i32, u32, d = C.c_void_p, C.c_int32, C.c_uint32, C.c_double
    sig = {
        "lama_pf_default_options": (None, [vp]),
        "lama_pf_engine_origin": (C.c_char_p, [vp]), "lama_pf_create": (vp, [vp, vp, i32]),
        "lama_pf_destroy": (None, [vp]), "lama_pf_last_error": (C.c_char_p, [vp]),
        "lama_pf_set_prior": (None, [vp, d, d, d]), "lama_pf_update": (i32, [vp, vp, u32, vp, vp, vp, d]),
        "lama_pf_update_begin": (i32, [vp, vp, u32, vp, vp, vp, d]), "lama_pf_local_range": (i32, [vp, vp, vp]),
        "lama_pf_local_loglik": (i32, [vp, vp]), "lama_pf_plan_resample": (i32, [vp, vp, vp]),
        "lama_pf_apply_resample": (i32, [vp, vp]), "lama_pf_update_maps": (i32, [vp]),
        "lama_pf_device_context": (vp, [vp]), "lama_pf_get_poses": (i32, [vp, vp]),
        "lama_pf_set_pose": (i32, [vp, u32, vp]), "lama_pf_get_weights": (i32, [vp, vp, vp, vp]),
        "lama_pf_set_weights": (i32, [vp, vp, vp]), "lama_pf_neff": (d, [vp]), "lama_pf_best": (i32, [vp]),
        "lama_pf_best_pose_xyr": (i32, [vp, vp]), "lama_pf_num_resamples": (u32, [vp]),
        "lama_pf_exchange_times": (i32, [vp, vp]), "lama_pf_shard_context": (vp, [vp, u32]),
        "lama_pf_memory_usage": (C.c_uint64, [vp]), "lama_pf_summary": (i32, [vp, vp, i32]),
        "lama_pf_last_times": (i32, [vp, vp]), "lama_pf_draw_from_motion": (i32, [vp, vp, vp]),
        "lama_pf_normalize": (d, [vp]), "lama_pf_resample_indices": (i32, [vp, d, vp]),
        "lama_pose_minus": (None, [vp, vp, vp]), "lama_pose_from_xyr": (None, [d, d, d, vp]),
        "lama_slam_default_options": (None, [vp]), "lama_slam_create": (vp, [vp, vp, i32]), "lama_slam_destroy": (None, [vp]),
        "lama_slam_last_error": (C.c_char_p, [vp]), "lama_slam_set_pose": (None, [vp, d, d, d]),
        "lama_slam_get_pose": (i32, [vp, vp]), "lama_slam_update": (i32, [vp, vp, u32, vp, vp, vp, d]),
        "lama_slam_enough_motion": (i32, [vp, vp]), "lama_slam_processed_cells": (u32, [vp]),
        "lama_slam_iterations": (u32, [vp]), "lama_slam_device_context": (vp, [vp]), "lama_slam_deleted_patches": (u32, [vp]),
        "lama_slam_engine_origin": (C.c_char_p, [vp]),
        "lama_slam_view_bounds": (i32, [vp, i32, vp, vp, vp, vp]), "lama_slam_view_cells": (C.c_int64, [vp, i32, vp, C.c_uint64]),
        "lama_slam_view_occupancy": (i32, [vp, C.c_uint64, vp, vp, vp, vp, vp]),
        "lama_slam_view_distance_cells": (i32, [vp, C.c_uint64, vp, vp]), "lama_slam_view_distance_points": (i32, [vp, C.c_uint64, vp, vp]),
        "lama_slam_match_eval": (i32, [vp, vp, u32, vp, vp, vp, vp, vp, vp]),
        "lama_slam_match_solve": (i32, [vp, vp, u32, vp, vp, vp, C.c_char_p, C.c_char_p, d, u32, vp, vp]),
        "lama_slam_match_solve_generic": (i32, [vp, vp, u32, vp, vp, vp, C.c_char_p, C.c_char_p, d, u32, vp, vp]),
        "lama_slam_solve_batch": (i32, [vp, vp, u32, vp, vp, vp, vp, vp, vp, C.c_char_p, d, C.c_char_p, d, vp, vp, vp]),
        "lama_loc_create": (vp, [d, d, d, d, u32, i32, vp, i32]), "lama_loc_destroy": (None, [vp]),
        "lama_loc_last_error": (C.c_char_p, [vp]), "lama_loc_engine_origin": (C.c_char_p, [vp]),
        "lama_loc_set_obstacles_world": (i32, [vp, vp, u32]), "lama_loc_write_distance_map": (i32, [vp, C.c_char_p]), "lama_loc_read_distance_map": (i32, [vp, C.c_char_p]), "lama_loc_device_context": (vp, [vp]), "lama_loc_set_pose": (None, [vp, d, d, d]),
        "lama_loc_get_pose": (i32, [vp, vp]), "lama_loc_update": (i32, [vp, vp, u32, vp, vp, vp, d, i32]),
        "lama_loc_covar": (i32, [vp, vp]), "lama_loc_rmse": (d, [vp]), "lama_loc_iterations": (u32, [vp]),
        "lama_loc_create2": (vp, [d, d, d, d, u32, u32, u32, d, d, i32, vp, i32]),
        "lama_loc_create3": (vp, [d, d, d, d, u32, u32, u32, d, d, C.c_char_p, i32, vp, i32]),
        "lama_loc_occ_set_cells": (i32, [vp, vp, u32, i32]), "lama_loc_occ_bounds": (i32, [vp, vp]),
        "lama_loc_trigger_global_localization": (None, [vp]), "lama_loc_global_localization_active": (i32, [vp]),
        "lama_loc_gloc_candidates": (u32, [vp, vp, vp, u32]), "lama_loc_sampling_likelihoods": (u32, [vp, vp, u32]),
        "lama_random_set_seed": (None, [u32]), "lama_random_uniform": (d, []),
        "lama_lo_create": (vp, [d, u32, i32, vp, i32]), "lama_lo_destroy": (None, [vp]), "lama_lo_last_error": (C.c_char_p, [vp]),
        "lama_lo_engine_origin": (C.c_char_p, [vp]), "lama_lo_update": (i32, [vp, vp, u32, vp, vp, d]),
        "lama_lo_get_odom": (i32, [vp, vp]), "lama_lo_iterations": (u32, [vp]), "lama_lo_deleted_patches": (u32, [vp]),
        "lama_lo_device_context": (vp, [vp]),
        "lama_sdm_write": (i32, [C.c_char_p, i32, d, u32, u32, vp, vp, vp]),
        "lama_sdm_read": (i32, [C.c_char_p, vp, vp, vp, u32, vp, vp, vp, vp]),
        "lama_sdm_image": (i32, [i32, d, u32, u32, vp, vp, vp, vp, vp, vp, C.c_uint64]),
        "lama_sdm_export_png": (i32, [i32, d, u32, u32, vp, vp, vp, C.c_char_p]),
        "lama_dm_build": (C.c_int64, [vp, C.c_uint64, u32, vp]), "lama_dm_build_fetch": (i32, [vp, vp, vp]),
        "lama_pgo_optimize": (i32, [vp, u32, vp, vp, vp, u32, vp, vp, u32, i32, vp, vp, vp, u32, vp, i32]),
        "lama_mapbuilder_default_options": (None, [vp]), "lama_mapbuilder_create": (vp, [vp, vp, i32]), "lama_mapbuilder_destroy": (None, [vp]),
        "lama_mapbuilder_last_error": (C.c_char_p, [vp]), "lama_mapbuilder_engine_origin": (C.c_char_p, [vp]),
        "lama_mapbuilder_device_context": (vp, [vp]), "lama_mapbuilder_add": (C.c_int64, [vp, vp, u32, vp, vp, vp]),
        "lama_mapbuilder_set_pose": (i32, [vp, C.c_uint64, vp]), "lama_mapbuilder_set_poses": (i32, [vp, vp, C.c_uint64]),
        "lama_mapbuilder_build": (i32, [vp]), "lama_mapbuilder_reset": (i32, [vp]),
        "lama_mapbuilder_occupied_cells": (C.c_int64, [vp, vp, C.c_uint64]), "lama_mapbuilder_timing": (i32, [vp, vp]),
        "lama_mapbuilder_view_cells": (C.c_int64, [vp, i32, vp, C.c_uint64]),
        "lama_mapbuilder_match_solve": (i32, [vp, vp, u32, vp, vp, vp, u32, vp]),
    }
    for name, (res, args) in sig.items():
        f = getattr(L, name)
        f.restype = res
        f.argtypes = args


_host_bound = False


def _hostlib():
    global _host_bound
    L = host_lib()
    if not _host_bound:
        _bind_host(L)
        _host_bound = True
    return L


def use_host_library(path=None):
    global _host, _host_bound, HOST_LIB
# ... 749 lines not shown
```

Before: 16860 particle-scans/s.

## Defer map-update status check into next scan match and pack readbacks into one block

Scan match and set_poses no longer block on the pending map update. The new scan goes up on a side stream into a double-buffered points array, and the deferred map-update error and status check is collected with the same device-to-host copy as the match results. Transforms, status, stats, error words and results are placed in one contiguous device block, so each readback is a single memcpy, and the per-update memset is folded into the transform upload. If the deferred update needs capacity recovery, the earlier poses and scan are restored, the update is replayed and the scan match is redone, which adds complexity and a rare extra pass.

```diff
diff --git a/include/lama_hip.h b/include/lama_hip.h
--- a/include/lama_hip.h
+++ b/include/lama_hip.h
@@ -197,6 +197,7 @@
 int32_t lama_hip_get_counters_sized(lama_hip_ctx* ctx, void* out, uint32_t bytes);
 uint32_t lama_hip_counters_bytes(void);
 int32_t lama_hip_reset_counters(lama_hip_ctx* ctx);
+int32_t lama_hip_pf_scan_match_redone(lama_hip_ctx* ctx, uint64_t* redone, uint64_t* collected);
 
 #ifdef __cplusplus
 }
diff --git a/iris_lama_amd/csrc/lama_hip.hip b/iris_lama_amd/csrc/lama_hip.hip
--- a/iris_lama_amd/csrc/lama_hip.hip
+++ b/iris_lama_amd/csrc/lama_hip.hip
@@ -195,12 +195,11 @@
     PinVec<double> h_tfs, h_pts;
     PinVec<int32_t> h_err;
     PinVec<uint32_t> h_slow_n;
-    DevBuf<double> d_tfs;
+    double* d_tfs = nullptr;
     double* d_loglik = nullptr; int32_t* d_iters = nullptr;
     DevBuf<uint8_t> d_results;
-    size_t results_bytes = 0, status_off = 0, status_bytes = 0;
-    PinVec<uint8_t> h_status;
-    PinVec<uint8_t> h_results;
+    size_t status_off = 0, results_off = 0, block_bytes = 0;
+    PinVec<uint8_t> h_block;
     DevBuf<int32_t> d_oldcounts;
     DevBuf<double> d_mb_pts, d_mb_tfs; DevBuf<uint32_t> d_mb_offs; DevBuf<lama_dev::MbRay> d_mb_rays;
     DevBuf<uint32_t> d_mb_table, d_mb_off, d_mb_list, d_mb_bins; DevBuf<int32_t> d_mb_slot; DevBuf<uint64_t> d_mb_meta;
@@ -222,6 +221,11 @@
     bool unguarded_retry = false;
     uint32_t saved_visit_bound = 0; lama_hip_counters saved_ctr;
     bool pending_maps = false;
+    std::vector<double> upd_poses; uint32_t upd_n = 0; double upd_reach = 0.0;
+    bool upd_saved = false, upd_scan_replaced = false;
+    Stream stream_up; Event ev_up, ev_head; bool up_dirty = false;
+    DevBuf<double> d_pts_alt;
+    uint64_t scan_match_redone = 0, collected_with_match = 0;
     PinVec<double> h_poses;
     PinVec<int32_t> h_counts;
     lama_hip_counters ctr;
@@ -229,6 +233,7 @@
     ~lama_hip_ctx()
     {
         (void)hipSetDevice(cfg.device);
+        if (stream_up) (void)hipStreamSynchronize(stream_up);
         if (stream) (void)hipStreamSynchronize(stream);
     }
 };
@@ -302,7 +307,7 @@
     return p;
 }
 
-int32_t upload_scan(lama_hip_ctx* c, const double* pts, uint32_t n)
+int32_t upload_scan(lama_hip_ctx* c, const double* pts, uint32_t n, hipStream_t on = nullptr)
 {
     if (!pts) {
         if (c->last_n == 0 || n != c->last_n) return fail(c, LAMA_HIP_E_INVALID, "pts == NULL but no matching scan is resident");
@@ -316,7 +321,7 @@
     for (uint32_t i = 0; i < n; ++i) r2 = std::max(r2, pts[3 * i] * pts[3 * i] + pts[3 * i + 1] * pts[3 * i + 1] + pts[3 * i + 2] * pts[3 * i + 2]);
     if (!std::isfinite(r2)) { c->last_n = 0; return fail(c, LAMA_HIP_E_INVALID, "the scan holds a non-finite point (filter NaN / inf ranges before the update, as iris_lama_ros does)"); }
     c->scan_reach = std::sqrt(r2);
-    HIPCHK(c, hipMemcpyAsync(c->d_pts, c->h_pts.data(), sizeof(double) * 3 * n, hipMemcpyHostToDevice, c->stream));
+    HIPCHK(c, hipMemcpyAsync(c->d_pts, c->h_pts.data(), sizeof(double) * 3 * n, hipMemcpyHostToDevice, on ? on : (hipStream_t)c->stream));
     return LAMA_HIP_OK;
 }
 
@@ -333,47 +338,32 @@
 void resolve_timers(lama_hip_ctx* c);
 
 int32_t grow_arenas(lama_hip_ctx* c, uint32_t need_dm, uint32_t need_occ);
-int32_t recover_update(lama_hip_ctx* c, int32_t e);
+int32_t recover_update(lama_hip_ctx* c, int32_t e, bool* rematch);
 int32_t run_update_maps(lama_hip_ctx* c, uint32_t n, const Affine& mtf, uint32_t first, uint32_t count);
 int32_t permute_particles(lama_hip_ctx* c, const int32_t* idx);
 
-int32_t check_device_errors(lama_hip_ctx* c, bool maps = false, bool match = false, bool err_in_results = false)
-{
-    c->h_err.resize(1);
-    int32_t& e = c->h_err[0];
-    e = 0;
-    const bool stats = maps || match;
-    const bool packed = maps && !err_in_results;
-    if (stats) c->h_stats.resize((size_t)c->P * 4);
-    if (packed) {
-        c->h_status.resize(c->status_bytes); c->h_guard.resize(c->P); c->h_slow_n.resize(5);
-        HIPCHK(c, hipMemcpyAsync(c->h_status.data(), c->d_results + c->status_off, c->status_bytes, hipMemcpyDeviceToHost, c->stream));
-    } else {
-        if (stats) {
-            HIPCHK(c, hipMemcpyAsync(c->h_counts.data(), c->ms.counts, sizeof(int32_t) * 2 * c->P, hipMemcpyDeviceToHost, c->stream));
-            if (maps) { c->h_guard.resize(c->P); HIPCHK(c, hipMemcpyAsync(c->h_guard.data(), c->d_guard, sizeof(uint32_t) * c->P, hipMemcpyDeviceToHost, c->stream)); }
-            HIPCHK(c, hipMemcpyAsync(c->h_stats.data(), c->d_stats, sizeof(uint64_t) * c->h_stats.size(), hipMemcpyDeviceToHost, c->stream));
-        }
-        if (!err_in_results) HIPCHK(c, hipMemcpyAsync(&e, c->d_err, sizeof(e), hipMemcpyDeviceToHost, c->stream));
-        if (maps) { c->h_slow_n.resize(5); HIPCHK(c, hipMemcpyAsync(c->h_slow_n.data(), c->d_slow_n, 5 * sizeof(uint32_t), hipMemcpyDeviceToHost, c->stream)); }
-    }
-    HIPCHK(c, hipStreamSynchronize(c->stream));
-    if (packed) {
-        const uint8_t* b = c->h_status.data();
-        const size_t o_slow = (const uint8_t*)c->d_slow_n - (c->d_results + c->status_off);
-        std::memcpy(&e, b, sizeof(e));
-        std::memcpy(c->h_slow_n.data(), b + o_slow, 5 * sizeof(uint32_t));
-        std::memcpy(c->h_stats.data(), b + o_slow + 32, sizeof(uint64_t) * 4 * c->P);
-        std::memcpy(c->h_guard.data(), b + o_slow + 32 + sizeof(uint64_t) * 4 * c->P, sizeof(uint32_t) * c->P);
-        std::memcpy(c->h_counts.data(), b + o_slow + 32 + sizeof(uint64_t) * 4 * c->P + sizeof(uint32_t) * 2 * c->P, sizeof(int32_t) * 2 * c->P);
-    }
-    if (maps) { c->ctr.brushfire_handovers += c->h_slow_n[0]; c->ctr.replay_handovers += c->h_slow_n[1] + c->h_slow_n[3]; c->ctr.brushfire_routed += c->h_slow_n[2] + c->h_slow_n[4]; c->ctr.brushfire_early += c->h_slow_n[4]; c->early_candidates = c->h_slow_n[2] + c->h_slow_n[4]; }
-    if (err_in_results) std::memcpy(&e, c->h_results.data() + ((const uint8_t*)c->d_err - c->d_results), sizeof(e));
-    resolve_timers(c);
+int32_t digest_status(lama_hip_ctx* c, bool maps, bool match, bool stats, bool* rematch = nullptr)
+{
+    const uint8_t* b = c->h_block.data();
+    const int word = match ? 1 : 0;
+    int32_t e = 0;
+    std::memcpy(&e, b + c->results_off + 4 * word, sizeof(e));
+    stats = stats || maps;
+    if (stats) {
+        c->h_stats.resize((size_t)c->P * 4);
+        std::memcpy(c->h_stats.data(), b + c->status_off + 32, sizeof(uint64_t) * 4 * c->P);
+        std::memcpy(c->h_counts.data(), b + c->status_off + 32 + sizeof(uint64_t) * 4 * c->P + sizeof(uint32_t) * 2 * c->P, sizeof(int32_t) * 2 * c->P);
+    }
+    if (maps) {
+        c->h_guard.resize(c->P); c->h_slow_n.resize(5);
+        std::memcpy(c->h_slow_n.data(), b + c->status_off, 5 * sizeof(uint32_t));
+        std::memcpy(c->h_guard.data(), b + c->status_off + 32 + sizeof(uint64_t) * 4 * c->P, sizeof(uint32_t) * c->P);
+        c->ctr.brushfire_handovers += c->h_slow_n[0]; c->ctr.replay_handovers += c->h_slow_n[1] + c->h_slow_n[3]; c->ctr.brushfire_routed += c->h_slow_n[2] + c->h_slow_n[4]; c->ctr.brushfire_early += c->h_slow_n[4]; c->early_candidates = c->h_slow_n[2] + c->h_slow_n[4];
+    }
     if (e != 0) {
-        HIPCHK(c, hipMemsetAsync(c->d_err, 0, sizeof(int32_t), c->stream));
+        HIPCHK(c, hipMemsetAsync(c->d_err + word, 0, sizeof(int32_t), c->stream));
         if (maps && (e & ERR_CLEAN_ABORT) && (e & (ERR_DM_CAP | ERR_OCC_CAP)) && !(e & ERR_WINDOW) && c->last_guarded && c->recover_depth < 10) {
-            const int32_t rr = recover_update(c, e);
+            const int32_t rr = recover_update(c, e, rematch);
             if (rr != LAMA_HIP_E_CAPACITY) return rr;
         }
         if (e & (ERR_DM_CAP | ERR_OCC_CAP)) {
@@ -411,8 +401,8 @@
             c->ctr.bf_longest_chain_sum += mx; c->ctr.bf_longest_chain_last = mx;
             if (c->debug_tail) {
                 uint32_t rank = 0; double ll = 0, mean_ll = 0;
-                if (c->h_results.size() >= c->results_bytes && c->P > 1) {
-                    const double* L = reinterpret_cast<const double*>(c->h_results.data() + sizeof(double) * 4 * c->P);
+                if (c->ll_valid && c->P > 1) {
+                    const std::vector<double>& L = c->h_ll;
                     ll = L[arg];
                     for (uint32_t p = 0; p < c->P; ++p) { rank += L[p] < ll ? 1u : 0u; mean_ll += L[p]; }
                     mean_ll /= c->P;
@@ -423,6 +413,15 @@
         if (maps) return grow_arenas(c, 0, 0);
     }
     return LAMA_HIP_OK;
+}
+
+int32_t check_device_errors(lama_hip_ctx* c, bool maps = false)
+{
+    const size_t from = maps ? c->status_off : c->results_off, to = c->results_off + sizeof(int32_t);
+    HIPCHK(c, hipMemcpyAsync(c->h_block.data() + from, c->d_results + from, to - from, hipMemcpyDeviceToHost, c->stream));
+    HIPCHK(c, hipStreamSynchronize(c->stream));
+    resolve_timers(c);
+    return digest_status(c, maps, false, false);
 }
 
 constexpr uint32_t MAX_PATCHES = 32767u;
@@ -602,7 +601,7 @@
     return set_capacities(c, reqs);
 }
 
-int32_t recover_update(lama_hip_ctx* c, int32_t e)
+static int32_t recover_update_pass(lama_hip_ctx* c, int32_t e)
 {
     ++c->recover_depth;
     c->visit_bound = c->saved_visit_bound;
@@ -646,21 +645,54 @@
     const bool saved_unguarded = c->unguarded_retry;
     c->unguarded_retry = at_limit;
     if (rc == LAMA_HIP_OK) rc = run_update_maps(c, c->last_n, c->last_mtf, c->last_first, c->last_count);
-    if (rc == LAMA_HIP_OK) rc = check_device_errors(c, true, false);
+    if (rc == LAMA_HIP_OK) rc = check_device_errors(c, true);
     --c->recover_depth;
     c->unguarded_retry = saved_unguarded;
     return rc;
 }
 
+int32_t recover_update(lama_hip_ctx* c, int32_t e, bool* rematch)
+{
+    if (c->recover_depth != 0 || !c->upd_saved) return recover_update_pass(c, e);
+    std::vector<double> now_poses(c->h_poses.data(), c->h_poses.data() + c->h_poses.size());
+    std::memcpy(c->h_poses.data(), c->upd_poses.data(), sizeof(double) * c->upd_poses.size());
+    if (c->upd_scan_replaced) { c->d_pts.swap(c->d_pts_alt); c->last_n = c->upd_n; c->scan_reach = c->upd_reach; }
+    const int32_t rc = recover_update_pass(c, e);
+    std::memcpy(c->h_poses.data(), now_poses.data(), sizeof(double) * now_poses.size());
+    if (c->upd_scan_replaced) { c->last_n = 0; if (rematch) *rematch = true; }
+    return rc;
+}
+
+int32_t order_side_upload(lama_hip_ctx* c)
+{
+#ifndef LAMA_WAVE_SIM
+    HIPCHK(c, hipEventSynchronize(c->ev_head));
+#endif
+    HIPCHK(c, hipStreamWaitEvent(c->stream_up, c->ev_head, 0));
+    return LAMA_HIP_OK;
+}
+
+int32_t join_uploads(lama_hip_ctx* c)
+{
+    if (!c->up_dirty) return LAMA_HIP_OK;
+    c->up_dirty = false;
+    HIPCHK(c, hipEventRecord(c->ev_up, c->stream_up));
+    HIPCHK(c, hipStreamWaitEvent(c->stream, c->ev_up, 0));
+    return LAMA_HIP_OK;
+}
+
 int32_t finish_pending(lama_hip_ctx* c)
 {
     if (!c->pending_maps) return LAMA_HIP_OK;
     c->pending_maps = false;
     (void)hipSetDevice(c->cfg.device);
-    const int32_t rc = check_device_errors(c, true, false);
+    { const int32_t rj = join_uploads(c); if (rj) return rj; }
+    const int32_t rc = check_device_errors(c, true);
+    c->upd_saved = false;
     if (rc) c->error = "deferred from lama_hip_pf_update_maps_begin: " + c->error;
     return rc;
 }
+#define ENTER_NOWAIT(c) do { if ((c)->poisoned) return fail((c), LAMA_HIP_E_STATE, "the context ran out of device memory in the middle of a resample and cannot continue"); } while (0)
 #define ENTER(c) do { if ((c)->poisoned) return fail((c), LAMA_HIP_E_STATE, "the context ran out of device memory in the middle of a resample and cannot continue"); const int32_t rc_enter_ = finish_pending(c); if (rc_enter_) return rc_enter_; } while (0)
 
 struct Timer {
@@ -823,14 +855,14 @@
     c->last_mtf = mtf; c->last_first = first; c->last_count = count;
     if (c->recover_depth == 0) { c->saved_visit_bound = c->visit_bound; c->saved_ctr = c->ctr; }
     PinVec<double>& tfs = c->h_tfs;
-    tfs.resize((size_t)c->P * 12);
+    tfs.resize((size_t)c->P * 12 + 4 + (size_t)c->P * 4);
     for (uint32_t p = 0; p < c->P; ++p) host_scan_tf(&c->h_poses[4 * p], mtf, &tfs[12 * (size_t)p]);
     HIPCHK(c, hipMemcpyAsync(c->d_tfs, tfs.data(), sizeof(double) * tfs.size(), hipMemcpyHostToDevice, c->stream));
+    HIPCHK(c, hipEventRecord(c->ev_head, c->stream));
     DevParams prm = make_params(c);
     bool early_lane = false;
     {
         Timer t(c, &c->ctr.ms_raycast, &c->ctr.launches_raycast);
-        (void)hipMemsetAsync(c->d_slow_n, 0, 32 + sizeof(uint64_t) * 4 * c->P, c->stream);
         bool sequential = c->cfg.sequential_raycast == 1 || c->cfg.occupancy_policy == 1 ||
                           c->cfg.ray_rule == 1;
         if (!sequential && (n > 4096u || (uint64_t)n + 4096u > c->cfg.active_capacity)) sequential = true;
@@ -1141,19 +1173,20 @@
         if (upload_part(c) != LAMA_HIP_OK) return LAMA_HIP_E_HIP;
         if (hipStreamSynchronize(c->stream)) return LAMA_HIP_E_HIP;
     }
-    c->results_bytes = P * 4 * 8 + P * 8 + P * 4 + 8;
-    c->status_off = P * 4 * 8 + P * 8 + P * 4;
-    const size_t slow_off = (c->results_bytes + 7) / 8 * 8;
-    c->status_bytes = (slow_off - c->status_off) + 32 + P * 4 * 8 + P * 2 * 4 + P * 2 * 4;
-    if (c->d_results.alloc(c->status_off + c->status_bytes) || hipMemset(c->d_results, 0, c->status_off + c->status_bytes)) return LAMA_HIP_E_HIP;
-    c->d_poses = reinterpret_cast<double*>(c->d_results.p);
+    c->status_off = P * 12 * 8;
+    c->results_off = c->status_off + 32 + P * 4 * 8 + P * 2 * 4 + P * 2 * 4;
+    c->block_bytes = c->results_off + 8 + P * 4 * 8 + P * 8 + P * 4;
+    if (c->d_results.alloc(c->block_bytes) || hipMemset(c->d_results, 0, c->block_bytes)) return LAMA_HIP_E_HIP;
+    c->h_block.resize(c->block_bytes);
+    c->d_tfs = reinterpret_cast<double*>(c->d_results.p);
+    c->d_slow_n = reinterpret_cast<uint32_t*>(c->d_results + c->status_off);
+    c->d_stats = reinterpret_cast<uint64_t*>(c->d_results + c->status_off + 32);
+    c->d_guard = reinterpret_cast<uint32_t*>(c->d_stats + P * 4);
+    c->ms.counts = reinterpret_cast<int32_t*>(c->d_guard + P * 2);
+    c->d_err = reinterpret_cast<int32_t*>(c->d_results + c->results_off);
+    c->d_poses = reinterpret_cast<double*>(c->d_results + c->results_off + 8);
     c->d_loglik = c->d_poses + P * 4;
     c->d_iters = reinterpret_cast<int32_t*>(c->d_loglik + P);
-    c->d_err = c->d_iters + P;
-    c->d_slow_n = reinterpret_cast<uint32_t*>(c->d_results + slow_off);
-    c->d_stats = reinterpret_cast<uint64_t*>(c->d_results + slow_off + 32);
-    c->d_guard = reinterpret_cast<uint32_t*>(c->d_stats + P * 4);
-    c->ms.counts = reinterpret_cast<int32_t*>(c->d_guard + P * 2);
     if (c->d_qlower.alloc(P * (size_t)cfg.queue_capacity) || c->d_qraise.alloc(P * (size_t)cfg.queue_capacity)) return LAMA_HIP_E_HIP;
     if (c->d_qsizes.alloc(P * 2) || hipMemset(c->d_qsizes, 0, P * 2 * 4)) return LAMA_HIP_E_HIP;
     if (c->d_dbg.alloc(P * 16 + (1u << 20) / 8) || hipMemset(c->d_dbg, 0, P * 16 * 8 + (1u << 20))) return LAMA_HIP_E_HIP;
@@ -1163,7 +1196,8 @@
     if (c->d_early.alloc(P) || hipMemset(c->d_early, 0, P)) return LAMA_HIP_E_HIP;
     if (c->d_elist.alloc(256) || hipMemset(c->d_elist, 0, 256 * 4)) return LAMA_HIP_E_HIP;
     if (c->d_hlist.alloc(256) || hipMemset(c->d_hlist, 0, 256 * 4)) return LAMA_HIP_E_HIP;
-    if (hipStreamCreate(&c->stream2.h) || hipStreamCreate(&c->stream3.h)) return LAMA_HIP_E_HIP;
+    if (hipStreamCreate(&c->stream2.h) || hipStreamCreate(&c->stream3.h) || hipStreamCreate(&c->stream_up.h)) return LAMA_HIP_E_HIP;
+    if (hipEventCreateWithFlags(&c->ev_up.h, hipEventDisableTiming) || hipEventCreateWithFlags(&c->ev_head.h, hipEventDisableTiming)) return LAMA_HIP_E_HIP;
     if (hipEventCreateWithFlags(&c->ev_alloc.h, hipEventDisableTiming) || hipEventCreateWithFlags(&c->ev_early.h, hipEventDisableTiming) ||
         hipEventCreateWithFlags(&c->ev_go.h, hipEventDisableTiming) ||
         hipEventCreateWithFlags(&c->ev_route.h, hipEventDisableTiming) || hipEventCreateWithFlags(&c->ev_heavy.h, hipEventDisableTiming))
@@ -1171,7 +1205,7 @@
     if (c->d_scalar.alloc(4) || hipMemset(c->d_scalar, 0, 16)) return LAMA_HIP_E_HIP;
     if (c->d_act.alloc(P * (size_t)cfg.active_capacity)) return LAMA_HIP_E_HIP;
     if (c->d_act_count.alloc(P) || hipMemset(c->d_act_count, 0, P * 4)) return LAMA_HIP_E_HIP;
-    if (c->d_tfs.alloc(P * 12) || c->d_oldcounts.alloc(P * 2)) return LAMA_HIP_E_HIP;
+    if (c->d_oldcounts.alloc(P * 2)) return LAMA_HIP_E_HIP;
     if (hipDeviceSynchronize()) return LAMA_HIP_E_HIP;
     c->h_poses.assign(P * 4, 0.0);
     c->h_counts.assign(P * 2, 0);
@@ -1184,10 +1218,17 @@
 int32_t lama_hip_pf_set_poses(lama_hip_ctx* c, const double* poses)
 {
     if (!c || !poses) return LAMA_HIP_E_INVALID;
-    ENTER(c);
+    ENTER_NOWAIT(c);
     HIPCHK(c, hipSetDevice(c->cfg.device));
+    const bool side = c->pending_maps;
+    if (side) {
+        const int32_t ro = order_side_upload(c);
+        if (ro) return ro;
+        if (c->up_dirty) HIPCHK(c, hipStreamSynchronize(c->stream_up));
+    }
     std::memcpy(c->h_poses.data(), poses, sizeof(double) * 4 * c->P);
-    HIPCHK(c, hipMemcpyAsync(c->d_poses, c->h_poses.data(), sizeof(double) * 4 * c->P, hipMemcpyHostToDevice, c->stream));
+    HIPCHK(c, hipMemcpyAsync(c->d_poses, c->h_poses.data(), sizeof(double) * 4 * c->P, hipMemcpyHostToDevice, side ? c->stream_up : c->stream));
+    if (side) c->up_dirty = true;
     return LAMA_HIP_OK;
 }
 
@@ -1217,14 +1258,14 @@
     const Affine mtf = moving_tf(origin3, quat);
     rc = run_update_maps(c, n, mtf, 0, 1);
     if (rc) return rc;
-    rc = check_device_errors(c, true, false);
+    rc = check_device_errors(c, true);
     if (rc) return rc;
     if (c->P > 1) {
         std::vector<int32_t> idx(c->P, 0);
         rc = permute_particles(c, idx.data());
         if (rc) return rc;
     }
-    rc = check_device_errors(c, true, false);
+    rc = check_device_errors(c, true);
     if (rc) return rc;
     c->initialised = true;
     return LAMA_HIP_OK;
@@ -1234,25 +1275,61 @@
                                double* poses_out, double* loglik_out, int32_t* iters_out)
 {
     if (!c || !pts || n == 0) return LAMA_HIP_E_INVALID;
-    ENTER(c);
+    ENTER_NOWAIT(c);
     if (!c->initialised) return fail(c, LAMA_HIP_E_STATE, "lama_hip_pf_scan_match before lama_hip_pf_init");
     HIPCHK(c, hipSetDevice(c->cfg.device));
-    int32_t rc = upload_scan(c, pts, n);
-    if (rc) return rc;
+    bool collect = c->pending_maps;
+    if (collect) { c->upd_n = c->last_n; c->upd_reach = c->scan_reach; }
     const Affine mtf = moving_tf(origin3, quat);
-    DevParams prm = make_params(c);
-    {
-        Timer t(c, &c->ctr.ms_scan_match, &c->ctr.launches_scan_match);
-        if (c->max_sqdist > (uint32_t)SM_LUT) hipLaunchKernelGGL(k_scan_match<true>, dim3(c->P), dim3(SM_BLOCK), 0, c->stream, prm, c->d_pts, (int)n, mtf, c->d_loglik, c->d_iters);
-        else hipLaunchKernelGGL(k_scan_match<false>, dim3(c->P), dim3(SM_BLOCK), 0, c->stream, prm, c->d_pts, (int)n, mtf, c->d_loglik, c->d_iters);
-        t.stop();
-    }
-    HIPCHK(c, hipGetLastError());
-    c->h_results.resize(c->results_bytes);
-    HIPCHK(c, hipMemcpyAsync(c->h_results.data(), c->d_results, c->results_bytes, hipMemcpyDeviceToHost, c->stream));
-    rc = check_device_errors(c, false, c->cfg.profile != 0, true);
-    if (rc) return rc;
-    const uint8_t* r = c->h_results.data();
+    const bool stats = c->cfg.profile != 0;
+    for (;;) {
+        const bool side = collect;
+        int32_t rc = side ? order_side_upload(c) : LAMA_HIP_OK;
+        if (rc) return rc;
+        if (side) c->d_pts.swap(c->d_pts_alt);
+        rc = upload_scan(c, pts, n, side ? (hipStream_t)c->stream_up : nullptr);
+        if (side) c->up_dirty = true;
+        if (rc) {
+            if (side) { c->d_pts.swap(c->d_pts_alt); c->last_n = c->upd_n; c->scan_reach = c->upd_reach; }
+            return rc;
+        }
+        if (side) c->upd_scan_replaced = true;
+        rc = join_uploads(c);
+        if (rc) return rc;
+        DevParams prm = make_params(c);
+        prm.err = c->d_err + 1;
+        {
+            Timer t(c, &c->ctr.ms_scan_match, &c->ctr.launches_scan_match);
+            if (c->max_sqdist > (uint32_t)SM_LUT) hipLaunchKernelGGL(k_scan_match<true>, dim3(c->P), dim3(SM_BLOCK), 0, c->stream, prm, c->d_pts, (int)n, mtf, c->d_loglik, c->d_iters);
+            else hipLaunchKernelGGL(k_scan_match<false>, dim3(c->P), dim3(SM_BLOCK), 0, c->stream, prm, c->d_pts, (int)n, mtf, c->d_loglik, c->d_iters);
+            t.stop();
+        }
+        HIPCHK(c, hipGetLastError());
+        const size_t from = collect || stats ? c->status_off : c->results_off;
+        HIPCHK(c, hipMemcpyAsync(c->h_block.data() + from, c->d_results + from, c->block_bytes - from, hipMemcpyDeviceToHost, c->stream));
+        HIPCHK(c, hipStreamSynchronize(c->stream));
+        resolve_timers(c);
+        if (collect) {
+            collect = false; c->pending_maps = false; c->collected_with_match += 1;
+            bool rematch = false;
+            rc = digest_status(c, true, false, true, &rematch);
+            c->upd_saved = false; c->upd_scan_replaced = false;
+            if (rc || rematch) {
+                const std::string msg = c->error;
+                HIPCHK(c, hipMemsetAsync(c->d_err + 1, 0, sizeof(int32_t), c->stream));
+                HIPCHK(c, hipMemcpyAsync(c->d_poses, c->h_poses.data(), sizeof(double) * 4 * c->P, hipMemcpyHostToDevice, c->stream));
+                if (rc) { HIPCHK(c, hipStreamSynchronize(c->stream)); c->error = "deferred from lama_hip_pf_update_maps_begin: " + msg; return rc; }
+            }
+            if (rematch) {
+                c->scan_match_redone += 1;
+                continue;
+            }
+        }
+        rc = digest_status(c, false, true, stats);
+        if (rc) return rc;
+        break;
+    }
+    const uint8_t* r = c->h_block.data() + c->results_off + 8;
     std::memcpy(c->h_poses.data(), r, sizeof(double) * 4 * c->P);
     if (poses_out) std::memcpy(poses_out, r, sizeof(double) * 4 * c->P);
     if (loglik_out) std::memcpy(loglik_out, r + sizeof(double) * 4 * c->P, sizeof(double) * c->P);
@@ -1286,6 +1363,7 @@
     rc = run_update_maps(c, n, mtf, 0, c->P);
     if (rc) return rc;
     c->pending_maps = true;
+    c->upd_poses.assign(c->h_poses.data(), c->h_poses.data() + c->h_poses.size()); c->upd_saved = true; c->upd_scan_replaced = false;
     return LAMA_HIP_OK;
 }
 
@@ -1873,7 +1951,7 @@
     hipLaunchKernelGGL((k_brushfire<LQ_BIG, RQ_BIG, true, true>), dim3(1), dim3(2 * UM_BLOCK), 0, c->stream, prm, (int)particle, 0);
     hipLaunchKernelGGL(k_brushfire_slow, dim3(1), dim3(UM_BLOCK), 0, c->stream, prm, (int)particle);
     HIPCHK(c, hipGetLastError());
-    return check_device_errors(c, true, false);
+    return check_device_errors(c, true);
 }
 
 int32_t lama_hip_map_integrate_scans(lama_hip_ctx* c, uint32_t particle, uint32_t K, const double* poses4, const double* pts, const uint32_t* offs,
@@ -2479,7 +2557,7 @@
     o->hbm_bytes_allocated = dirs + dm_pool * (SV_PATCH_BYTES + 4096 + 128) + occ_pool * (4096 + 128 + 128 + 4);
     o->hbm_bytes_used = dirs + dm_used * (SV_PATCH_BYTES + 4096 + 128) + occ_used * (4096 + 128 + 128 + 4);
     const uint64_t other = 2 * P * (uint64_t)c->cfg.queue_capacity * 8 + P * (uint64_t)c->cfg.active_capacity * 8 + (uint64_t)c->d_rrec.n * (sizeof(lama_dev::RayRec) + 8) +
-                           P * (16 * 8 + 12 * 8 + 4 * 8 + 64) + (1u << 20) + (uint64_t)c->d_pts.bytes();
+                           P * (16 * 8 + 12 * 8 + 4 * 8 + 64) + (1u << 20) + (uint64_t)c->d_pts.bytes() + (uint64_t)c->d_pts_alt.bytes();
     o->hbm_bytes_total = o->hbm_bytes_allocated + other;
 }
 
@@ -2514,7 +2592,16 @@
     c->ctr.dm_patches = old.dm_patches; c->ctr.occ_patches = old.occ_patches;
     c->ctr.brushfire_mode = old.brushfire_mode; c->ctr.brushfire_waves = old.brushfire_waves;
     c->ctr.window_patches = c->W; c->ctr.peer_access = old.peer_access;
-    return LAMA_HIP_OK;
-}
-
-}
+    c->scan_match_redone = 0; c->collected_with_match = 0;
+    return LAMA_HIP_OK;
+}
+
+int32_t lama_hip_pf_scan_match_redone(lama_hip_ctx* c, uint64_t* redone, uint64_t* collected)
+{
+    if (!c || !redone) return LAMA_HIP_E_INVALID;
+    *redone = c->scan_match_redone;
+    if (collected) *collected = c->collected_with_match;
+    return LAMA_HIP_OK;
+}
+
+}
diff --git a/iris_lama_amd/ffi.py b/iris_lama_amd/ffi.py
--- a/iris_lama_amd/ffi.py
+++ b/iris_lama_amd/ffi.py
@@ -68,7 +68,7 @@
     "lama_hip_pgo_pattern", "lama_hip_pgo_set_poses", "lama_hip_pgo_get_poses", "lama_hip_pgo_linearize_system",
     "lama_hip_pgo_try_step", "lama_hip_pgo_accept",
     "lama_hip_map_integrate_scans", "lama_hip_map_occupied_cells",
-    "lama_hip_match_solve_batch",
+    "lama_hip_match_solve_batch", "lama_hip_pf_scan_match_redone",
 ]
 
 _hip = None
@@ -163,6 +163,9 @@
         L.lama_hip_counters_bytes.argtypes = []
         L.lama_hip_counters_bytes.restype = C.c_uint32
         L.lama_hip_reset_counters.argtypes = [vp]
+        has_redone = hasattr(L, "lama_hip_pf_scan_match_redone")
+        if has_redone:
+            L.lama_hip_pf_scan_match_redone.argtypes = [vp, vp, vp]
         L.lama_hip_map_add_obstacles.argtypes = [vp, u32, vp, u32]
         L.lama_hip_match_solve.argtypes = [vp, u32, vp, u32, vp, vp, vp, vp, vp, i32]
         L.lama_hip_eval_batch.argtypes = [vp, u32, vp, u32, vp, vp, vp, u32, vp, vp]
@@ -205,6 +208,8 @@
                 continue
             if s == "lama_hip_match_solve_batch" and not has_msb:
                 continue
+            if s == "lama_hip_pf_scan_match_redone" and not has_redone:
+                continue
             if s not in ("lama_hip_default_cfg", "lama_hip_ctx_destroy", "lama_hip_last_error", "lama_hip_pgo_destroy",
                          "lama_hip_pgo_last_error"):
                 getattr(L, s).restype = i32
@@ -531,6 +536,14 @@
 
     def reset_counters(self):
         self._chk(self.L.lama_hip_reset_counters(self.h))
+
+    def scan_match_redone(self):
+        return self.deferred_counts()[0]
+
+    def deferred_counts(self):
+        n, m = C.c_uint64(0), C.c_uint64(0)
+        self._chk(self.L.lama_hip_pf_scan_match_redone(self.h, C.byref(n), C.byref(m)))
+        return int(n.value), int(m.value)
 
 
 _host = None
```

Result: faster. 17200 particle-scans/s, median of 6 (+2.0%).
